# GrumpyZhou/patch2pix

Hardware: AMD Instinct MI355X
Metric: image-pairs/sec (480x640, ptmax=400), matching hot path, feature pyramids resident in HBM (higher is better)
Workload: dtype f32-equivalent: fp16x2 (every f32 operand, scaled by an exact power of two, = sum of 2 fp16 planes to within 2^-24 of its magnitude; 3 fp16 MFMA products per f32 product, f32 accumulate); second convolution as Winograd F(2x2,3x3) (transforms in f32, filters transformed in f64)

## Files before the change

include/p2p_hip.h:

```cpp
#ifndef P2P_HIP_H
#define P2P_HIP_H

#include <stddef.h>
#include <stdint.h>

#ifdef __cplusplus
extern "C" {
#endif

#define P2P_OK            0
#define P2P_EINVAL       -1
#define P2P_EHIP         -2
#define P2P_EUNSUPPORTED -3
#define P2P_ENOMEM       -4

typedef void *p2p_stream_t;
typedef struct p2p_ncn p2p_ncn;
typedef struct p2p_regressor p2p_regressor;

int p2p_version(void);
const char *p2p_last_error(void);


int p2p_ncn_create(const float *w1, const float *b1, const float *w2, const float *b2, p2p_ncn **out);
void p2p_ncn_destroy(p2p_ncn *ncn);
int p2p_ncn_set_tile(p2p_ncn *ncn, int ta, int tb, int tc);

typedef struct p2p_ncn_config { int n_layers, kernel_size[4], channels[4], symmetric; } p2p_ncn_config;
typedef struct p2p_ncn_tensors { const float *w[4], *b[4]; } p2p_ncn_tensors;
int p2p_ncn_create_config(const p2p_ncn_config *config, const p2p_ncn_tensors *tensors, p2p_ncn **out);
int p2p_ncn_is_generic(const p2p_ncn *ncn);

typedef struct p2p_bn_params {
    const float *weight, *bias, *running_mean, *running_var;
} p2p_bn_params;

typedef struct p2p_regressor_params {
    const float *conv1_w;
    p2p_bn_params bn1;
    const float *conv2_w;
    p2p_bn_params bn2;
    const float *fc1_w, *fc1_b;
    p2p_bn_params bnf1;
    const float *fc2_w, *fc2_b;
    p2p_bn_params bnf2;
    const float *fc3_w, *fc3_b;
} p2p_regressor_params;

int p2p_regressor_create(const p2p_regressor_params *params, p2p_regressor **out);
void p2p_regressor_destroy(p2p_regressor *reg);

#define P2P_REGRESS_F32     0
#define P2P_REGRESS_FP16X2  3
#define P2P_REGRESS_FP16X2W 4
#define P2P_REGRESS_DEFAULT P2P_REGRESS_FP16X2W
int p2p_regressor_set_mode(p2p_regressor *reg, int mode);
int p2p_regressor_get_mode(const p2p_regressor *reg);

#define P2P_FEAT_COMB_PRE  0
#define P2P_FEAT_COMB_POST 1
typedef struct p2p_regressor_config {
    int n_feat, feat_idx[4];
    int feat_comb;
    int n_conv, conv_dim[4], conv_ker[4], conv_str[4];
    int n_fc, fc_dim[4];
    int psize;
} p2p_regressor_config;
typedef struct p2p_regressor_tensors {
    const float *conv_w[4];
    p2p_bn_params conv_bn[4];
    const float *fc_w[4], *fc_b[4];
    p2p_bn_params fc_bn[4];
    const float *out_w, *out_b;
} p2p_regressor_tensors;
int p2p_regressor_create_config(const p2p_regressor_config *config, const p2p_regressor_tensors *tensors, p2p_regressor **out);
#define P2P_REGRESS_GENERIC 16


size_t p2p_coarse_workspace_bytes(int channels, int hA, int wA, int hB, int wB, int ksize);
size_t p2p_coarse_workspace_bytes_for(const p2p_ncn *ncn, int channels, int hA, int wA, int hB, int wB, int ksize);
size_t p2p_neigh_consensus_workspace_bytes(const p2p_ncn *ncn, int hA, int wA, int hB, int wB);

int p2p_coarse_forward(const float *featA, const float *featB, int channels, int hA, int wA, int hB, int wB,
                       int ksize, const p2p_ncn *ncn, float *corr4d_out, uint8_t *delta_out,
                       void *workspace, size_t workspace_bytes, p2p_stream_t stream);

int p2p_coarse_forward_batch(const float *featA, const float *featB, int batch, int channels, int hA, int wA, int hB,
                             int wB, int ksize, const p2p_ncn *ncn, float *corr4d_out, uint8_t *delta_out,
                             void *workspace, size_t workspace_bytes, p2p_stream_t stream);

int p2p_neigh_consensus_batch(const float *x, int batch, int hA, int wA, int hB, int wB, const p2p_ncn *ncn, float *y_out,
                              void *workspace, size_t workspace_bytes, p2p_stream_t stream);

int p2p_delta_unpack(const uint8_t *delta, size_t n, int ksize, int64_t *out, p2p_stream_t stream);

int p2p_coarse_matches(const float *corr4d, const uint8_t *delta, int hA, int wA, int hB, int wB, int ksize,
                       int upsample, int center, int64_t *matches_out, float *scores_out, p2p_stream_t stream);

int p2p_coarse_matches_batch(const float *corr4d, const uint8_t *delta, int batch, int hA, int wA, int hB, int wB,
                             int ksize, int upsample, int center, int64_t *matches_out, float *scores_out,
                             p2p_stream_t stream);

int p2p_coarse_matches_topk_batch(const float *corr4d, const uint8_t *delta, int batch, int hA, int wA, int hB, int wB,
                                  int ksize, int upsample, int center, int topk, int do_softmax,
                                  int64_t *matches_out, float *scores_out, p2p_stream_t stream);

#define P2P_SCORE_NONE    0
#define P2P_SCORE_SOFTMAX 1
#define P2P_SCORE_L1      2
size_t p2p_coarse_score_workspace_bytes(int batch, int hA, int wA, int hB, int wB);
int p2p_coarse_score_batch(const float *corr4d, int batch, int hA, int wA, int hB, int wB, int normalize,
                           float *cell_scores, float *pair_scores, void *workspace, size_t workspace_bytes,
                           p2p_stream_t stream);

size_t p2p_filter_coarse_workspace_bytes(int batch, int n);
int p2p_filter_coarse_batch(const int64_t *matches, const float *scores, int batch, int n, float ncn_thres, int mutual,
                            int64_t *out_matches, float *out_scores, int *out_counts, void *workspace,
                            size_t workspace_bytes, p2p_stream_t stream);

int p2p_match_tail_batch(const float *fine, const float *scores, const int64_t *coarse, const int *counts,
                         const double *scale, int batch, int stride, float io_thres, double *out_matches,
                         float *out_scores, double *out_coarse, int *out_counts, p2p_stream_t stream);

#define P2P_F32 0
#define P2P_F64 1
#define P2P_I64 2
#define P2P_EPI_SAMPSON  0
#define P2P_EPI_SYM      1
#define P2P_EPI_SYM_SQRT 2
#define P2P_EPI_VALUE    3
int p2p_epipolar_batch(const void *matches, int matches_dtype, const int *counts, const double *F, int batch, int stride,
                       int kind, double eps, const double *edges, int nbins, void *dist, int dist_dtype, int *hist,
                       p2p_stream_t stream);



int p2p_correlation_batch(const float *featA, const float *featB, int batch, int channels, int hA, int wA, int hB, int wB,
                          float *out, p2p_stream_t stream);

int p2p_maxpool4d_batch(const float *x, int batch, int h1, int w1, int h2, int w2, int k, float *pooled_out, uint8_t *delta_out,
                        p2p_stream_t stream);

size_t p2p_mutual_matching_workspace_bytes(int batch, int hA, int wA, int hB, int wB);
int p2p_mutual_matching_batch(const float *x, int batch, int hA, int wA, int hB, int wB, float *y_out, void *workspace,
                              size_t workspace_bytes, p2p_stream_t stream);

typedef struct p2p_conv4d p2p_conv4d;
int p2p_conv4d_create(const float *weight, const float *bias, int c_in, int c_out, int kernel_size, p2p_conv4d **out);
void p2p_conv4d_destroy(p2p_conv4d *conv);
int p2p_conv4d_forward_batch(const p2p_conv4d *conv, const float *x, int batch, int h1, int w1, int h2, int w2, float *y_out,
                             p2p_stream_t stream);

int p2p_l2_normalize(const float *x, size_t outer, int channels, size_t inner, float *y, p2p_stream_t stream);


typedef struct p2p_pyramid {
    const float *level[4];
    int height, width;
} p2p_pyramid;

size_t p2p_regress_workspace_bytes(int n);
size_t p2p_regress_workspace_bytes_mode(int n, int mode);
size_t p2p_regress_workspace_bytes_for(const p2p_regressor *reg, int n);
int p2p_regress(const p2p_regressor *reg1, const p2p_regressor *reg2,
                const p2p_pyramid *im1, const p2p_pyramid *im2,
                const void *proposals, int is_float, int n,
                float *matches1, float *probs1, float *raw1,
                float *matches2, float *probs2, float *raw2,
                void *workspace, size_t workspace_bytes, p2p_stream_t stream);

int p2p_regress_batch(const p2p_regressor *reg1, const p2p_regressor *reg2, int nitems,
                      const p2p_pyramid *im1, const p2p_pyramid *im2, const int *counts,
                      const void *proposals, int is_float,
                      float *matches1, float *probs1, float *raw1,
                      float *matches2, float *probs2, float *raw2,
                      void *workspace, size_t workspace_bytes, p2p_stream_t stream);

int p2p_regress_batch_dev(const p2p_regressor *reg1, const p2p_regressor *reg2, int nitems,
                          const p2p_pyramid *im1, const p2p_pyramid *im2, const int *dev_counts, int stride,
                          const void *proposals, int is_float,
                          float *matches1, float *probs1, float *raw1,
                          float *matches2, float *probs2, float *raw2,
                          void *workspace, size_t workspace_bytes, p2p_stream_t stream);


typedef struct p2p_conv p2p_conv;
int p2p_conv_create(const float *weight, const p2p_bn_params *bn, int ci, int co, int ks, int stride, p2p_conv **out);
void p2p_conv_destroy(p2p_conv *conv);
int p2p_conv_set_tile(p2p_conv *conv, int mt, int nt, int wn);

int p2p_conv_forward(const p2p_conv *conv, const float *x, const int *xmax, int n, int h, int w, const float *residual,
                     int relu, float *y, int *ymax, p2p_stream_t stream);

typedef struct p2p_stem p2p_stem;
int p2p_stem_create(const float *weight, const p2p_bn_params *bn, p2p_stem **out);
void p2p_stem_destroy(p2p_stem *stem);
int p2p_stem_forward(const p2p_stem *stem, const float *image, const int *imax, int n, int h, int w, float *y, p2p_stream_t stream);

int p2p_maxpool_nhwc(const float *x, int n, int c, int h, int w, float *y, int *ymax, p2p_stream_t stream);

int p2p_nhwc_to_nchw(const float *x, int n, int h, int w, int c, float *y, p2p_stream_t stream);

int p2p_absmax_batch(const float *x, size_t count, int items, int *out, p2p_stream_t stream);


typedef struct p2p_resize_item {
    const uint8_t *pixels;
    int in_h, in_w;
    const int32_t *table_x, *table_y;
    int ksize_x, ksize_y;
} p2p_resize_item;
size_t p2p_resize_workspace_bytes(int batch, int max_in_h, int max_in_w, int out_h, int out_w);
int p2p_resize_bicubic_batch(const p2p_resize_item *items, int batch, int out_h, int out_w, uint8_t *out_u8, float *out_f32,
                             size_t out_f32_stride, const float *lut, void *workspace, size_t workspace_bytes,
                             p2p_stream_t stream);

#ifdef __cplusplus
}
#endif
#endif
```

patch2pix_amd/_lib.py:

```python
import ctypes
import os

import torch

_HERE = os.path.dirname(os.path.abspath(__file__))
LIB_PATH = os.path.join(_HERE, "csrc", "libp2p_hip.so")
_ALLOW_EXPERIMENT = os.environ.get("P2P_ALLOW_EXPERIMENT") == "1"
if os.environ.get("P2P_LIB_PATH"):
    if not _ALLOW_EXPERIMENT:
        raise ImportError("P2P_LIB_PATH is set but P2P_ALLOW_EXPERIMENT=1 is not: refusing to load a library other than "
                          f"{LIB_PATH}")
    LIB_PATH = os.environ["P2P_LIB_PATH"]

if not os.path.exists(LIB_PATH):
    raise ImportError(
        f"{LIB_PATH} not found: build the HIP extension first (python -m patch2pix_amd.build, "
        "or __graft_entry__.build()). There is no CPU fallback for the matching path.")

lib = ctypes.CDLL(LIB_PATH)

c_float_p = ctypes.c_void_p
c_stream = ctypes.c_void_p


class BnParams(ctypes.Structure):
    _fields_ = [("weight", ctypes.c_void_p), ("bias", ctypes.c_void_p),
                ("running_mean", ctypes.c_void_p), ("running_var", ctypes.c_void_p)]


class RegressorParams(ctypes.Structure):
    _fields_ = [("conv1_w", ctypes.c_void_p), ("bn1", BnParams),
                ("conv2_w", ctypes.c_void_p), ("bn2", BnParams),
                ("fc1_w", ctypes.c_void_p), ("fc1_b", ctypes.c_void_p), ("bnf1", BnParams),
                ("fc2_w", ctypes.c_void_p), ("fc2_b", ctypes.c_void_p), ("bnf2", BnParams),
                ("fc3_w", ctypes.c_void_p), ("fc3_b", ctypes.c_void_p)]


class RegressorConfig(ctypes.Structure):
    _fields_ = [("n_feat", ctypes.c_int), ("feat_idx", ctypes.c_int * 4), ("feat_comb", ctypes.c_int),
                ("n_conv", ctypes.c_int), ("conv_dim", ctypes.c_int * 4), ("conv_ker", ctypes.c_int * 4),
                ("conv_str", ctypes.c_int * 4), ("n_fc", ctypes.c_int), ("fc_dim", ctypes.c_int * 4), ("psize", ctypes.c_int)]


class RegressorTensors(ctypes.Structure):
    _fields_ = [("conv_w", ctypes.c_void_p * 4), ("conv_bn", BnParams * 4),
                ("fc_w", ctypes.c_void_p * 4), ("fc_b", ctypes.c_void_p * 4), ("fc_bn", BnParams * 4),
                ("out_w", ctypes.c_void_p), ("out_b", ctypes.c_void_p)]


class NcnConfig(ctypes.Structure):
    _fields_ = [("n_layers", ctypes.c_int), ("kernel_size", ctypes.c_int * 4), ("channels", ctypes.c_int * 4),
                ("symmetric", ctypes.c_int)]


class NcnTensors(ctypes.Structure):
    _fields_ = [("w", ctypes.c_void_p * 4), ("b", ctypes.c_void_p * 4)]


class ResizeItem(ctypes.Structure):
    _fields_ = [("pixels", ctypes.c_void_p), ("in_h", ctypes.c_int), ("in_w", ctypes.c_int),
                ("table_x", ctypes.c_void_p), ("table_y", ctypes.c_void_p), ("ksize_x", ctypes.c_int), ("ksize_y", ctypes.c_int)]


class Pyramid(ctypes.Structure):
    _fields_ = [("level", ctypes.c_void_p * 4), ("height", ctypes.c_int), ("width", ctypes.c_int)]


def _sig(name, restype, argtypes):
    fn = getattr(lib, name)
    fn.restype = restype
    fn.argtypes = argtypes
    return fn


p2p_version = _sig("p2p_version", ctypes.c_int, [])
VERSION_EXPERIMENT = 0x40000000
if p2p_version() & VERSION_EXPERIMENT and not _ALLOW_EXPERIMENT:
    raise ImportError(f"{LIB_PATH} is an experiment build (-DP2P_EXPERIMENT); set P2P_ALLOW_EXPERIMENT=1 to load it")
p2p_last_error = _sig("p2p_last_error", ctypes.c_char_p, [])
p2p_ncn_create = _sig("p2p_ncn_create", ctypes.c_int,
                      [ctypes.c_void_p] * 4 + [ctypes.POINTER(ctypes.c_void_p)])
p2p_ncn_destroy = _sig("p2p_ncn_destroy", None, [ctypes.c_void_p])
p2p_ncn_set_tile = _sig("p2p_ncn_set_tile", ctypes.c_int, [ctypes.c_void_p] + [ctypes.c_int] * 3)
p2p_ncn_create_config = _sig("p2p_ncn_create_config", ctypes.c_int,
                             [ctypes.POINTER(NcnConfig), ctypes.POINTER(NcnTensors), ctypes.POINTER(ctypes.c_void_p)])
p2p_ncn_is_generic = _sig("p2p_ncn_is_generic", ctypes.c_int, [ctypes.c_void_p])
p2p_regressor_create = _sig("p2p_regressor_create", ctypes.c_int,
                            [ctypes.POINTER(RegressorParams), ctypes.POINTER(ctypes.c_void_p)])
p2p_regressor_create_config = _sig("p2p_regressor_create_config", ctypes.c_int,
                                   [ctypes.POINTER(RegressorConfig), ctypes.POINTER(RegressorTensors),
                                    ctypes.POINTER(ctypes.c_void_p)])
p2p_regressor_destroy = _sig("p2p_regressor_destroy", None, [ctypes.c_void_p])
p2p_coarse_workspace_bytes = _sig("p2p_coarse_workspace_bytes", ctypes.c_size_t, [ctypes.c_int] * 6)
p2p_coarse_workspace_bytes_for = _sig("p2p_coarse_workspace_bytes_for", ctypes.c_size_t, [ctypes.c_void_p] + [ctypes.c_int] * 6)
p2p_neigh_consensus_workspace_bytes = _sig("p2p_neigh_consensus_workspace_bytes", ctypes.c_size_t,
                                           [ctypes.c_void_p] + [ctypes.c_int] * 4)
p2p_coarse_forward = _sig("p2p_coarse_forward", ctypes.c_int,
                          [ctypes.c_void_p, ctypes.c_void_p] + [ctypes.c_int] * 6 +
                          [ctypes.c_void_p, ctypes.c_void_p, ctypes.c_void_p, ctypes.c_void_p, ctypes.c_size_t, c_stream])
p2p_coarse_forward_batch = _sig("p2p_coarse_forward_batch", ctypes.c_int,
                                [ctypes.c_void_p, ctypes.c_void_p] + [ctypes.c_int] * 7 +
                                [ctypes.c_void_p, ctypes.c_void_p, ctypes.c_void_p, ctypes.c_void_p, ctypes.c_size_t, c_stream])
p2p_neigh_consensus_batch = _sig("p2p_neigh_consensus_batch", ctypes.c_int,
                                 [ctypes.c_void_p] + [ctypes.c_int] * 5 + [ctypes.c_void_p, ctypes.c_void_p, ctypes.c_void_p,
                                                                           ctypes.c_size_t, c_stream])
p2p_delta_unpack = _sig("p2p_delta_unpack", ctypes.c_int,
                        [ctypes.c_void_p, ctypes.c_size_t, ctypes.c_int, ctypes.c_void_p, c_stream])
p2p_coarse_matches = _sig("p2p_coarse_matches", ctypes.c_int,
                          [ctypes.c_void_p, ctypes.c_void_p] + [ctypes.c_int] * 7 +
                          [ctypes.c_void_p, ctypes.c_void_p, c_stream])
p2p_coarse_matches_batch = _sig("p2p_coarse_matches_batch", ctypes.c_int,
                                [ctypes.c_void_p, ctypes.c_void_p] + [ctypes.c_int] * 8 +
                                [ctypes.c_void_p, ctypes.c_void_p, c_stream])
p2p_coarse_matches_topk_batch = _sig("p2p_coarse_matches_topk_batch", ctypes.c_int,
                                     [ctypes.c_void_p, ctypes.c_void_p] + [ctypes.c_int] * 10 +
                                     [ctypes.c_void_p, ctypes.c_void_p, c_stream])
p2p_coarse_score_workspace_bytes = _sig("p2p_coarse_score_workspace_bytes", ctypes.c_size_t, [ctypes.c_int] * 5)
p2p_coarse_score_batch = _sig("p2p_coarse_score_batch", ctypes.c_int,
                              [ctypes.c_void_p] + [ctypes.c_int] * 6 +
                              [ctypes.c_void_p, ctypes.c_void_p, ctypes.c_void_p, ctypes.c_size_t, c_stream])
SCORE_NORMS = {None: 0, "softmax": 1, "l1": 2}
p2p_filter_coarse_workspace_bytes = _sig("p2p_filter_coarse_workspace_bytes", ctypes.c_size_t, [ctypes.c_int, ctypes.c_int])
p2p_filter_coarse_batch = _sig("p2p_filter_coarse_batch", ctypes.c_int,
                               [ctypes.c_void_p, ctypes.c_void_p, ctypes.c_int, ctypes.c_int, ctypes.c_float, ctypes.c_int,
                                ctypes.c_void_p, ctypes.c_void_p, ctypes.c_void_p, ctypes.c_void_p, ctypes.c_size_t, c_stream])
p2p_match_tail_batch = _sig("p2p_match_tail_batch", ctypes.c_int,
                            [ctypes.c_void_p] * 5 + [ctypes.c_int, ctypes.c_int, ctypes.c_float] + [ctypes.c_void_p] * 4 + [c_stream])
p2p_epipolar_batch = _sig("p2p_epipolar_batch", ctypes.c_int,
                          [ctypes.c_void_p, ctypes.c_int, ctypes.c_void_p, ctypes.c_void_p, ctypes.c_int, ctypes.c_int, ctypes.c_int,
                           ctypes.c_double, ctypes.c_void_p, ctypes.c_int, ctypes.c_void_p, ctypes.c_int, ctypes.c_void_p, c_stream])
DTYPES = {"float32": 0, "float64": 1, "int64": 2}
EPI_KINDS = {"sampson": 0, "sym": 1, "sym_sqrt": 2, "value": 3}
EPI_MAX_BINS = 16
p2p_regress = _sig("p2p_regress", ctypes.c_int,
                   [ctypes.c_void_p, ctypes.c_void_p, ctypes.POINTER(Pyramid), ctypes.POINTER(Pyramid),
                    ctypes.c_void_p, ctypes.c_int, ctypes.c_int] + [ctypes.c_void_p] * 6 + [ctypes.c_void_p, ctypes.c_size_t, c_stream])
p2p_regress_workspace_bytes = _sig("p2p_regress_workspace_bytes", ctypes.c_size_t, [ctypes.c_int])
p2p_regress_workspace_bytes_mode = _sig("p2p_regress_workspace_bytes_mode", ctypes.c_size_t, [ctypes.c_int, ctypes.c_int])
p2p_regress_workspace_bytes_for = _sig("p2p_regress_workspace_bytes_for", ctypes.c_size_t, [ctypes.c_void_p, ctypes.c_int])

p2p_regress_batch = _sig("p2p_regress_batch", ctypes.c_int,
                         [ctypes.c_void_p, ctypes.c_void_p, ctypes.c_int, ctypes.POINTER(Pyramid), ctypes.POINTER(Pyramid),
                          ctypes.POINTER(ctypes.c_int), ctypes.c_void_p, ctypes.c_int] + [ctypes.c_void_p] * 6 +
                         [ctypes.c_void_p, ctypes.c_size_t, c_stream])

p2p_regress_batch_dev = _sig("p2p_regress_batch_dev", ctypes.c_int,
                             [ctypes.c_void_p, ctypes.c_void_p, ctypes.c_int, ctypes.POINTER(Pyramid), ctypes.POINTER(Pyramid),
                              ctypes.c_void_p, ctypes.c_int, ctypes.c_void_p, ctypes.c_int] + [ctypes.c_void_p] * 6 +
                             [ctypes.c_void_p, ctypes.c_size_t, c_stream])

p2p_conv_create = _sig("p2p_conv_create", ctypes.c_int,
                       [ctypes.c_void_p, ctypes.POINTER(BnParams)] + [ctypes.c_int] * 4 + [ctypes.POINTER(ctypes.c_void_p)])
p2p_conv_destroy = _sig("p2p_conv_destroy", None, [ctypes.c_void_p])
p2p_conv_set_tile = _sig("p2p_conv_set_tile", ctypes.c_int, [ctypes.c_void_p, ctypes.c_int, ctypes.c_int, ctypes.c_int])
p2p_conv_forward = _sig("p2p_conv_forward", ctypes.c_int,
                        [ctypes.c_void_p, ctypes.c_void_p, ctypes.c_void_p] + [ctypes.c_int] * 3 +
                        [ctypes.c_void_p, ctypes.c_int, ctypes.c_void_p, ctypes.c_void_p, c_stream])
p2p_stem_create = _sig("p2p_stem_create", ctypes.c_int, [ctypes.c_void_p, ctypes.POINTER(BnParams), ctypes.POINTER(ctypes.c_void_p)])
p2p_stem_destroy = _sig("p2p_stem_destroy", None, [ctypes.c_void_p])
p2p_stem_forward = _sig("p2p_stem_forward", ctypes.c_int, [ctypes.c_void_p] * 3 + [ctypes.c_int] * 3 + [ctypes.c_void_p, c_stream])
p2p_maxpool_nhwc = _sig("p2p_maxpool_nhwc", ctypes.c_int, [ctypes.c_void_p] + [ctypes.c_int] * 4 + [ctypes.c_void_p, ctypes.c_void_p, c_stream])
p2p_nhwc_to_nchw = _sig("p2p_nhwc_to_nchw", ctypes.c_int, [ctypes.c_void_p] + [ctypes.c_int] * 4 + [ctypes.c_void_p, c_stream])
p2p_absmax_batch = _sig("p2p_absmax_batch", ctypes.c_int, [ctypes.c_void_p, ctypes.c_size_t, ctypes.c_int, ctypes.c_void_p, c_stream])

p2p_resize_workspace_bytes = _sig("p2p_resize_workspace_bytes", ctypes.c_size_t, [ctypes.c_int] * 5)
p2p_resize_bicubic_batch = _sig("p2p_resize_bicubic_batch", ctypes.c_int,
                                [ctypes.POINTER(ResizeItem)] + [ctypes.c_int] * 3 +
                                [ctypes.c_void_p, ctypes.c_void_p, ctypes.c_size_t, ctypes.c_void_p, ctypes.c_void_p, ctypes.c_size_t,
                                 c_stream])

p2p_correlation_batch = _sig("p2p_correlation_batch", ctypes.c_int, [ctypes.c_void_p, ctypes.c_void_p] + [ctypes.c_int] * 6 + [ctypes.c_void_p, c_stream])
p2p_maxpool4d_batch = _sig("p2p_maxpool4d_batch", ctypes.c_int, [ctypes.c_void_p] + [ctypes.c_int] * 6 + [ctypes.c_void_p, ctypes.c_void_p, c_stream])
p2p_mutual_matching_workspace_bytes = _sig("p2p_mutual_matching_workspace_bytes", ctypes.c_size_t, [ctypes.c_int] * 5)
p2p_mutual_matching_batch = _sig("p2p_mutual_matching_batch", ctypes.c_int,
                                 [ctypes.c_void_p] + [ctypes.c_int] * 5 + [ctypes.c_void_p, ctypes.c_void_p, ctypes.c_size_t, c_stream])
p2p_conv4d_create = _sig("p2p_conv4d_create", ctypes.c_int, [ctypes.c_void_p, ctypes.c_void_p] + [ctypes.c_int] * 3 + [ctypes.POINTER(ctypes.c_void_p)])
p2p_conv4d_destroy = _sig("p2p_conv4d_destroy", None, [ctypes.c_void_p])
p2p_conv4d_forward_batch = _sig("p2p_conv4d_forward_batch", ctypes.c_int,
                                [ctypes.c_void_p, ctypes.c_void_p] + [ctypes.c_int] * 5 + [ctypes.c_void_p, c_stream])
p2p_l2_normalize = _sig("p2p_l2_normalize", ctypes.c_int, [ctypes.c_void_p, ctypes.c_size_t, ctypes.c_int, ctypes.c_size_t, ctypes.c_void_p, c_stream])

p2p_regressor_set_mode = _sig("p2p_regressor_set_mode", ctypes.c_int, [ctypes.c_void_p, ctypes.c_int])
p2p_regressor_get_mode = _sig("p2p_regressor_get_mode", ctypes.c_int, [ctypes.c_void_p])
REGRESS_MODES = {"f32": 0, "fp16x2": 3, "fp16x2w": 4}
REGRESS_GENERIC = 16
FEAT_COMB = {"pre": 0, "post": 1}

EXPORTS = ["p2p_version", "p2p_last_error", "p2p_ncn_create", "p2p_ncn_destroy", "p2p_ncn_set_tile", "p2p_regressor_create",
           "p2p_regressor_destroy", "p2p_coarse_workspace_bytes", "p2p_coarse_forward", "p2p_coarse_forward_batch",
           "p2p_neigh_consensus_batch", "p2p_delta_unpack", "p2p_coarse_matches", "p2p_coarse_matches_batch", "p2p_filter_coarse_workspace_bytes", "p2p_filter_coarse_batch", "p2p_match_tail_batch", "p2p_regress", "p2p_regress_workspace_bytes", "p2p_regress_workspace_bytes_mode", "p2p_regress_batch", "p2p_regress_batch_dev", "p2p_regressor_set_mode",
           "p2p_regressor_get_mode", "p2p_conv_create", "p2p_conv_destroy", "p2p_conv_set_tile", "p2p_conv_forward", "p2p_absmax_batch", "p2p_stem_create", "p2p_stem_destroy", "p2p_stem_forward",
           "p2p_maxpool_nhwc", "p2p_nhwc_to_nchw", "p2p_regressor_create_config", "p2p_regress_workspace_bytes_for",
           "p2p_coarse_matches_topk_batch", "p2p_ncn_create_config", "p2p_ncn_is_generic", "p2p_coarse_workspace_bytes_for",
           "p2p_neigh_consensus_workspace_bytes", "p2p_resize_workspace_bytes", "p2p_resize_bicubic_batch",
           "p2p_coarse_score_workspace_bytes", "p2p_coarse_score_batch", "p2p_epipolar_batch",
           "p2p_correlation_batch", "p2p_maxpool4d_batch", "p2p_mutual_matching_workspace_bytes", "p2p_mutual_matching_batch",
           "p2p_conv4d_create", "p2p_conv4d_destroy", "p2p_conv4d_forward_batch", "p2p_l2_normalize"]


def check(status, what):
    if status != 0:
        msg = p2p_last_error().decode("utf-8", "replace")
        if status == -3:
            raise NotImplementedError(f"{what}: {msg}")
        raise RuntimeError(f"{what} failed with status {status}: {msg}")
```

patch2pix_amd/csrc/api.hip:

```cpp
#include "p2p_common.h"

namespace p2p {
static thread_local char g_err[512] = "";
void set_error(const char *fmt, ...) {
    va_list ap;
    va_start(ap, fmt);
    vsnprintf(g_err, sizeof(g_err), fmt, ap);
    va_end(ap);
}
}

#ifdef P2P_EXPERIMENT
extern "C" int p2p_version(void) { return 110 | P2P_VERSION_EXPERIMENT; }
#else
extern "C" int p2p_version(void) { return 110; }
#endif
extern "C" const char *p2p_last_error(void) { return p2p::g_err; }

#include "coarse_api.hip"
#include "operators_api.hip"
#include "regress_api.hip"
#include "preprocess.hip"
```

patch2pix_amd/csrc/coarse.hip:

```cpp
#include "coarse_common.h"

namespace p2p {

constexpr float MM_EPS = 1e-5f;

__device__ __forceinline__ int f2key(float f) {
    int b = __float_as_int(f);
    return b >= 0 ? b : b ^ 0x7fffffff;
}
__device__ __forceinline__ float key2f(int k) { return __int_as_float(k >= 0 ? k : k ^ 0x7fffffff); }
constexpr int KEY_NEG_INF = (int)0xff800000 ^ 0x7fffffff;

constexpr int PREP_P = 16;
constexpr float CORR_FP16_SCALE = 4096.0f;
__device__ __forceinline__ int prep_row_k4(int pp) { return (pp & ~31) + (pp & 3) + 2 * (pp & 12) + ((pp >> 2) & 4); }
template <bool PERM_A>
__global__ __launch_bounds__(256) void prep_kernel(PrepArgs a) {
    const int img = blockIdx.y;
    if (img == 0) {
        const int i = blockIdx.x * 256 + threadIdx.x;
        if (i <= a.nkeys) a.keys[blockIdx.z * a.sKeys + i] = (i < a.nkeys) ? KEY_NEG_INF : 0;
    }
    const int h = a.h[img], w = a.w[img], C = a.C, k = a.k;
    const bool perm = PERM_A && img == 0;
    if ((int)blockIdx.x * PREP_P >= h * w) return;
    const float *__restrict__ F = a.F[img] + blockIdx.z * a.sF[img];
    unsigned short *__restrict__ Fn = a.Fn[img] + blockIdx.z * a.sFn;
    if (((int)blockIdx.x + 1) * PREP_P >= h * w) {
        const int pad0 = h * w, pad1 = (pad0 + 127) & ~127, pieces = (C >> 5) * 2 * 4;
        for (int e = threadIdx.x; e < (pad1 - pad0) * pieces; e += 256) {
            const int pr = pad0 + e / pieces;
            const int r = (perm ? prep_row_k4(pr) : pr) & 127, q = e % pieces, kc = q >> 3, pl = (q >> 2) & 1, piece = q & 3;
            unsigned short *d = Fn + ((size_t)(pad0 >> 7) * (C >> 5) + kc) * (2 * 128 * 32) + pl * (128 * 32) + (r * 4 + piece) * 8;
            *(f32x4 *)d = (f32x4){0.f, 0.f, 0.f, 0.f};
        }
    }
    __shared__ float tile[256 * (PREP_P + 1)];
    __shared__ float part[16][PREP_P];
    __shared__ float inv[PREP_P];
    const int hw = h * w;
    const int p0 = blockIdx.x * PREP_P;
    const int tid = threadIdx.x;
    for (int e = tid; e < C * 4; e += 256) {
        const int c = e >> 2, q = e & 3;
        const int pos = p0 + 4 * q;
        f32x4 v = {0.f, 0.f, 0.f, 0.f};
        if (pos + 3 < hw && (hw & 3) == 0) v = *(const f32x4 *)(F + (size_t)c * hw + pos);
        else
            for (int i = 0; i < 4; ++i) if (pos + i < hw) v[i] = F[(size_t)c * hw + pos + i];
        float *t = tile + c * (PREP_P + 1) + 4 * q;
        t[0] = v[0]; t[1] = v[1]; t[2] = v[2]; t[3] = v[3];
    }
    __syncthreads();
    {
        const int p = tid & 15, g = tid >> 4;
        float ss = 0.f;
        for (int c = g; c < C; c += 16) { const float v = tile[c * (PREP_P + 1) + p]; ss = fmaf(v, v, ss); }
        part[g][p] = ss;
    }
    __syncthreads();
    if (tid < PREP_P) {
        float ss = 0.f;
#pragma unroll
        for (int g = 0; g < 16; ++g) ss += part[g][tid];
        inv[tid] = 1.0f / sqrtf(ss + 1e-6f);
    }
    __syncthreads();
    const int wc = w / k;
    for (int p = 0; p < PREP_P; ++p) {
        const int pos = p0 + p;
        if (pos >= hw) break;
        const int i = pos / w, j = pos - i * w;
        int pp = ((i / k) * wc + (j / k)) * (k * k) + (i % k) * k + (j % k);
        if (perm) pp = prep_row_k4(pp);
        for (int c = tid; c < C; c += 256) {
            const float x = tile[c * (PREP_P + 1) + p] * inv[p] * CORR_FP16_SCALE;
            const int r = pp & 127;
            unsigned short *d = Fn + ((size_t)(pp >> 7) * (C >> 5) + (c >> 5)) * (2 * 128 * 32) +
                                (r * 4 + (((c >> 3) & 3) ^ ((r >> 2) & 3))) * 8 + (c & 7);
            const _Float16 h0 = (_Float16)x;
            d[0] = __builtin_bit_cast(unsigned short, h0);
            d[128 * 32] = __builtin_bit_cast(unsigned short, (_Float16)(x - (float)h0));
        }
    }
}

void launch_prep(const PrepArgs &a, unsigned nz, hipStream_t stream) {
    const int gp = std::max(ceil_div(std::max(a.h[0] * a.w[0], a.h[1] * a.w[1]), PREP_P), ceil_div(a.nkeys + 1, 256));
    if (a.k == 4) hipLaunchKernelGGL(prep_kernel<true>, dim3(gp, 2, nz), dim3(256), 0, stream, a);
    else hipLaunchKernelGGL(prep_kernel<false>, dim3(gp, 2, nz), dim3(256), 0, stream, a);
}

constexpr int CT = 128;
constexpr int CX_AB = 16;
typedef _Float16 cf16x8 __attribute__((ext_vector_type(8)));
constexpr int CX_BLK = 2 * CT * 64;
constexpr int CX_STAGE = 2 * CX_BLK, CX_LDS = 2 * CX_STAGE;
__device__ __forceinline__ f32x16 cx_mfma(const f32x4 &a, const f32x4 &b, const f32x16 &c) {
    return __builtin_amdgcn_mfma_f32_32x32x16_f16(__builtin_bit_cast(cf16x8, a), __builtin_bit_cast(cf16x8, b), c, 0, 0, 0);
}
#define CX_ISSUE(IT, SLOT)                                                                                             \
    {                                                                                                                  \
        const unsigned char *ga_ = Ab + (size_t)(IT) * CX_BLK + lane16;                                                \
        const unsigned char *gb_ = Bb + (size_t)(IT) * CX_BLK + lane16;                                                \
        unsigned char *la_ = cx + (SLOT) * CX_STAGE + wave * 4096;                                                     \
        P2P_GLOBAL_LOAD_LDS16(ga_, la_, 0); P2P_GLOBAL_LOAD_LDS16(ga_, la_, 1024);                                     \
        P2P_GLOBAL_LOAD_LDS16(ga_, la_, 2048); P2P_GLOBAL_LOAD_LDS16(ga_, la_, 3072);                                  \
        P2P_GLOBAL_LOAD_LDS16(gb_, la_ + CX_BLK, 0); P2P_GLOBAL_LOAD_LDS16(gb_, la_ + CX_BLK, 1024);                   \
        P2P_GLOBAL_LOAD_LDS16(gb_, la_ + CX_BLK, 2048); P2P_GLOBAL_LOAD_LDS16(gb_, la_ + CX_BLK, 3072);                \
    }
#define CX_READ(FA, FB, SLOT, S)                                                                                       \
    {                                                                                                                  \
        const unsigned char *pa_ = cx + (SLOT) * CX_STAGE + ((S) ? aoff1 : aoff0);                                     \
        const unsigned char *pb_ = cx + (SLOT) * CX_STAGE + CX_BLK + ((S) ? boff1 : boff0);                            \
        _Pragma("unroll") for (int t_ = 0; t_ < 2; ++t_)                                                               \
            _Pragma("unroll") for (int q_ = 0; q_ < 2; ++q_) {                                                         \
                FA[t_][q_] = *(const f32x4 *)(pa_ + t_ * 2048 + q_ * 8192);                                            \
                FB[t_][q_] = *(const f32x4 *)(pb_ + t_ * 2048 + q_ * 8192);                                            \
            }                                                                                                          \
    }
#define CX_SLAB(FA, FB)                                                                                                \
    _Pragma("unroll") for (int t_ = 0; t_ < 3; ++t_) {                                                                 \
        const int pa_ = (t_ == 0) ? 1 : 0, pb_ = (t_ == 1) ? 1 : 0;                                                    \
        _Pragma("unroll") for (int i_ = 0; i_ < 2; ++i_)                                                               \
            _Pragma("unroll") for (int j_ = 0; j_ < 2; ++j_) acc[i_][j_] = cx_mfma(FA[i_][pa_], FB[j_][pb_], acc[i_][j_]); \
    }
#define CX_PIPE()                                                                                                      \
    _Pragma("unroll") for (int g_ = 0; g_ < 8; ++g_) {                                                                 \
        __builtin_amdgcn_sched_group_barrier(0x008, 1, 0); __builtin_amdgcn_sched_group_barrier(0x100, 1, 0); }        \
    __builtin_amdgcn_sched_group_barrier(0x008, 4, 0); __builtin_amdgcn_sched_barrier(0);

template <int KS>
__global__ __launch_bounds__(256, 2) void corr_pool_kernel(const unsigned short *__restrict__ A, const unsigned short *__restrict__ B,
                                                           int nA, int nB, int C, float *__restrict__ P,
                                                           uint8_t *__restrict__ delta, size_t sAB, size_t sP, size_t sDelta,
                                                           int gx, int gy, int ntiles, int per_xcd) {
    const int Gx = gridDim.x >> 3, xcd = blockIdx.x & 7;
    int tj = blockIdx.x >> 3;
    int rowA0 = 0, rowB0 = 0, zp = 0;
    const unsigned char *Ab = nullptr, *Bb = nullptr;
    auto locate = [&](int j, int &ra, int &rb, int &z, const unsigned char *&pa, const unsigned char *&pb) -> bool {
        const int L = xcd * per_xcd + j;
        if (j >= per_xcd || L >= ntiles) return false;
        const int tp = gx * gy;
        z = L / tp;
        const int r = L - z * tp;
        const int blk = r / (CX_AB * gx), rr = r - blk * (CX_AB * gx);
        const int hb = min(CX_AB, gy - blk * CX_AB);
        const int bcol = rr / hb, arow = blk * CX_AB + rr - bcol * hb;
        ra = arow * CT; rb = bcol * CT;
        pa = (const unsigned char *)(A + (size_t)z * sAB) + (size_t)arow * (C >> 5) * CX_BLK;
        pb = (const unsigned char *)(B + (size_t)z * sAB) + (size_t)bcol * (C >> 5) * CX_BLK;
        return true;
    };
    if (!locate(tj, rowA0, rowB0, zp, Ab, Bb)) return;
    P2P_DYN_SHARED(unsigned char, cx);
    const int tid = threadIdx.x, lane = tid & 63;
    const int wave = __builtin_amdgcn_readfirstlane(tid >> 6);
    const int wr = wave >> 1, wc = wave & 1;
    const int half = lane >> 5, l31 = lane & 31;
    const unsigned lane16 = wave * 4096 + lane * 16;
    const int sw = (l31 >> 2) & 3;
    const unsigned aoff0 = ((wr * 64 + l31) * 4 + ((0 + half) ^ sw)) * 16, aoff1 = ((wr * 64 + l31) * 4 + ((2 + half) ^ sw)) * 16;
    const unsigned boff0 = ((wc * 64 + l31) * 4 + ((0 + half) ^ sw)) * 16, boff1 = ((wc * 64 + l31) * 4 + ((2 + half) ^ sw)) * 16;

    const int nk = C / 32;
    CX_ISSUE(0, 0)
#pragma unroll 1
  for (;;) {
    f32x16 acc[2][2];
#pragma unroll
    for (int i = 0; i < 2; ++i)
#pragma unroll
        for (int j = 0; j < 2; ++j) acc[i][j] = (f32x16){0};

    f32x4 xa[2][2], xb[2][2], ya[2][2], yb[2][2];
#pragma unroll 1
    for (int it = 0; it < nk; it += 2) {
        P2P_WAIT_VMCNT(0);
        __builtin_amdgcn_s_barrier();
        __builtin_amdgcn_sched_barrier(0);
        if (it + 1 < nk) CX_ISSUE(it + 1, 1)
        CX_READ(xa, xb, 0, 0)
        __builtin_amdgcn_sched_barrier(0);
        CX_READ(ya, yb, 0, 1)
        CX_SLAB(xa, xb)
        CX_PIPE()
        CX_SLAB(ya, yb)
        __builtin_amdgcn_sched_barrier(0);
        if (it + 1 >= nk) break;
        P2P_WAIT_VMCNT(0);
        __builtin_amdgcn_s_barrier();
        __builtin_amdgcn_sched_barrier(0);
        if (it + 2 < nk) CX_ISSUE(it + 2, 0)
        CX_READ(xa, xb, 1, 0)
        __builtin_amdgcn_sched_barrier(0);
        CX_READ(ya, yb, 1, 1)
        CX_SLAB(xa, xb)
        CX_PIPE()
        CX_SLAB(ya, yb)
        __builtin_amdgcn_sched_barrier(0);
    }
    const int rowA0c = rowA0, rowB0c = rowB0;
    float *Pz = P + (size_t)zp * sP;
    uint8_t *dz = delta ? delta + (size_t)zp * sDelta : nullptr;
    tj += Gx;
    const bool more = locate(tj, rowA0, rowB0, zp, Ab, Bb);
    __builtin_amdgcn_s_barrier();
    if (more) CX_ISSUE(0, 0)
    __builtin_amdgcn_sched_barrier(0);
    constexpr float inv = 1.0f / (CORR_FP16_SCALE * CORR_FP16_SCALE);

    if (KS == 1) {
#pragma unroll
        for (int i = 0; i < 2; ++i)
#pragma unroll
            for (int j = 0; j < 2; ++j) {
                const int tr = rowA0c + wr * 64 + i * 32, tc = rowB0c + wc * 64 + j * 32;
#pragma unroll
                for (int r = 0; r < 16; ++r) {
                    const int row = tr + (r & 3) + 8 * (r >> 2) + 4 * half, col = tc + l31;
                    if (row < nA && col < nB) Pz[(size_t)row * nB + col] = acc[i][j][r] * inv;
                }
            }
    } else if (KS == 2)
    {
        const int nAc = nA >> 2, nBc = nB >> 2;
        const int crow0 = ((rowA0c + wr * 64) >> 2) + half, ccol0 = (rowB0c + wc * 64 + l31) >> 2;
        const bool writer = (lane & 3) == 0;
        const bool full = ((rowA0c + CT) >> 2) <= nAc && ((rowB0c + CT) >> 2) <= nBc;
        float pbest[2][2][4];
        int ps[2][2][4];
#pragma unroll
        for (int i = 0; i < 2; ++i)
#pragma unroll
            for (int j = 0; j < 2; ++j)
#pragma unroll
                for (int g = 0; g < 4; ++g) {
                    float best = acc[i][j][4 * g];
                    int s = 0;
#pragma unroll
                    for (int r = 1; r < 4; ++r) {
                        const float v = acc[i][j][4 * g + r];
                        if (v > best) { best = v; s = r; }
                    }
                    s = s * 4 + (lane & 3);
                    {
                        const float ov = __uint_as_float(P2P_SWAP_ADJACENT(__float_as_uint(best)));
                        const int os = (int)P2P_SWAP_ADJACENT((unsigned)s);
                        if (ov > best || (ov == best && os < s)) { best = ov; s = os; }
                    }
                    {
                        const float ov = __uint_as_float(P2P_SWAP_PAIRS(__float_as_uint(best)));
                        const int os = (int)P2P_SWAP_PAIRS((unsigned)s);
                        if (ov > best || (ov == best && os < s)) { best = ov; s = os; }
                    }
                    pbest[i][j][g] = best * inv;
                    ps[i][j][g] = s;
                }
        if (writer) {
            float *Pl = Pz + (unsigned)(crow0 * nBc + ccol0);
            uint8_t *Dl = dz ? dz + (unsigned)(crow0 * nBc + ccol0) : nullptr;
#pragma unroll
            for (int i = 0; i < 2; ++i)
#pragma unroll
                for (int j = 0; j < 2; ++j)
#pragma unroll
                    for (int g = 0; g < 4; ++g) {
                        const int dr = 8 * i + 2 * g, dc = 8 * j;
                        if (full || (crow0 + dr < nAc && ccol0 + dc < nBc)) {
                            const unsigned at = (unsigned)(dr * nBc + dc);
                            Pl[at] = pbest[i][j][g];
                            if (Dl) Dl[at] = (uint8_t)ps[i][j][g];
                        }
                    }
        }
    }
    if (KS == 4) {
        const int nAc = nA >> 4, nBc = nB >> 4;
        const int crow0 = ((rowA0c + wr * 64) >> 4) + half, ccol0 = (rowB0c + wc * 64 + l31) >> 4;
        float pbest[2][2];
        int ps[2][2];
#pragma unroll
        for (int i = 0; i < 2; ++i)
#pragma unroll
            for (int j = 0; j < 2; ++j) {
                float best = acc[i][j][0];
                int s = 0;
#pragma unroll
                for (int r = 1; r < 16; ++r) {
                    const float v = acc[i][j][r];
                    if (v > best) { best = v; s = r; }
                }
                s = s * 16 + (lane & 15);
#define CX_K4_STEP(XCHG)                                                                                               \
                {                                                                                                      \
                    const float ov = __uint_as_float(XCHG(__float_as_uint(best)));                                     \
                    const int os = (int)XCHG((unsigned)s);                                                             \
                    if (ov > best || (ov == best && os < s)) { best = ov; s = os; }                                    \
                }
                CX_K4_STEP(P2P_SWAP_ADJACENT)
                CX_K4_STEP(P2P_SWAP_PAIRS)
                CX_K4_STEP(P2P_MIRROR_HALF_ROW)
                CX_K4_STEP(P2P_SWAP_HALF_ROWS)
#undef CX_K4_STEP
                pbest[i][j] = best * inv;
                ps[i][j] = s;
            }
        if ((lane & 15) == 0) {
#pragma unroll
            for (int i = 0; i < 2; ++i)
#pragma unroll
                for (int j = 0; j < 2; ++j) {
                    const int cr = crow0 + 2 * i, cc = ccol0 + 2 * j;
                    if (cr < nAc && cc < nBc) {
                        const unsigned at = (unsigned)(cr * nBc + cc);
                        Pz[at] = pbest[i][j];
                        if (dz) dz[at] = (uint8_t)ps[i][j];
                    }
                }
        }
    }
    if (!more) break;
  }
}

int launch_corr_pool(const unsigned short *fnA, const unsigned short *fnB, int nA, int nB, int C, int ksize, float *P, uint8_t *delta,
                     size_t sAB, size_t sP, size_t sDelta, unsigned nz, hipStream_t stream) {
    static DeviceOnce attr_set_dev;
    const int dev = raise_lds_limit(attr_set_dev, {{(const void *)corr_pool_kernel<1>, CX_LDS}, {(const void *)corr_pool_kernel<2>, CX_LDS},
                                                   {(const void *)corr_pool_kernel<4>, CX_LDS}});
    if (dev < 0) return dev;
    const int gx = ceil_div(nB, CT), gy = ceil_div(nA, CT);
    const long long ntiles = (long long)gx * gy * nz;
    P2P_REQUIRE(ntiles < (1ll << 30), P2P_EUNSUPPORTED, "p2p_coarse_forward: %lld correlation tiles in one launch", ntiles);
    const int per_xcd = (int)((ntiles + 7) / 8);
    const dim3 cgrid((unsigned)(8 * std::min(per_xcd, 64)));
    if (ksize == 1) delta = nullptr, sDelta = 0;
    const auto kernel = ksize == 1 ? corr_pool_kernel<1> : (ksize == 4 ? corr_pool_kernel<4> : corr_pool_kernel<2>);
    hipLaunchKernelGGL(kernel, cgrid, dim3(256), CX_LDS, stream, fnA, fnB, nA, nB, C, P, delta, sAB, sP, sDelta, gx, gy, (int)ntiles, per_xcd);
    return P2P_OK;
}

__global__ __launch_bounds__(256) void maxima_kernel(const float *__restrict__ X, int nA, int nB, int *rkey, int *ckey, size_t sX,
                                                     size_t sKeys, const float *__restrict__ X2, int col_groups) {
    X += blockIdx.z * sX;
    if (X2) X2 += blockIdx.z * sX;
    rkey += blockIdx.z * sKeys;
    ckey += blockIdx.z * sKeys;
    const int gcol = (nB + 255) / 256;
    if ((int)blockIdx.x < col_groups) {
        const int col = ((int)blockIdx.x % gcol) * 256 + threadIdx.x;
        if (col >= nB) return;
        const int r0 = ((int)blockIdx.x / gcol) * 64, r1 = min(r0 + 64, nA);
        float cm = -INFINITY;
        if (X2) {
#pragma unroll 8
            for (int r = r0; r < r1; ++r) cm = fmaxf(cm, X[(size_t)r * nB + col] + X2[(size_t)r * nB + col]);
        } else {
#pragma unroll 8
            for (int r = r0; r < r1; ++r) cm = fmaxf(cm, X[(size_t)r * nB + col]);
        }
        atomicMax(&ckey[col], f2key(cm));
        return;
    }
    const int row = ((int)blockIdx.x - col_groups) * 4 + (threadIdx.x >> 6), lane = threadIdx.x & 63;
    if (row >= nA) return;
    const float *x = X + (size_t)row * nB;
    float rm = -INFINITY;
    if (X2) {
        const float *x2 = X2 + (size_t)row * nB;
        for (int c = lane; c < nB; c += 64) rm = fmaxf(rm, x[c] + x2[c]);
    } else {
        for (int c = lane; c < nB; c += 64) rm = fmaxf(rm, x[c]);
    }
#pragma unroll
    for (int m = 32; m >= 1; m >>= 1) rm = fmaxf(rm, __shfl_xor(rm, m));
    if (lane == 0) rkey[row] = f2key(rm);
}

void launch_maxima(const float *X, int nA, int nB, int *rkey, int *ckey, size_t sX, size_t sKeys, const float *X2, unsigned nz,
                   hipStream_t stream) {
    const int col_groups = ceil_div(nB, 256) * ceil_div(nA, 64);
    const dim3 grid(col_groups + ceil_div(nA, 4), 1, nz);
    hipLaunchKernelGGL(maxima_kernel, grid, dim3(256), 0, stream, X, nA, nB, rkey, ckey, sX, sKeys, X2, col_groups);
}

__device__ __forceinline__ float mm_value(float x, float max_over_b, float max_over_a) {
    const float xa = x / (max_over_b + MM_EPS);
    const float xb = x / (max_over_a + MM_EPS);
    return x * (xa * xb);
}

typedef int mm_i32x4 __attribute__((ext_vector_type(4)));
template <bool VEC>
__global__ __launch_bounds__(256) void mm_apply_kernel(const float *X, int nA, int nB, const int *__restrict__ rkey,
                                                       const int *__restrict__ ckey, float *out, size_t sX, size_t sKeys,
                                                       size_t sOut, int *amax, const float *X2) {
    X += blockIdx.z * sX;
    if (X2) X2 += blockIdx.z * sX;
    rkey += blockIdx.z * sKeys;
    ckey += blockIdx.z * sKeys;
    out += blockIdx.z * sOut;
    constexpr int V = VEC ? 4 : 1;
    const unsigned per_row = (unsigned)nB / V;
    const unsigned i = blockIdx.x * 256u + threadIdx.x;
    float m = 0.f;
    if (i < (unsigned)nA * per_row) {
        const unsigned r = i / per_row, c = (i - r * per_row) * V;
        const size_t at = (size_t)r * nB + c;
        const float mb = key2f(rkey[r]);
        if constexpr (VEC) {
            f32x4 x = *(const f32x4 *)(X + at);
            if (X2) {
                const f32x4 y = *(const f32x4 *)(X2 + at);
#pragma unroll
                for (int j = 0; j < 4; ++j) x[j] += y[j];
            }
            const mm_i32x4 ck = *(const mm_i32x4 *)(ckey + c);
            f32x4 v;
#pragma unroll
            for (int j = 0; j < 4; ++j) {
                v[j] = mm_value(x[j], mb, key2f(ck[j]));
                m = fmaxf(m, fabsf(v[j]));
            }
            *(f32x4 *)(out + at) = v;
        } else {
            const float v = mm_value(X2 ? X[at] + X2[at] : X[at], mb, key2f(ckey[c]));
            out[at] = v;
            m = fabsf(v);
        }
    }
    if (amax) {
#pragma unroll
        for (int d = 32; d >= 1; d >>= 1) m = fmaxf(m, __shfl_xor(m, d));
        int *dst = amax + blockIdx.z * sKeys;
        if ((threadIdx.x & 63) == 0 && __float_as_int(m) > *(volatile int *)dst) atomicMax(dst, __float_as_int(m));
    }
}

void launch_mm_apply(const float *X, int nA, int nB, const int *rkey, const int *ckey, float *out, size_t sX, size_t sKeys,
                     size_t sOut, int *amax, const float *X2, size_t nz, hipStream_t stream) {
    const bool vec = nB % 4 == 0 && sX % 4 == 0 && sOut % 4 == 0 && sKeys % 4 == 0 && ((uintptr_t)X & 15) == 0 &&
                     ((uintptr_t)out & 15) == 0 && ((uintptr_t)X2 & 15) == 0 && ((uintptr_t)ckey & 15) == 0;
    const size_t items = (size_t)nA * (nB / (vec ? 4 : 1));
    const dim3 grid((unsigned)((items + 255) / 256), 1, (unsigned)nz);
    if (vec) hipLaunchKernelGGL(mm_apply_kernel<true>, grid, dim3(256), 0, stream, X, nA, nB, rkey, ckey, out, sX, sKeys, sOut, amax, X2);
    else hipLaunchKernelGGL(mm_apply_kernel<false>, grid, dim3(256), 0, stream, X, nA, nB, rkey, ckey, out, sX, sKeys, sOut, amax, X2);
}

}

#include "consensus_generic.hip"
#include "matches.hip"
#include "score.hip"
#include "operators.hip"
```

patch2pix_amd/csrc/coarse_api.hip:

```cpp
#include "coarse_common.h"

using namespace p2p;

struct CoarseWs {
    size_t fnA, fnB, P, Y, Y2, keys, act, total;
};
static CoarseWs coarse_ws(int C, int hA, int wA, int hB, int wB, int k, const NcGen *gen = nullptr) {
    auto al = [](size_t b) { return (b + 255) & ~size_t(255); };
    const size_t nA = (size_t)hA * wA, nB = (size_t)hB * wB;
    const size_t nAc = nA / (k * k), nBc = nB / (k * k);
    CoarseWs w;
    size_t off = 0;
    w.fnA = off; off += al(((nA + 127) / 128) * 128 * C * 4);
    w.fnB = off; off += al(((nB + 127) / 128) * 128 * C * 4);
    w.P = off; off += al(nAc * nBc * 4);
    w.Y = off; off += al(nAc * nBc * 4);
    w.Y2 = off; off += al(nAc * nBc * 4);
    w.keys = off; off += al((2 * (nAc + nBc) + 1) * 4);
    w.act = off;
    if (gen) off += nc_generic_ws_bytes(*gen, nAc * nBc);
    w.total = off;
    return w;
}

extern "C" int p2p_ncn_create(const float *w1, const float *b1, const float *w2, const float *b2, p2p_ncn **out) {
    P2P_REQUIRE(w1 && b1 && w2 && b2 && out, P2P_EINVAL, "p2p_ncn_create: null argument");
    DeviceBlob wf;
    pack_nc_fused(w1, b1, w2, wf);
    const int st = wf.upload("p2p_ncn_create: the consensus weights");
    if (st != P2P_OK) return st;
    *out = new p2p_ncn{b2[0], std::move(wf), {0, 0, 0}, nullptr};
    return P2P_OK;
}

extern "C" int p2p_ncn_create_config(const p2p_ncn_config *config, const p2p_ncn_tensors *tensors, p2p_ncn **out) {
    P2P_REQUIRE(out, P2P_EINVAL, "p2p_ncn_create_config: null argument");
    NcGen *g = nullptr;
    const int st = nc_generic_create(config, tensors, &g);
    if (st != P2P_OK) return st;
    *out = new p2p_ncn{0.f, DeviceBlob(), {0, 0, 0}, g};
    return P2P_OK;
}

extern "C" int p2p_ncn_is_generic(const p2p_ncn *ncn) { return ncn ? (ncn->gen ? 1 : 0) : -1; }

extern "C" int p2p_ncn_set_tile(p2p_ncn *ncn, int ta, int tb, int tc) {
    P2P_REQUIRE(ncn && ta >= 0 && tb >= 0 && tc >= 0, P2P_EINVAL, "p2p_ncn_set_tile: bad argument");
    P2P_REQUIRE(!ncn->gen, P2P_EUNSUPPORTED, "p2p_ncn_set_tile: a generic consensus handle has no work-group tile to force");
    P2P_REQUIRE((tb > 0 && tc > 0) || (ta == 0 && tb == 0 && tc == 0), P2P_EINVAL,
                "p2p_ncn_set_tile: (%d, %d, %d) is neither (0, 0, 0) nor a tile with tb, tc > 0", ta, tb, tc);
    ncn->tile[0] = ta; ncn->tile[1] = tb; ncn->tile[2] = tc;
    return P2P_OK;
}

extern "C" void p2p_ncn_destroy(p2p_ncn *ncn) { delete ncn; }

extern "C" size_t p2p_coarse_workspace_bytes(int channels, int hA, int wA, int hB, int wB, int ksize) {
    if (channels <= 0 || hA <= 0 || wA <= 0 || hB <= 0 || wB <= 0 || ksize < 1) return 0;
    return coarse_ws(channels, hA, wA, hB, wB, ksize).total;
}

extern "C" size_t p2p_coarse_workspace_bytes_for(const p2p_ncn *ncn, int channels, int hA, int wA, int hB, int wB, int ksize) {
    if (!ncn || channels <= 0 || hA <= 0 || wA <= 0 || hB <= 0 || wB <= 0 || ksize < 1) return 0;
    return coarse_ws(channels, hA, wA, hB, wB, ksize, ncn->gen).total;
}

extern "C" size_t p2p_neigh_consensus_workspace_bytes(const p2p_ncn *ncn, int hA, int wA, int hB, int wB) {
    if (!ncn || hA <= 0 || wA <= 0 || hB <= 0 || wB <= 0) return 0;
    return ncn->gen ? nc_generic_ws_bytes(*ncn->gen, (size_t)hA * wA * hB * wB) : sizeof(int);
}

extern "C" int p2p_coarse_forward_batch(const float *featA, const float *featB, int batch, int C, int hA, int wA, int hB,
                                        int wB, int ksize, const p2p_ncn *ncn, float *corr4d_out, uint8_t *delta_out,
                                        void *workspace, size_t workspace_bytes, p2p_stream_t stream_) {
    hipStream_t stream = (hipStream_t)stream_;
    P2P_REQUIRE(featA && featB && ncn && corr4d_out && workspace, P2P_EINVAL, "p2p_coarse_forward: null argument");
    P2P_REQUIRE(batch >= 1 && batch <= 65535, P2P_EINVAL, "p2p_coarse_forward: batch %d out of range", batch);
    P2P_REQUIRE(ksize == 1 || ksize == 2 || ksize == 4, P2P_EUNSUPPORTED, "p2p_coarse_forward: ksize %d not supported (1, 2 or 4)", ksize);
    P2P_REQUIRE(C > 0 && C % 32 == 0 && C <= 256, P2P_EUNSUPPORTED, "p2p_coarse_forward: channels %d (multiple of 32, <= 256)", C);
    P2P_REQUIRE(hA > 0 && wA > 0 && hB > 0 && wB > 0 && hA % ksize == 0 && wA % ksize == 0 && hB % ksize == 0 &&
                    wB % ksize == 0, P2P_EINVAL, "p2p_coarse_forward: feature map sizes must be positive multiples of ksize");
    const size_t ws_any = coarse_ws(C, hA, wA, hB, wB, ksize).total;
    P2P_REQUIRE(workspace_bytes >= ws_any, P2P_ENOMEM, "p2p_coarse_forward: workspace %zu < %zu bytes (one pair)", workspace_bytes, ws_any);
    const CoarseWs ws = coarse_ws(C, hA, wA, hB, wB, ksize, ncn->gen);
    P2P_REQUIRE(workspace_bytes >= ws.total, P2P_ENOMEM, "p2p_coarse_forward: workspace %zu < %zu bytes (one pair)", workspace_bytes,
                ws.total);
    P2P_REQUIRE(!ncn->gen || ((uintptr_t)workspace & 15) == 0, P2P_EINVAL,
                "p2p_coarse_forward: the workspace of a generic handle must be 16-byte aligned");
    const int nA = hA * wA, nB = hB * wB, kk = ksize * ksize;
    const int nAc = nA / kk, nBc = nB / kk;
    const size_t nel = (size_t)nAc * nBc;
    const size_t sWs = ws.total / 4;
    const int per_launch = (int)std::min<size_t>(batch, workspace_bytes / ws.total);
    const int d0 = hA / ksize, d1 = wA / ksize, d2 = hB / ksize, d3 = wB / ksize;
    for (int z0 = 0; z0 < batch; z0 += per_launch) {
        const unsigned nz = (unsigned)std::min(per_launch, batch - z0);
        const float *fA = featA + (size_t)z0 * C * nA, *fB = featB + (size_t)z0 * C * nB;
        float *out = corr4d_out + (size_t)z0 * nel;
        uint8_t *dout = delta_out ? delta_out + (size_t)z0 * nel : nullptr;
        char *base = (char *)workspace;
        unsigned short *fnA = (unsigned short *)(base + ws.fnA), *fnB = (unsigned short *)(base + ws.fnB);
        float *P = (float *)(base + ws.P), *Y = (float *)(base + ws.Y), *Y2 = (float *)(base + ws.Y2);
        int *rkey1 = (int *)(base + ws.keys), *ckey1 = rkey1 + nAc, *rkey2 = ckey1 + nBc, *ckey2 = rkey2 + nAc;
        const int nkeys = 2 * (nAc + nBc);
        int *xmax = rkey1 + nkeys;
        launch_prep(PrepArgs{{fA, fB}, {fnA, fnB}, {hA, hB}, {wA, wB}, {(size_t)C * nA, (size_t)C * nB}, C, ksize, 2 * sWs, rkey1, nkeys, sWs},
                    nz, stream);
        int st = launch_corr_pool(fnA, fnB, nA, nB, C, ksize, P, dout, 2 * sWs, sWs, nel, nz, stream);
        if (st != P2P_OK) return st;
        launch_maxima(P, nAc, nBc, rkey1, ckey1, sWs, sWs, nullptr, nz, stream);
        launch_mm_apply(P, nAc, nBc, rkey1, ckey1, P, sWs, sWs, sWs, xmax, nullptr, nz, stream);
        if (ncn->gen) {
            st = launch_nc_generic(*ncn->gen, P, sWs, Y, sWs, (float *)(base + ws.act), sWs, (int)nz, d0, d1, d2, d3, stream);
            Y2 = nullptr;
        } else {
            st = launch_nc_fused(P, Y, Y2, sWs, (int)nz, d0, d1, d2, d3, ncn->wfused.dev<unsigned char>(), ncn->b2, xmax, sWs, ncn->tile, stream);
        }
        if (st != P2P_OK) return st;
        launch_maxima(Y, nAc, nBc, rkey2, ckey2, sWs, sWs, Y2, nz, stream);
        launch_mm_apply(Y, nAc, nBc, rkey2, ckey2, out, sWs, sWs, nel, nullptr, Y2, nz, stream);
    }
    return check_launch("coarse_forward kernels");
}

extern "C" int p2p_coarse_forward(const float *featA, const float *featB, int C, int hA, int wA, int hB, int wB,
                                  int ksize, const p2p_ncn *ncn, float *corr4d_out, uint8_t *delta_out,
                                  void *workspace, size_t workspace_bytes, p2p_stream_t stream) {
    return p2p_coarse_forward_batch(featA, featB, 1, C, hA, wA, hB, wB, ksize, ncn, corr4d_out, delta_out, workspace,
                                    workspace_bytes, stream);
}

extern "C" int p2p_neigh_consensus_batch(const float *x, int batch, int hA, int wA, int hB, int wB, const p2p_ncn *ncn, float *y_out,
                                         void *workspace, size_t workspace_bytes, p2p_stream_t stream_) {
    hipStream_t stream = (hipStream_t)stream_;
    P2P_REQUIRE(x && ncn && y_out && workspace, P2P_EINVAL, "p2p_neigh_consensus: null argument");
    P2P_REQUIRE(batch >= 1 && batch <= 65535 && hA > 0 && wA > 0 && hB > 0 && wB > 0, P2P_EINVAL, "p2p_neigh_consensus: bad sizes");
    if (ncn->gen) {
        const size_t cells = (size_t)hA * wA * hB * wB, per = nc_generic_ws_bytes(*ncn->gen, cells);
        P2P_REQUIRE(workspace_bytes >= per, P2P_ENOMEM, "p2p_neigh_consensus: workspace %zu < %zu bytes (one volume)", workspace_bytes, per);
        P2P_REQUIRE(((uintptr_t)workspace & 15) == 0, P2P_EINVAL, "p2p_neigh_consensus: the workspace of a generic handle must be 16-byte aligned");
        const int per_launch = (int)std::min<size_t>(batch, workspace_bytes / per);
        for (int z0 = 0; z0 < batch; z0 += per_launch) {
            const int st = launch_nc_generic(*ncn->gen, x + (size_t)z0 * cells, cells, y_out + (size_t)z0 * cells, cells, (float *)workspace,
                                             per / sizeof(float), std::min(per_launch, batch - z0), hA, wA, hB, wB, stream);
            if (st != P2P_OK) return st;
        }
        return P2P_OK;
    }
    P2P_REQUIRE(workspace_bytes >= (size_t)batch * sizeof(int), P2P_ENOMEM, "p2p_neigh_consensus: workspace of %zu bytes needed (4 per volume)",
                (size_t)batch * sizeof(int));
    const size_t nel = (size_t)hA * wA * hB * wB;
    int *xmax = (int *)workspace;
    P2P_HIP_CHECK(hipMemsetAsync(y_out, 0, (size_t)batch * nel * sizeof(float), stream));
    P2P_HIP_CHECK(hipMemsetAsync(xmax, 0, (size_t)batch * sizeof(int), stream));
    const int st = launch_absmax(x, nel, nel, batch, xmax, 1, stream);
    if (st != P2P_OK) return st;
    return launch_nc_fused(x, y_out, nullptr, nel, batch, hA, wA, hB, wB, ncn->wfused.dev<unsigned char>(), ncn->b2, xmax, 1, ncn->tile, stream);
}

extern "C" int p2p_delta_unpack(const uint8_t *delta, size_t n, int ksize, int64_t *out, p2p_stream_t stream) {
    P2P_REQUIRE(delta && out && ksize >= 1, P2P_EINVAL, "p2p_delta_unpack: bad argument");
    if (n == 0) return P2P_OK;
    launch_delta_unpack(delta, n, ksize, (long long *)out, (hipStream_t)stream);
    return check_launch("delta_unpack_kernel");
}

static int check_match_args(const char *fn, const float *corr4d, const uint8_t *delta, int batch, int hA, int wA, int hB, int wB,
                            int ksize, const int64_t *matches_out, const float *scores_out) {
    P2P_REQUIRE(corr4d && matches_out && scores_out, P2P_EINVAL, "%s: null argument", fn);
    P2P_REQUIRE(batch >= 1 && batch <= 65535, P2P_EINVAL, "%s: batch %d out of range", fn, batch);
    P2P_REQUIRE(hA > 0 && wA > 0 && hB > 0 && wB > 0 && ksize >= 1, P2P_EINVAL, "%s: bad sizes", fn);
    P2P_REQUIRE(ksize == 1 || delta, P2P_EINVAL, "%s: delta required when ksize > 1", fn);
    return P2P_OK;
}

extern "C" int p2p_coarse_matches_batch(const float *corr4d, const uint8_t *delta, int batch, int hA, int wA, int hB, int wB,
                                        int ksize, int upsample, int center, int64_t *matches_out, float *scores_out,
                                        p2p_stream_t stream) {
    const int st = check_match_args("p2p_coarse_matches", corr4d, delta, batch, hA, wA, hB, wB, ksize, matches_out, scores_out);
    if (st != P2P_OK) return st;
    const int nA = hA * wA, nB = hB * wB;
    MatchArgs m{corr4d, delta, hA, wA, hB, wB, ksize, upsample, center, (long long *)matches_out, scores_out,
                (size_t)nA * nB, (size_t)nA + nB};
    launch_matches(m, batch, (hipStream_t)stream);
    return check_launch("match kernels");
}

extern "C" int p2p_coarse_matches_topk_batch(const float *corr4d, const uint8_t *delta, int batch, int hA, int wA, int hB, int wB,
                                             int ksize, int upsample, int center, int topk, int do_softmax,
                                             int64_t *matches_out, float *scores_out, p2p_stream_t stream) {
    const int st = check_match_args("p2p_coarse_matches_topk", corr4d, delta, batch, hA, wA, hB, wB, ksize, matches_out, scores_out);
    if (st != P2P_OK) return st;
    const int nA = hA * wA, nB = hB * wB;
    P2P_REQUIRE(topk >= 1 && topk <= 8, P2P_EINVAL, "p2p_coarse_matches_topk: topk %d out of range (1 to 8)", topk);
    P2P_REQUIRE(topk <= std::min(nA, nB), P2P_EINVAL, "p2p_coarse_matches_topk: topk %d exceeds the %d cells of an image", topk,
                std::min(nA, nB));
    MatchArgs m{corr4d, delta, hA, wA, hB, wB, ksize, upsample, center, (long long *)matches_out, scores_out,
                (size_t)nA * nB, (size_t)topk * ((size_t)nA + nB)};
    launch_matches_topk(m, batch, topk, do_softmax ? 1 : 0, (hipStream_t)stream);
    return check_launch("top-k match kernels");
}

extern "C" size_t p2p_coarse_score_workspace_bytes(int batch, int hA, int wA, int hB, int wB) {
    if (batch < 1 || batch > 65535 || hA <= 0 || wA <= 0 || hB <= 0 || wB <= 0) return 0;
    return (size_t)batch * ((size_t)hA * wA + (size_t)hB * wB) * sizeof(float);
}

extern "C" int p2p_coarse_score_batch(const float *corr4d, int batch, int hA, int wA, int hB, int wB, int normalize,
                                      float *cell_scores, float *pair_scores, void *workspace, size_t workspace_bytes,
                                      p2p_stream_t stream) {
    P2P_REQUIRE(corr4d && pair_scores, P2P_EINVAL, "p2p_coarse_score: null argument");
    P2P_REQUIRE(batch >= 1 && batch <= 65535, P2P_EINVAL, "p2p_coarse_score: batch %d out of range", batch);
    P2P_REQUIRE(hA > 0 && wA > 0 && hB > 0 && wB > 0, P2P_EINVAL, "p2p_coarse_score: bad sizes");
    const long long nA = (long long)hA * wA, nB = (long long)hB * wB;
    P2P_REQUIRE(nA + nB < (1ll << 30), P2P_EINVAL, "p2p_coarse_score: bad sizes (%lld + %lld cells)", nA, nB);
    P2P_REQUIRE(normalize == P2P_SCORE_NONE || normalize == P2P_SCORE_SOFTMAX || normalize == P2P_SCORE_L1, P2P_EINVAL,
                "p2p_coarse_score: unknown normalisation %d", normalize);
    if (!cell_scores) {
        const size_t need = p2p_coarse_score_workspace_bytes(batch, hA, wA, hB, wB);
        P2P_REQUIRE(workspace && workspace_bytes >= need, P2P_ENOMEM, "p2p_coarse_score: workspace of %zu bytes needed without cell_scores",
                    need);
        P2P_REQUIRE(((uintptr_t)workspace & 3) == 0, P2P_EINVAL, "p2p_coarse_score: the workspace must be 4-byte aligned");
        cell_scores = (float *)workspace;
    }
    launch_score(ScoreArgs{corr4d, cell_scores, pair_scores, (int)nA, (int)nB, (size_t)(nA * nB)}, batch, normalize, (hipStream_t)stream);
    return check_launch("score kernels");
}

extern "C" int p2p_coarse_matches(const float *corr4d, const uint8_t *delta, int hA, int wA, int hB, int wB, int ksize,
                                  int upsample, int center, int64_t *matches_out, float *scores_out, p2p_stream_t stream) {
    return p2p_coarse_matches_batch(corr4d, delta, 1, hA, wA, hB, wB, ksize, upsample, center, matches_out, scores_out, stream);
}
```

patch2pix_amd/csrc/coarse_common.h:

```cpp
#pragma once
#include "host_pack.h"
#include <algorithm>

namespace p2p {

struct NcGen;

struct PrepArgs {
    const float *F[2];
    unsigned short *Fn[2];
    int h[2], w[2];
    size_t sF[2];
    int C, k;
    size_t sFn;
    int *keys;
    int nkeys;
    size_t sKeys;
};
void launch_prep(const PrepArgs &a, unsigned nz, hipStream_t stream);
int launch_corr_pool(const unsigned short *fnA, const unsigned short *fnB, int nA, int nB, int C, int ksize, float *P, uint8_t *delta,
                     size_t sAB, size_t sP, size_t sDelta, unsigned nz, hipStream_t stream);
void launch_maxima(const float *X, int nA, int nB, int *rkey, int *ckey, size_t sX, size_t sKeys, const float *X2, unsigned nz, hipStream_t stream);
void launch_mm_apply(const float *X, int nA, int nB, const int *rkey, const int *ckey, float *out, size_t sX, size_t sKeys,
                     size_t sOut, int *amax, const float *X2, size_t nz, hipStream_t stream);

struct MatchArgs {
    const float *X;
    const uint8_t *delta;
    int hA, wA, hB, wB, ksize, upsample, center;
    long long *matches;
    float *scores;
    size_t sX, sM;
};
void launch_matches(const MatchArgs &m, int batch, hipStream_t stream);
void launch_matches_topk(const MatchArgs &m, int batch, int topk, int do_softmax, hipStream_t stream);
void launch_delta_unpack(const uint8_t *delta, size_t n, int k, long long *out, hipStream_t stream);

struct ScoreArgs {
    const float *X;
    float *cells;
    float *pair;
    int nA, nB;
    size_t sX;
};
void launch_score(const ScoreArgs &a, int batch, int normalize, hipStream_t stream);

void pack_nc_fused(const float *w1, const float *b1, const float *w2, DeviceBlob &out);
int launch_nc_fused(const float *X, float *Y, float *Y2, size_t stride, int pairs, int d0, int d1, int d2, int d3,
                    const unsigned char *w_dev, float b2, const int *xmax, size_t xmax_stride, const int *forced_tile,
                    hipStream_t stream);
int launch_absmax(const float *x, size_t n, size_t stride, int pairs, int *out, size_t out_stride, hipStream_t stream);

int nc_generic_create(const p2p_ncn_config *cfg, const p2p_ncn_tensors *t, NcGen **out);
void nc_generic_destroy(NcGen *g);
size_t nc_generic_ws_bytes(const NcGen &g, size_t cells);
int launch_nc_generic(const NcGen &g, const float *X, size_t s_x, float *Y, size_t s_y, float *act, size_t s_act, int pairs,
                      int d0, int d1, int d2, int d3, hipStream_t stream);

struct Conv4dLayer;
int conv4d_create(const float *weight, const float *bias, int c_in, int c_out, int k, Conv4dLayer **out);
void conv4d_destroy(Conv4dLayer *h);
void conv4d_dims(const Conv4dLayer &h, int *c_in, int *c_out);
int launch_conv4d(const Conv4dLayer &h, const float *x, float *y, int pairs, int d0, int d1, int d2, int d3, hipStream_t stream);

struct CorrelationArgs {
    const float *A, *B;
    float *out;
    int C, nA, nB;
    size_t sA, sB, sOut;
};
void launch_correlation(const CorrelationArgs &a, int batch, hipStream_t stream);
struct MaxPool4dArgs {
    const float *x;
    float *pooled;
    uint8_t *code;
    int k, p1, p2, p3;
    size_t cells;
};
void launch_maxpool4d(const MaxPool4dArgs &a, int batch, hipStream_t stream);
void launch_l2_normalize(const float *x, size_t outer, int C, size_t inner, float *y, hipStream_t stream);
void launch_mutual_matching(const float *x, int nA, int nB, float *y, int *keys, size_t sKeys, int batch, hipStream_t stream);

}

struct p2p_ncn {
    float b2;
    p2p::DeviceBlob wfused;
    int tile[3];
    p2p::NcGen *gen;
    ~p2p_ncn() { p2p::nc_generic_destroy(gen); }
};

struct p2p_conv4d {
    p2p::Conv4dLayer *layer;
    ~p2p_conv4d() { p2p::conv4d_destroy(layer); }
};
```

patch2pix_amd/csrc/consensus.hip:

```cpp
#include "coarse_common.h"

#include <algorithm>
#include <cmath>
#include <cstdlib>
#include <cstring>
#include <vector>

namespace p2p {

typedef _Float16 nh8 __attribute__((ext_vector_type(8)));
typedef float nf4 __attribute__((ext_vector_type(4)));

constexpr int NCF_THREADS = 512, NCF_WAVES = 8, NCF_HWAVES = 4;
constexpr int NCF_W1_BYTES = 7 * 2 * 64 * 16;
constexpr int NCF_W2_BYTES = 5 * 2 * 64 * 16;
constexpr int NCF_C_FLOATS = 64;
constexpr int NCF_BRANCH_BYTES = NCF_W1_BYTES + NCF_W2_BYTES + NCF_C_FLOATS * 4;

struct NcFusedArgs {
    const float *X;
    float *Y;
    float *Y2;
    size_t stride;
    int d0, d1, d2, d3;
    int ta, tb, tc, td, P;
    int na, nb, nc, nd;
    const unsigned char *w;
    float b2;
    const int *xmax;
    size_t xmax_stride;
};

__host__ __device__ __forceinline__ int nc_hidden_used(int tc, int P) {
    const int n = (tc + 2) * P, r = ((n + 63) >> 6) * 64;
    return (n > r ? n : r) + 2;
}
__host__ __device__ __forceinline__ int nc_hidden_slots(int tc, int P) { return (nc_hidden_used(tc, P) + 15) & ~15; }
__host__ __device__ __forceinline__ int nc_yrow(int tc, int P) {
    int r = (tc * P + 3) & ~3;
    while ((r & 63) != 4 && (r & 63) != 12 && (r & 63) != 20 && (r & 63) != 28 && (r & 63) != 36 && (r & 63) != 44 && (r & 63) != 52 && (r & 63) != 60) r += 4;
    return r;
}
__device__ __forceinline__ int clampi(int v, int lo, int hi) { return v < lo ? lo : (v > hi ? hi : v); }
__device__ __forceinline__ unsigned short nf2h(float f) { return __builtin_bit_cast(unsigned short, (_Float16)f); }
__device__ __forceinline__ float nh2f(unsigned short b) { return (float)__builtin_bit_cast(_Float16, b); }
#define NCF_MFMA32(a, b, c) __builtin_amdgcn_mfma_f32_32x32x16_f16(__builtin_bit_cast(nh8, (a)), __builtin_bit_cast(nh8, (b)), (c), 0, 0, 0)
#define NCF_MFMA16(a, b, c) __builtin_amdgcn_mfma_f32_16x16x32_f16(__builtin_bit_cast(nh8, (a)), __builtin_bit_cast(nh8, (b)), (c), 0, 0, 0)

typedef _Float16 nh2 __attribute__((ext_vector_type(2)));
typedef float nf2 __attribute__((ext_vector_type(2)));
__device__ __forceinline__ unsigned npk(float x, float y) {
    const nf2 v = {x, y};
    return __builtin_bit_cast(unsigned, __builtin_convertvector(v, nh2));
}
__device__ __forceinline__ float npk_lo(unsigned h) { return (float)__builtin_bit_cast(nh2, h)[0]; }
__device__ __forceinline__ float npk_hi(unsigned h) { return (float)__builtin_bit_cast(nh2, h)[1]; }

#ifdef NCF_TIMING
#define NT_DECL unsigned nt_[8] = {0, 0, 0, 0, 0, 0, 0, 0}; unsigned nt_last_ = (unsigned)__builtin_amdgcn_s_memtime();
#define NT(i) { const unsigned n_ = (unsigned)__builtin_amdgcn_s_memtime(); nt_[i] += n_ - nt_last_; nt_last_ = n_; }
#else
#define NT_DECL
#define NT(i)
#endif
constexpr int NCF_KRING = 3;

__host__ __device__ __forceinline__ int nc_xplane(int tc, int P) { return (9 * (tc + 4) * P * 2 + 15) & ~15; }

template <int FTB>
__global__ __launch_bounds__(NCF_THREADS, 1) void nc_fused_kernel(NcFusedArgs a) {
    P2P_DYN_SHARED(unsigned char, sm);
    constexpr bool FIXED = FTB > 0;
    const int tid = threadIdx.x, lane = tid & 63, wave = __builtin_amdgcn_readfirstlane(tid >> 6);
    const int br = wave >> 2, hw = wave & 3;
    const float *X = a.X + (size_t)blockIdx.z * a.stride;
    float *Y = ((br && a.Y2) ? a.Y2 : a.Y) + (size_t)blockIdx.z * a.stride;
    const bool plain = a.Y2 != nullptr;
    int g = blockIdx.x;
    const int dt0 = (g % a.nd) * a.td; g /= a.nd;
    const int c0 = (g % a.nc) * a.tc; g /= a.nc;
    const int b0 = (g % a.nb) * a.tb; g /= a.nb;
    const int a0 = g * a.ta;
    const int TA = a.ta, TB = FIXED ? FTB : a.tb, TC = FIXED ? 8 : a.tc, TD = FIXED ? 40 : a.td, P = FIXED ? 44 : a.P;
    const int XROWS = TC + 4, HROWS = TC + 2;
    const int HNU = FIXED ? nc_hidden_used(8, 44) : nc_hidden_used(TC, P), HN = FIXED ? nc_hidden_slots(8, 44) : nc_hidden_slots(TC, P);
    const int XPLANE = FIXED ? nc_xplane(8, 44) : nc_xplane(TC, P);
    const int HKH = HN * 16, HPLANE = 2 * HKH;
    const int YROW = nc_yrow(TC, P), YSLOT = TB * YROW;
    unsigned char *Xs = sm;
    unsigned char *Hs = sm + 2 * XPLANE + br * 2 * HPLANE;
    float *Ya = (float *)(sm + 2 * XPLANE + 4 * HPLANE) + br * 3 * YSLOT;
    const size_t nB = (size_t)a.d2 * a.d3;

    const unsigned char *wb = a.w + (size_t)br * NCF_BRANCH_BYTES;
    nf4 w1[7][2];
#pragma unroll
    for (int s = 0; s < 7; ++s)
#pragma unroll
        for (int p = 0; p < 2; ++p) w1[s][p] = *(const nf4 *)(wb + ((s * 2 + p) * 64 + lane) * 16);
    nf4 w2[5][2];
#pragma unroll
    for (int s = 0; s < 5; ++s)
#pragma unroll
        for (int p = 0; p < 2; ++p) w2[s][p] = *(const nf4 *)(wb + NCF_W1_BYTES + ((s * 2 + p) * 64 + lane) * 16);
#pragma unroll
    for (int s = 0; s < 7; ++s)
#pragma unroll
        for (int p = 0; p < 2; ++p) P2P_OPAQUE_V4(w1[s][p]);
#pragma unroll
    for (int s = 0; s < 5; ++s)
#pragma unroll
        for (int p = 0; p < 2; ++p) P2P_OPAQUE_V4(w2[s][p]);
    const float *cf = (const float *)(wb + NCF_W1_BYTES + NCF_W2_BYTES);
    const int xeb = (a.xmax[(size_t)blockIdx.z * a.xmax_stride] >> 23) & 0xff;
    const int E = min(max(xeb - 126, 0), 100);
    const float up = __int_as_float((127 + E) << 23), down = __int_as_float((127 - E) << 23);
    const float xscale = 4096.0f * down;
    const float yun = cf[33] * up;
    float e1s[16], e1b[16];
    {
        const float hscale = cf[32] * down;
#pragma unroll
        for (int c = 0; c < 16; ++c) { e1s[c] = cf[c] * up * hscale; e1b[c] = cf[16 + c] * hscale; }
    }

    for (int i = tid; i < 2 * 3 * YSLOT; i += NCF_THREADS) ((float *)(sm + 2 * XPLANE + 4 * HPLANE))[i] = 0.f;
    for (int i = tid; i < 4 * HPLANE / 16; i += NCF_THREADS) *(nf4 *)(sm + 2 * XPLANE + i * 16) = (nf4){0.f, 0.f, 0.f, 0.f};

    const int a_hi = min(a0 + TA, a.d0);
    const int ap_first = max(a0 - 1, 0), ap_last = min(a0 + TA, a.d0 - 1);
    const int bp_first = max(b0 - 1, 0), bp_last = min(b0 + TB, a.d1 - 1);

    auto flush = [&](int aout) {
        float *slot = Ya + (aout % 3) * YSLOT;
        const int ybase = (aout * a.d1 + b0) * (int)nB + c0 * a.d3 + dt0 + lane;
        const bool lane_in = lane < TD && dt0 + lane < a.d3;
        auto row = [&](int r) {
            const int bb = r / TC, ro = r - bb * TC;
            if (lane < TD) {
                float *cell = slot + bb * YROW + ro * P + lane + 1;
                const float v = fmaxf(*cell + a.b2, 0.f);
                *cell = 0.f;
                if (lane_in && b0 + bb < a.d1 && c0 + ro < a.d2) {
                    float *dst = Y + (unsigned)(ybase + bb * (int)nB + ro * a.d3);
                    if (plain) *dst = v; else unsafeAtomicAdd(dst, v);
                }
            }
        };
        if (FIXED) {
#pragma unroll 2
            for (int i = 0; i < 2 * FTB; ++i) row(hw + NCF_HWAVES * i);
        } else {
            for (int r = hw; r < TB * TC; r += NCF_HWAVES) row(r);
        }
    };

    const int nbp = bp_last - bp_first + 1, nstrips = (ap_last - ap_first + 1) * nbp;
    const int sB = (int)nB, sA = a.d1 * sB;
    const int cp = min(lane & 31, P / 2 - 1), rh = lane >> 5;
    const int dcol = dt0 - 2 + 2 * cp;
    const int coff0 = clampi(dcol, 0, a.d3 - 1), coff1 = clampi(dcol + 1, 0, a.d3 - 1);
    const bool okd0 = dcol >= 0 && dcol < a.d3, okd1 = dcol + 1 >= 0 && dcol + 1 < a.d3;
    float q0v[NCF_KRING], q1v[NCF_KRING];
    int crow[NCF_KRING], lrow[NCF_KRING];
    float m0v[NCF_KRING], m1v[NCF_KRING];
#pragma unroll
    for (int k = 0; k < NCF_KRING; ++k) {
        const int it = wave + NCF_WAVES * k, i3 = min(it / 6, 2), rp = it - 6 * i3;
        const int xr = min(2 * rp + rh, XROWS - 1), ic = c0 - 2 + xr;
        crow[k] = clampi(ic, 0, a.d2 - 1) * a.d3;
        lrow[k] = (xr * P + 2 * cp) * 2;
        const bool rowok = ic >= 0 && ic < a.d2;
        m0v[k] = (rowok && okd0) ? xscale : 0.f;
        m1v[k] = (rowok && okd1) ? xscale : 0.f;
    }
    int isrc[NCF_KRING], idst[NCF_KRING];
    bool iin[NCF_KRING];
    const bool k0_second = wave >= 6, k1_third = wave >= 4;
    auto rot3 = [](int m, int i) { return m + i >= 3 ? m + i - 3 : m + i; };
    auto triple = [&](int pa, int pb, bool along_a, int ma, int mb) {
        int src3[3], dst3[3];
        bool in3[3];
#pragma unroll
        for (int i = 0; i < 3; ++i) {
            const int ia = along_a ? pa + i : pa, ib = along_a ? pb : pb + i;
            const int sa = along_a ? rot3(ma, i) : ma, sb = along_a ? mb : rot3(mb, i);
            src3[i] = clampi(ia, 0, a.d0 - 1) * sA + clampi(ib, 0, a.d1 - 1) * sB;
            in3[i] = ia >= 0 && ia < a.d0 && ib >= 0 && ib < a.d1;
            dst3[i] = (sa * 3 + sb) * XROWS * P * 2;
        }
        isrc[0] = k0_second ? src3[1] : src3[0]; iin[0] = k0_second ? in3[1] : in3[0]; idst[0] = k0_second ? dst3[1] : dst3[0];
        isrc[1] = k1_third ? src3[2] : src3[1]; iin[1] = k1_third ? in3[2] : in3[1]; idst[1] = k1_third ? dst3[2] : dst3[1];
        isrc[2] = src3[2]; iin[2] = in3[2]; idst[2] = dst3[2];
    };
    static_assert(NCF_KRING == 3 && NCF_WAVES == 8, "the item -> plane table above");
    auto ring_load = [&]() {
#pragma unroll
        for (int k = 0; k < NCF_KRING; ++k) {
            const int src = isrc[k] + crow[k];
            q0v[k] = X[(unsigned)(src + coff0)]; q1v[k] = X[(unsigned)(src + coff1)];
        }
    };
    auto ring_store = [&]() {
#pragma unroll
        for (int k = 0; k < NCF_KRING; ++k) {
            const float f = iin[k] ? 1.f : 0.f;
            const int dst = idst[k] + lrow[k];
            const float x0 = q0v[k] * m0v[k] * f, x1 = q1v[k] * m1v[k] * f;
            const unsigned h = npk(x0, x1);
            *(unsigned *)(Xs + dst) = h;
            *(unsigned *)(Xs + XPLANE + dst) = npk(x0 - npk_lo(h), x1 - npk_hi(h));
        }
    };

    const int l31 = lane & 31, kb5 = lane >> 5;
    const int nt1 = (HROWS * P + 63) >> 6;
    int s2qh[2] = {0, 0};
    int s2dst[2] = {0, 0};
    unsigned s2ok = 0;
#pragma unroll
    for (int u = 0; u < 2; ++u) {
        const int t = hw + NCF_HWAVES * u, q0 = t * 64;
        s2qh[u] = min(q0 + 2 * l31, HROWS * P - 2);
#pragma unroll
        for (int sp = 0; sp < 2; ++sp) {
            const int fl = q0 + 2 * l31 + sp, rowh = fl / P, col = fl - rowh * P;
            const int ic = c0 - 1 + rowh, id = dt0 + col - 1;
            const bool ok = t < nt1 && rowh < HROWS && col <= TD + 1 && ic >= 0 && ic < a.d2 && id >= 0 && id < a.d3;
            s2ok |= (unsigned)ok << (2 * u + sp);
        }
        s2dst[u] = (((s2ok >> (2 * u + kb5)) & 1u) ? q0 + 2 * l31 + kb5 + 1 : HNU) * 16;
    }
    const unsigned char *s2x[2] = {Xs + s2qh[0] * 2, Xs + s2qh[1] * 2};
    const int row16 = lane & 15, kb4 = lane >> 4;
    const int l2da3 = (lane & 15) / 3 % 3, l2da = (lane & 15) < 9 ? (lane & 15) / 3 : 64, l2db = (lane & 15) < 9 ? (lane & 15) % 3 : 64;
    int s3off[5];
#pragma unroll
    for (int st = 0; st < 5; ++st) {
        const int tap = min(2 * st + (kb4 >> 1), 8);
        s3off[st] = (kb4 & 1) * HKH + ((tap / 3) * P + tap % 3) * 16;
    }
    const int nt2 = (TC * P + 15) >> 4;

    auto strip_bp = [&](int ap, int j) { return (ap & 1) ? bp_last - j : bp_first + j; };
    __syncthreads();
    NT_DECL
    {
        const int bq = strip_bp(ap_first, 0);
        for (int i = 0; i < 3; ++i) {
            triple(ap_first - 1, bq - 1 + i, true, (ap_first + 2) % 3, (bq + 2 + i) % 3);
            ring_load();
            ring_store();
        }
    }
    __syncthreads();
    NT(0)
    int pending = -1;
    for (int strip = 0, row = 0, j = 0; strip < nstrips; ++strip, (j + 1 < nbp ? ++j : (j = 0, ++row))) {
        const int ap = ap_first + row, bp = strip_bp(ap, j);
        const bool more = strip + 1 < nstrips, same_row = j + 1 < nbp;
        const int dir = (ap & 1) ? -1 : 1;
        const int npa = same_row ? ap - 1 : ap + 2, npb = same_row ? bp + 2 * dir : bp - 1;
        if (pending >= 0) flush(pending);
        pending = -1;
        NT(5)
        const int am = (ap + 2) % 3, bm = (bp + 2) % 3;
        triple(npa, npb, same_row, am, same_row ? rot3(bm, dir > 0 ? 0 : 2) : bm);
        if (more) ring_load();
        {
            const int sa0 = am * 3 * XROWS * P, sa1 = rot3(am, 1) * 3 * XROWS * P, sa2 = rot3(am, 2) * 3 * XROWS * P;
            const int sl0 = bm * XROWS * P, sl1 = rot3(bm, 1) * XROWS * P, sl2 = rot3(bm, 2) * XROWS * P;
            auto xoff = [&](int gq) {
                const int da = gq / 9, db = (gq / 3) % 3, dc = gq % 3;
                return (da == 0 ? sa0 : da == 1 ? sa1 : sa2) + (db == 0 ? sl0 : db == 1 ? sl1 : sl2) + dc * P;
            };
            f32x16 acc[2] = {{0}, {0}};
            nf4 xv[2][2][2];
            auto frags = [&](int sl, nf4 (&d)[2][2]) {
                int oa0 = xoff(4 * sl), oa1 = xoff(4 * sl + 1), ob0 = xoff(4 * sl + 2), ob1 = xoff(min(4 * sl + 3, 26));
                P2P_OPAQUE_S(oa0); P2P_OPAQUE_S(oa1); P2P_OPAQUE_S(ob0); P2P_OPAQUE_S(ob1);
                const int o0 = kb5 ? ob0 : oa0, o1 = kb5 ? ob1 : oa1;
#pragma unroll
                for (int u = 0; u < 2; ++u)
#pragma unroll
                    for (int p = 0; p < 2; ++p) {
                        const unsigned *x0 = (const unsigned *)(s2x[u] + p * XPLANE + o0 * 2);
                        const unsigned *x1 = (const unsigned *)(s2x[u] + p * XPLANE + o1 * 2);
                        d[u][p] = (nf4){__uint_as_float(x0[0]), __uint_as_float(x0[1]), __uint_as_float(x1[0]), __uint_as_float(x1[1])};
                    }
            };
            frags(0, xv[0]);
#ifndef NCF_NOPRIO
            __builtin_amdgcn_s_setprio(1);
#endif
#pragma unroll
            for (int sl = 0; sl < 7; ++sl) {
                nf4 (&c)[2][2] = xv[sl & 1];
                if (sl < 6) frags(sl + 1, xv[(sl + 1) & 1]);
                acc[0] = NCF_MFMA32(w1[sl][0], c[0][1], acc[0]); acc[1] = NCF_MFMA32(w1[sl][0], c[1][1], acc[1]);
                acc[0] = NCF_MFMA32(w1[sl][1], c[0][0], acc[0]); acc[1] = NCF_MFMA32(w1[sl][1], c[1][0], acc[1]);
                acc[0] = NCF_MFMA32(w1[sl][0], c[0][0], acc[0]); acc[1] = NCF_MFMA32(w1[sl][0], c[1][0], acc[1]);
#pragma unroll
                for (int q = 0; q < 6; ++q) {
                    __builtin_amdgcn_sched_group_barrier(0x008, 1, 0);
                    __builtin_amdgcn_sched_group_barrier(0x002, 6, 0);
                    __builtin_amdgcn_sched_group_barrier(0x100, 2, 0);
                }
                __builtin_amdgcn_sched_barrier(0);
            }
            __builtin_amdgcn_s_setprio(0);
#pragma unroll
            for (int u = 0; u < 2; ++u) {
                if (hw + NCF_HWAVES * u >= nt1) break;
                unsigned char *dst = Hs + s2dst[u];
#pragma unroll
                for (int kh = 0; kh < 2; ++kh) {
                    float h[8];
#pragma unroll
                    for (int j = 0; j < 4; ++j) {
                        const nf2 av = {acc[u][8 * kh + 2 * j], acc[u][8 * kh + 2 * j + 1]};
                        const nf2 sv = {e1s[8 * kh + 2 * j], e1s[8 * kh + 2 * j + 1]}, bv = {e1b[8 * kh + 2 * j], e1b[8 * kh + 2 * j + 1]};
                        const nf2 hv = __builtin_elementwise_fma(av, sv, bv);
                        h[2 * j] = fmaxf(hv[0], 0.f); h[2 * j + 1] = fmaxf(hv[1], 0.f);
                    }
                    unsigned p0[4], p1[4];
#pragma unroll
                    for (int j = 0; j < 4; ++j) {
                        p0[j] = npk(h[2 * j], h[2 * j + 1]);
                        p1[j] = npk(h[2 * j] - npk_lo(p0[j]), h[2 * j + 1] - npk_hi(p0[j]));
                    }
                    *(nf4 *)(dst + kh * HKH) = (nf4){__uint_as_float(p0[0]), __uint_as_float(p0[1]), __uint_as_float(p0[2]), __uint_as_float(p0[3])};
                    *(nf4 *)(dst + kh * HKH + HPLANE) = (nf4){__uint_as_float(p1[0]), __uint_as_float(p1[1]), __uint_as_float(p1[2]), __uint_as_float(p1[3])};
                }
            }
        }
        NT(1)
        __syncthreads();
        NT(2)
        {
            const int aout = ap + 1 - l2da, bout = bp + 1 - l2db;
            const bool lane_ok = aout >= a0 && aout < a_hi && bout >= b0 && bout < min(b0 + TB, a.d1);
            const int apm = rot3(am, 2), sl3 = apm - l2da3;
            float *ydst = Ya + (sl3 < 0 ? sl3 + 3 : sl3) * YSLOT + (bout - b0) * YROW;
            const bool yalign = (YROW & 3) == 0;
            if (FIXED) {
                const unsigned char *hl = Hs + row16 * 16;
                float *yl = ydst + 4 * kb4;
#pragma unroll
                for (int i = 0; i < 3; ++i) {
                    const int qa = (hw + 8 * i) * 16;
                    const bool has_b = i < 2 || hw < 2;
                    const int qb = has_b ? qa + 64 : qa;
                    const unsigned char *ha = hl + qa * 16, *hb = hl + qb * 16;
                    nf4 accA = {0.f, 0.f, 0.f, 0.f}, accB = {0.f, 0.f, 0.f, 0.f};
                    nf4 fr[2][4];
                    auto frags3 = [&](int st, nf4 (&d)[4]) {
                        d[0] = *(const nf4 *)(ha + s3off[st]); d[1] = *(const nf4 *)(ha + s3off[st] + HPLANE);
                        d[2] = *(const nf4 *)(hb + s3off[st]); d[3] = *(const nf4 *)(hb + s3off[st] + HPLANE);
                    };
                    frags3(0, fr[0]);
#pragma unroll
                    for (int st = 0; st < 5; ++st) {
                        nf4 (&c)[4] = fr[st & 1];
                        if (st < 4) frags3(st + 1, fr[(st + 1) & 1]);
                        __builtin_amdgcn_sched_barrier(0);
                        accA = NCF_MFMA16(c[1], w2[st][0], accA); accB = NCF_MFMA16(c[3], w2[st][0], accB);
                        accA = NCF_MFMA16(c[0], w2[st][1], accA); accB = NCF_MFMA16(c[2], w2[st][1], accB);
                        accA = NCF_MFMA16(c[0], w2[st][0], accA); accB = NCF_MFMA16(c[2], w2[st][0], accB);
                        __builtin_amdgcn_sched_barrier(0);
                    }
                    if (lane_ok) {
                        nf4 va = *(nf4 *)(yl + qa);
                        va += accA * yun;
                        *(nf4 *)(yl + qa) = va;
                        if (has_b) {
                            nf4 vb = *(nf4 *)(yl + qb);
                            vb += accB * yun;
                            *(nf4 *)(yl + qb) = vb;
                        }
                    }
                }
            } else
            for (int t = hw; t < nt2; t += 2 * NCF_HWAVES) {
                const int qa = t * 16, qb = qa + NCF_HWAVES * 16;
                const unsigned char *ha = Hs + min(qa + row16, TC * P - 1) * 16, *hb = Hs + min(qb + row16, TC * P - 1) * 16;
                nf4 accA = {0.f, 0.f, 0.f, 0.f}, accB = {0.f, 0.f, 0.f, 0.f};
                nf4 fr[2][4];
                auto frags3 = [&](int st, nf4 (&d)[4]) {
                    d[0] = *(const nf4 *)(ha + s3off[st]); d[1] = *(const nf4 *)(ha + s3off[st] + HPLANE);
                    d[2] = *(const nf4 *)(hb + s3off[st]); d[3] = *(const nf4 *)(hb + s3off[st] + HPLANE);
                };
                frags3(0, fr[0]);
#pragma unroll
                for (int st = 0; st < 5; ++st) {
                    nf4 (&c)[4] = fr[st & 1];
                    if (st < 4) frags3(st + 1, fr[(st + 1) & 1]);
                    __builtin_amdgcn_sched_barrier(0);
                    accA = NCF_MFMA16(c[1], w2[st][0], accA); accB = NCF_MFMA16(c[3], w2[st][0], accB);
                    accA = NCF_MFMA16(c[0], w2[st][1], accA); accB = NCF_MFMA16(c[2], w2[st][1], accB);
                    accA = NCF_MFMA16(c[0], w2[st][0], accA); accB = NCF_MFMA16(c[2], w2[st][0], accB);
                    __builtin_amdgcn_sched_barrier(0);
                }
                if (lane_ok) {
                    float *ya = ydst + qa + 4 * kb4, *yb = ydst + qb + 4 * kb4;
                    if (yalign) {
                        if (qa + 4 * kb4 + 3 < TC * P) {
                            nf4 v = *(nf4 *)ya;
                            v += accA * yun;
                            *(nf4 *)ya = v;
                        } else {
#pragma unroll
                            for (int r = 0; r < 4; ++r) if (qa + 4 * kb4 + r < TC * P) ya[r] += accA[r] * yun;
                        }
                        if (qb + 4 * kb4 + 3 < TC * P) {
                            nf4 v = *(nf4 *)yb;
                            v += accB * yun;
                            *(nf4 *)yb = v;
                        } else {
#pragma unroll
                            for (int r = 0; r < 4; ++r) if (qb + 4 * kb4 + r < TC * P) yb[r] += accB[r] * yun;
                        }
                    } else {
#pragma unroll
                        for (int r = 0; r < 4; ++r) {
                            if (qa + 4 * kb4 + r < TC * P) ya[r] += accA[r] * yun;
                            if (qb + 4 * kb4 + r < TC * P) yb[r] += accB[r] * yun;
                        }
                    }
                }
            }
        }
        NT(3)
        if (more) ring_store();
        NT(4)
        if (!same_row && ap - 1 >= a0) pending = ap - 1;
        __syncthreads();
        NT(6)
    }
    if (pending >= 0) flush(pending);
    if (nstrips > 0 && ap_last < a_hi && ap_last >= a0) flush(ap_last);
#ifdef NCF_TIMING
    __syncthreads();
    if (blockIdx.x == 5 && br == 0 && lane == 0) {
        for (int i = 0; i < 8; ++i) Y[hw * 8 + i] = (float)nt_[i];
        Y[32] = (float)nstrips;
    }
#endif
}

static void put2(unsigned char *frag, int lane, int j, float v) {
    uint16_t *d = (uint16_t *)frag;
    split_fp16_planes(v, &d[lane * 8 + j], &d[(64 + lane) * 8 + j]);
}

void pack_nc_fused(const float *w1, const float *b1, const float *w2, DeviceBlob &out) {
    unsigned char *const bytes = out.at<unsigned char>(out.take<unsigned char>(2 * NCF_BRANCH_BYTES));
    auto W1 = [&](int o, int da, int db, int dc, int dd) { return w1[(((da * 16 + o) * 3 + db) * 3 + dc) * 3 + dd]; };
    auto W2 = [&](int c, int da, int db, int dc, int dd) { return w2[(((da * 16 + c) * 3 + db) * 3 + dc) * 3 + dd]; };
    for (int br = 0; br < 2; ++br) {
        auto W1b = [&](int o, int da, int db, int dc, int dd) { return br ? W1(o, dc, dd, da, db) : W1(o, da, db, dc, dd); };
        auto W2b = [&](int c, int da, int db, int dc, int dd) { return br ? W2(c, dc, dd, da, db) : W2(c, da, db, dc, dd); };
        unsigned char *base = bytes + (size_t)br * NCF_BRANCH_BYTES;
        int t1[16];
        float hmax = 0.f, w2max = 0.f;
        for (int o = 0; o < 16; ++o) {
            float mx = 0.f, sum = std::fabs(b1[o]);
            for (int t = 0; t < 81; ++t) {
                const float v = W1b(o, t / 27, (t / 9) % 3, (t / 3) % 3, t % 3);
                mx = std::max(mx, std::fabs(v));
                sum += std::fabs(v);
            }
            t1[o] = pow2_exponent_to(mx, 12);
            hmax = std::max(hmax, sum);
            for (int t = 0; t < 81; ++t) w2max = std::max(w2max, std::fabs(W2b(o, t / 27, (t / 9) % 3, (t / 3) % 3, t % 3)));
        }
        const int sh = pow2_exponent_to(2.f * hmax, 13), t2 = pow2_exponent_to(w2max, 12);
        for (int sl = 0; sl < 7; ++sl)
            for (int lane = 0; lane < 64; ++lane)
                for (int j = 0; j < 8; ++j) {
                    const int k = sl * 16 + 8 * (lane >> 5) + j, gq = k >> 2, e = k & 3;
                    const int n = lane & 31, s = (n >> 2) & 1, o = (n & 3) + 4 * (n >> 3), dd = e - s;
                    float v = 0.f;
                    if (gq < 27 && dd >= 0 && dd <= 2) v = std::ldexp(W1b(o, gq / 9, (gq / 3) % 3, gq % 3, dd), t1[o]);
                    put2(base + sl * 2 * 64 * 16, lane, j, v);
                }
        for (int st = 0; st < 5; ++st)
            for (int lane = 0; lane < 64; ++lane)
                for (int j = 0; j < 8; ++j) {
                    const int kb = lane >> 4, tap = 2 * st + (kb >> 1), ch = 8 * (kb & 1) + j, n = lane & 15;
                    float v = 0.f;
                    if (tap < 9 && n < 9) v = std::ldexp(W2b(ch, n / 3, n % 3, tap / 3, tap % 3), t2);
                    put2(base + NCF_W1_BYTES + st * 2 * 64 * 16, lane, j, v);
                }
        float *cf = (float *)(base + NCF_W1_BYTES + NCF_W2_BYTES);
        for (int o = 0; o < 16; ++o) {
            cf[o] = std::ldexp(1.f, -12 - t1[o]);
            cf[16 + o] = b1[o];
        }
        cf[32] = std::ldexp(1.f, sh);
        cf[33] = std::ldexp(1.f, -sh - t2);
    }
}

size_t nc_fused_lds_bytes(int tb, int tc, int P) {
    return (size_t)2 * nc_xplane(tc, P) + 2 * ((size_t)2 * 2 * nc_hidden_slots(tc, P) * 16 + (size_t)3 * tb * nc_yrow(tc, P) * 4);
}

__global__ __launch_bounds__(256) void absmax_kernel(const float *__restrict__ x, size_t n, size_t stride, int *out, size_t out_stride) {
    __shared__ float part[4];
    x += (size_t)blockIdx.z * stride;
    float m = 0.f;
    const size_t n4 = (((size_t)x & 15) == 0) ? n >> 2 : 0;
    const size_t step = (size_t)gridDim.x * 256;
    size_t i = (size_t)blockIdx.x * 256 + threadIdx.x;
    for (; i + 3 * step < n4; i += 4 * step) {
        const nf4 v0 = ((const nf4 *)x)[i], v1 = ((const nf4 *)x)[i + step], v2 = ((const nf4 *)x)[i + 2 * step], v3 = ((const nf4 *)x)[i + 3 * step];
        m = fmaxf(fmaxf(m, fmaxf(fabsf(v0[0]), fabsf(v0[1]))), fmaxf(fabsf(v0[2]), fabsf(v0[3])));
        m = fmaxf(fmaxf(m, fmaxf(fabsf(v1[0]), fabsf(v1[1]))), fmaxf(fabsf(v1[2]), fabsf(v1[3])));
        m = fmaxf(fmaxf(m, fmaxf(fabsf(v2[0]), fabsf(v2[1]))), fmaxf(fabsf(v2[2]), fabsf(v2[3])));
        m = fmaxf(fmaxf(m, fmaxf(fabsf(v3[0]), fabsf(v3[1]))), fmaxf(fabsf(v3[2]), fabsf(v3[3])));
    }
    for (; i < n4; i += step) {
        const nf4 v = ((const nf4 *)x)[i];
        m = fmaxf(fmaxf(m, fmaxf(fabsf(v[0]), fabsf(v[1]))), fmaxf(fabsf(v[2]), fabsf(v[3])));
    }
    for (size_t j = 4 * n4 + (size_t)blockIdx.x * 256 + threadIdx.x; j < n; j += step) m = fmaxf(m, fabsf(x[j]));
#pragma unroll
    for (int d = 32; d >= 1; d >>= 1) m = fmaxf(m, __shfl_xor(m, d));
    if ((threadIdx.x & 63) == 0) part[threadIdx.x >> 6] = m;
    __syncthreads();
    if (threadIdx.x == 0) {
        const float mm = fmaxf(fmaxf(part[0], part[1]), fmaxf(part[2], part[3]));
        int *dst = out + (size_t)blockIdx.z * out_stride;
        if (__float_as_int(mm) > *(volatile int *)dst) atomicMax(dst, __float_as_int(mm));
    }
}

int launch_absmax(const float *x, size_t n, size_t stride, int pairs, int *out, size_t out_stride, hipStream_t stream) {
    const unsigned blocks = (unsigned)std::min<size_t>((n + 16383) / 16384, 256);
    hipLaunchKernelGGL(absmax_kernel, dim3(blocks, 1, pairs), dim3(256), 0, stream, x, n, stride, out, out_stride);
    return check_launch("absmax_kernel");
}

constexpr size_t NCF_LDS_MAX = 160 * 1024;
constexpr int NCF_SLOTS = 256;

static long nc_fused_tile(NcFusedArgs &a, int pairs, const int *forced) {
    const int d0 = a.d0, d1 = a.d1, d2 = a.d2, d3 = a.d3;
    a.nd = ceil_div(d3, 60);
    a.td = ceil_div(d3, a.nd);
    a.P = (a.td + 4 + 1) & ~1;
    a.tc = 8;
    const bool forced_bc = forced && forced[1] > 0 && forced[2] > 0;
    if (forced_bc) a.tc = forced[2];
    a.tc = std::min(a.tc, d2);
    while (a.tc > 1 && (a.tc + 4 > 12 || (a.tc + 2) * a.P > 512)) --a.tc;
    a.nc = ceil_div(d2, a.tc);
    const int forced_ta = forced_bc ? forced[0] : 0;
    long best = -1;
    int best_ta = 0, best_tb = 0;
    for (int cand : {10, 5}) {
        int tb = std::min(forced_bc ? forced[1] : cand, d1);
        while (tb > 1 && nc_fused_lds_bytes(tb, a.tc, a.P) > NCF_LDS_MAX) --tb;
        const long per_a = (long)ceil_div(d1, tb) * a.nc * a.nd * pairs;
        int ta = forced_ta > 0 ? forced_ta : d0;
        if (forced_ta <= 0)
            while (ta > 4 && ceil_div(d0, ta) * per_a < NCF_SLOTS) ta = (ta + 1) / 2;
        ta = std::min(ta, d0);
        const long groups = ceil_div(d0, ta) * per_a;
        const long cost = (groups + NCF_SLOTS - 1) / NCF_SLOTS * (ta + 2) * (tb + 2);
        if (best < 0 || cost < best) { best = cost; best_ta = ta; best_tb = tb; }
        if (forced_bc) break;
    }
    a.ta = best_ta; a.tb = best_tb;
    a.na = ceil_div(d0, a.ta); a.nb = ceil_div(d1, a.tb);
    return (long)a.na * a.nb * a.nc * a.nd * pairs;
}

int launch_nc_fused(const float *X, float *Y, float *Y2, size_t stride, int pairs, int d0, int d1, int d2, int d3,
                    const unsigned char *w_dev, float b2, const int *xmax, size_t xmax_stride, const int *forced_tile,
                    hipStream_t stream) {
    P2P_REQUIRE((unsigned long long)d0 * d1 * d2 * d3 < (1ull << 31), P2P_EUNSUPPORTED,
                "consensus volume %d x %d x %d x %d has 2^31 cells or more", d0, d1, d2, d3);
    NcFusedArgs a{};
    a.X = X; a.Y = Y; a.Y2 = Y2; a.stride = stride; a.d0 = d0; a.d1 = d1; a.d2 = d2; a.d3 = d3; a.w = w_dev; a.b2 = b2;
    a.xmax = xmax; a.xmax_stride = xmax_stride;
    nc_fused_tile(a, pairs, forced_tile);
    const size_t lds = nc_fused_lds_bytes(a.tb, a.tc, a.P);
    P2P_REQUIRE(a.P <= 64 && lds <= NCF_LDS_MAX && a.tc + 4 <= 12 && (a.tc + 2) * a.P <= 512, P2P_EUNSUPPORTED,
                "consensus tile does not fit (P %d, tc %d, LDS %zu)", a.P, a.tc, lds);
    static DeviceOnce attr_set;
    const int dev = raise_lds_limit(attr_set, {{(const void *)nc_fused_kernel<0>, (int)NCF_LDS_MAX}, {(const void *)nc_fused_kernel<5>, (int)NCF_LDS_MAX},
                                               {(const void *)nc_fused_kernel<10>, (int)NCF_LDS_MAX}});
    if (dev < 0) return dev;
    const dim3 grid(a.na * a.nb * a.nc * a.nd, 1, pairs);
    const bool fixed = a.tc == 8 && a.td == 40 && a.P == 44;
    if (fixed && a.tb == 10)
        hipLaunchKernelGGL(nc_fused_kernel<10>, grid, dim3(NCF_THREADS), lds, stream, a);
    else if (fixed && a.tb == 5)
        hipLaunchKernelGGL(nc_fused_kernel<5>, grid, dim3(NCF_THREADS), lds, stream, a);
    else
        hipLaunchKernelGGL(nc_fused_kernel<0>, grid, dim3(NCF_THREADS), lds, stream, a);
    return check_launch("nc_fused_kernel");
}

}
```

patch2pix_amd/csrc/matches.hip:

```cpp
#pragma once
#include "coarse_common.h"

namespace p2p {

__device__ __forceinline__ MatchArgs match_args_of_pair(MatchArgs m, size_t z) {
    m.X += z * m.sX;
    if (m.delta) m.delta += z * m.sX;
    m.matches += z * m.sM * 4;
    m.scores += z * m.sM;
    return m;
}

template <bool RECIP>
__device__ __forceinline__ void emit_match_as(const MatchArgs &m, int out_row, int ra, int cb, float s) {
    int ia = ra / m.wA, ja = ra - ia * m.wA, ib = cb / m.wB, jb = cb - ib * m.wB;
    if (m.ksize > 1 && m.delta) {
        const int k = m.ksize;
        int code = m.delta[(size_t)ra * (m.hB * m.wB) + cb];
        const int dl = code % k; code /= k;
        const int dk = code % k; code /= k;
        const int dj = code % k; code /= k;
        ia = ia * k + code; ja = ja * k + dj; ib = ib * k + dk; jb = jb * k + dl;
    } else if (m.ksize > 1) {
        ia *= m.ksize; ja *= m.ksize; ib *= m.ksize; jb *= m.ksize;
    }
    const long long up = m.upsample, off = m.center ? m.upsample / 2 : 0;
    long long *o = m.matches + (size_t)out_row * 4;
    o[0] = up * ja + off; o[1] = up * ia + off; o[2] = up * jb + off; o[3] = up * ib + off;
    m.scores[out_row] = RECIP ? 1.0f / s : s;
}
__device__ __forceinline__ void emit_match(const MatchArgs &m, int out_row, int ra, int cb, float sum_exp) { emit_match_as<true>(m, out_row, ra, cb, sum_exp); }

template <bool ONE>
__device__ __forceinline__ bool match_candidate(float v, int i, float pv, int pi) {
    if constexpr (ONE) return true;
    else return v < pv || (v == pv && i > pi);
}

constexpr int MC_COLS = 16, MC_SLICES = 16;
template <bool ONE>
__device__ __forceinline__ void match_cols_scan(const MatchArgs &m_, int topk, int do_softmax) {
    const MatchArgs m = match_args_of_pair(m_, blockIdx.z);
    __shared__ float smax[MC_SLICES][MC_COLS];
    __shared__ int sarg[MC_SLICES][MC_COLS];
    __shared__ float ssum[MC_SLICES][MC_COLS];
    const int nA = m.hA * m.wA, nB = m.hB * m.wB;
    const int cs = threadIdx.x & (MC_COLS - 1), rs = threadIdx.x / MC_COLS;
    const int col = blockIdx.x * MC_COLS + cs;
    const bool ok = col < nB;
    float pv = INFINITY, top = 0.f, total = 1.f;
    int pi = -1;
    for (int t = 0; ONE || t < topk; ++t) {
        float best = -INFINITY;
        int arg = 0x7fffffff;
        if (ok)
            for (int r = rs; r < nA; r += MC_SLICES) {
                const float v = m.X[(size_t)r * nB + col];
                if (match_candidate<ONE>(v, r, pv, pi) && v > best) { best = v; arg = r; }
            }
        smax[rs][cs] = best; sarg[rs][cs] = arg;
        __syncthreads();
        float gb = smax[0][cs];
        int ga = sarg[0][cs];
#pragma unroll
        for (int s = 1; s < MC_SLICES; ++s) {
            const float v = smax[s][cs];
            const int a = sarg[s][cs];
            if (v > gb || (v == gb && a < ga)) { gb = v; ga = a; }
        }
        bool softmax = true;
        if constexpr (!ONE) softmax = do_softmax;
        if (t == 0) {
            top = gb;
            if (softmax) {
                float sum = 0.f;
                if (ok)
                    for (int r = rs; r < nA; r += MC_SLICES) sum += expf(m.X[(size_t)r * nB + col] - gb);
                ssum[rs][cs] = sum;
                __syncthreads();
                if (rs == 0 && ok) {
                    total = 0.f;
#pragma unroll
                    for (int s = 0; s < MC_SLICES; ++s) total += ssum[s][cs];
                }
            }
        }
        if constexpr (ONE) {
            if (rs == 0 && ok) emit_match(m, col, ga, col, total);
            return;
        } else {
            ga = min(ga, nA - 1);
            if (rs == 0 && ok)
                emit_match_as<false>(m, t * nB + col, ga, col, softmax ? (t == 0 ? 1.0f : expf(gb - top)) / total : gb);
            pv = gb; pi = ga;
            __syncthreads();
        }
    }
}
__global__ __launch_bounds__(256) void match_cols_kernel(MatchArgs m) { match_cols_scan<true>(m, 1, 1); }
__global__ __launch_bounds__(256) void match_cols_topk_kernel(MatchArgs m, int topk, int do_softmax) { match_cols_scan<false>(m, topk, do_softmax); }

template <bool ONE>
__device__ __forceinline__ void match_rows_scan(const MatchArgs &m_, int topk, int do_softmax) {
    const MatchArgs m = match_args_of_pair(m_, blockIdx.z);
    const int nA = m.hA * m.wA, nB = m.hB * m.wB;
    const int row = blockIdx.x * 4 + (threadIdx.x >> 6);
    const int lane = threadIdx.x & 63;
    if (row >= nA) return;
    const float *x = m.X + (size_t)row * nB;
    float pv = INFINITY, top = 0.f, total = 1.f;
    int pi = -1;
    for (int t = 0; ONE || t < topk; ++t) {
        float best = -INFINITY;
        int arg = 0x7fffffff;
        for (int c = lane; c < nB; c += 64) {
            const float v = x[c];
            if (match_candidate<ONE>(v, c, pv, pi) && v > best) { best = v; arg = c; }
        }
#pragma unroll
        for (int s = 32; s >= 1; s >>= 1) {
            const float ov = __shfl_xor(best, s);
            const int oa = __shfl_xor(arg, s);
            if (ov > best || (ov == best && oa < arg)) { best = ov; arg = oa; }
        }
        bool softmax = true;
        if constexpr (!ONE) softmax = do_softmax;
        if (t == 0) {
            top = best;
            if (softmax) {
                float sum = 0.f;
                for (int c = lane; c < nB; c += 64) sum += expf(x[c] - best);
#pragma unroll
                for (int s = 32; s >= 1; s >>= 1) sum += __shfl_xor(sum, s);
                total = sum;
            }
        }
        if constexpr (ONE) {
            if (lane == 0) emit_match(m, nB + row, row, arg, total);
            return;
        } else {
            arg = min(arg, nB - 1);
            if (lane == 0)
                emit_match_as<false>(m, topk * nB + row * topk + t, row, arg, softmax ? (t == 0 ? 1.0f : expf(best - top)) / total : best);
            pv = best; pi = arg;
        }
    }
}
__global__ __launch_bounds__(256) void match_rows_kernel(MatchArgs m) { match_rows_scan<true>(m, 1, 1); }
__global__ __launch_bounds__(256) void match_rows_topk_kernel(MatchArgs m, int topk, int do_softmax) { match_rows_scan<false>(m, topk, do_softmax); }

void launch_matches(const MatchArgs &m, int batch, hipStream_t stream) {
    hipLaunchKernelGGL(match_cols_kernel, dim3(ceil_div(m.hB * m.wB, MC_COLS), 1, batch), dim3(256), 0, stream, m);
    hipLaunchKernelGGL(match_rows_kernel, dim3(ceil_div(m.hA * m.wA, 4), 1, batch), dim3(256), 0, stream, m);
}

void launch_matches_topk(const MatchArgs &m, int batch, int topk, int do_softmax, hipStream_t stream) {
    hipLaunchKernelGGL(match_cols_topk_kernel, dim3(ceil_div(m.hB * m.wB, MC_COLS), 1, batch), dim3(256), 0, stream, m, topk, do_softmax);
    hipLaunchKernelGGL(match_rows_topk_kernel, dim3(ceil_div(m.hA * m.wA, 4), 1, batch), dim3(256), 0, stream, m, topk, do_softmax);
}

__global__ void delta_unpack_kernel(const uint8_t *__restrict__ delta, size_t n, int k, long long *__restrict__ out) {
    const size_t i = (size_t)blockIdx.x * blockDim.x + threadIdx.x;
    if (i >= n) return;
    int s = delta[i];
    out[3 * n + i] = s % k; s /= k;
    out[2 * n + i] = s % k; s /= k;
    out[1 * n + i] = s % k; s /= k;
    out[i] = s;
}

void launch_delta_unpack(const uint8_t *delta, size_t n, int k, long long *out, hipStream_t stream) {
    hipLaunchKernelGGL(delta_unpack_kernel, dim3((unsigned)((n + 255) / 256)), dim3(256), 0, stream, delta, n, k, out);
}

}
```

patch2pix_amd/networks/patch2pix.py:

```python
import numpy as np
import torch
import torch.nn as nn

from . import resnet
from .utils import filter_coarse
from .. import ops, staging


class _Holder(nn.Module):

    def __init__(self, spec):
        super().__init__()
        children = {}
        for name, (shape, kind) in spec.items():
            head, _, rest = name.partition(".")
            if rest:
                children.setdefault(head, {})[rest] = (shape, kind)
            elif kind == "param":
                self.register_parameter(head, nn.Parameter(torch.zeros(shape), requires_grad=False))
            else:
                dtype = torch.int64 if kind == "long" else torch.float32
                self.register_buffer(head, torch.zeros(shape, dtype=dtype))
        for head, sub in children.items():
            self.add_module(head, _Holder(sub))


def _bn_spec(prefix, n):
    return {f"{prefix}.weight": ((n,), "param"), f"{prefix}.bias": ((n,), "param"),
            f"{prefix}.running_mean": ((n,), "buffer"), f"{prefix}.running_var": ((n,), "buffer"),
            f"{prefix}.num_batches_tracked": ((), "long")}


def _regressor_spec(layout):
    shapes, bns = ops.regressor_shapes(layout)
    spec = {k: (shp, "param") for k, shp in shapes.items()}
    for prefix, n in bns.items():
        spec.update(_bn_spec(prefix, n))
    return spec


def _ncn_spec(layout):
    return {k: (shp, "param") for k, shp in ops.ncn_shapes(layout).items()}


def _ncn_layout_of(config):
    nc = getattr(config, "ncn_config", None)
    if nc is not None:
        return ops.ncn_layout(nc)
    wd = getattr(config, "weights_dict", None) or {}
    sub = {k[len("ncn."):]: v for k, v in wd.items() if k.startswith("ncn.conv.")}
    return ops.ncn_layout(sub if sub else None)


_NCN_SPEC = _ncn_spec(ops.RELEASED_NCN_LAYOUT)


class Delta4d:

    def __init__(self, packed, ksize):
        self.packed = packed
        self.ksize = ksize
        self._planes = None

    def _materialise(self):
        if self._planes is None:
            planes = ops.delta_unpack(self.packed, self.ksize)
            self._planes = tuple(p.unsqueeze(1) for p in planes)
        return self._planes

    def __iter__(self):
        return iter(self._materialise())

    def __len__(self):
        return 4

    def __getitem__(self, i):
        return self._materialise()[i]


class Patch2Pix(nn.Module):
    def __init__(self, config):
        super().__init__()
        self.device = torch.device(config.device)
        if self.device.type != "cuda":
            raise RuntimeError("patch2pix_amd runs the matching path on an MI355X; no CPU fallback exists "
                               f"(config.device={config.device})")
        if getattr(config, "training", False):
            raise NotImplementedError("training is out of scope of the MI355X matching path")
        self.backbone = config.backbone
        if self.backbone != "ResNet34":
            raise NotImplementedError(f"backbone {self.backbone}: only ResNet34 (the released model) is provided")
        self.change_stride = config.change_stride
        self.upsample = 16
        self.feats_downsample = [1, 2, 2, 2, 2]
        feat_dims = [3, 64, 64, 128, 256]
        self.extract = resnet.ResNet34()
        if self.change_stride:
            self.extract.change_stride(target="layer3")
            self.upsample //= 2
            self.feats_downsample[-1] = 1
        else:
            raise NotImplementedError("change_stride=False (upsample 16) is not implemented by the HIP fine stage")
        self._ncn_layout = _ncn_layout_of(config)
        self.ncn = _Holder(_ncn_spec(self._ncn_layout))

        self.regressor_config = config.regressor_config
        self.regress_mid = None
        self.regress_fine = None
        if self.regressor_config:
            rc = self.regressor_config
            self.regr_batch = config.regr_batch
            self.feat_idx = list(config.feat_idx)
            self._layout = ops.regressor_layout(rc, self.feat_idx)
            rc.feat_dim = sum(feat_dims[i] for i in self.feat_idx)
            self.ptype = ["center", "center"]
            self.psize = rc.psize
            self.pshift = rc.pshift
            self.panc = rc.panc
            self.shared = rc.shared
            self.regress_mid = _Holder(_regressor_spec(self._layout))
            self.regress_fine = self.regress_mid if self.shared else _Holder(_regressor_spec(self._layout))
        self.to(self.device)
        self._packed = None
        self._ticket_ring = staging.PinnedRing(4)
        self.init_weights_(weights_dict=config.weights_dict)
        self.eval()

    def init_weights_(self, weights_dict=None, pretrained=True):
        if weights_dict:
            own = self.state_dict()
            picked = {k: v for k, v in weights_dict.items() if k in own}
            missing = [k for k in own if k not in picked and not k.endswith("num_batches_tracked")]
            if missing and any(not k.startswith("extract.") for k in missing) and any(
                    k.startswith(("ncn.", "regress_")) for k in weights_dict):
                raise KeyError(f"checkpoint lacks hot-path weights: {missing[:5]} ...")
            self.load_state_dict(picked, strict=False)
            if not any(k.startswith(("ncn.", "regress_")) for k in picked):
                import warnings
                warnings.warn("Patch2Pix: the checkpoint holds none of the ncn.* / regress_* weights; the matching path keeps "
                              "its initial (zero) parameters and its matches are meaningless", RuntimeWarning)
        self._packed = None

    def load_state_dict(self, *args, **kwargs):
        self._packed = None
        return super().load_state_dict(*args, **kwargs)

    def _weights(self):
        if self._packed is None:
            sd = self.state_dict()
            ncn = ops.NcnWeights.from_state_dict({k[len("ncn."):]: v for k, v in sd.items() if k.startswith("ncn.")}, self.device,
                                                 symmetric_mode=self._ncn_layout["symmetric_mode"])
            mid = fine = None
            if self.regress_mid is not None:
                sub = lambda p: {k[len(p):]: v for k, v in sd.items() if k.startswith(p)}
                mid = ops.RegressorWeights(sub("regress_mid."), self.device, self.regressor_config, self.feat_idx)
                fine = mid if self.shared else ops.RegressorWeights(sub("regress_fine."), self.device,
                                                                    self.regressor_config, self.feat_idx)
            self._packed = (ncn, mid, fine)
        return self._packed

    def forward_coarse_match(self, feat1, feat2, ksize=1):
        ncn = self._weights()[0]
        b, _, h1, w1 = feat1.shape
        _, _, h2, w2 = feat2.shape
        k = max(ksize, 1)
        shape = (b, 1, h1 // k, w1 // k, h2 // k, w2 // k)
        corr4d = torch.empty(shape, dtype=torch.float32, device=feat1.device)
        packed = torch.empty(shape, dtype=torch.uint8, device=feat1.device) if ksize > 1 else None
        ops.coarse_forward_batch(feat1, feat2, ksize, ncn, out_corr=corr4d[:, 0],
                                 out_delta=packed[:, 0] if packed is not None else None)
        delta4d = Delta4d(packed[:, 0], ksize) if ksize > 1 else None
        return corr4d, delta4d

    def forward(self, im1, im2, ksize=1, return_feats=False):
        feat1s, feat2s = self._pyramids(im1, im2)
        feat1, feat2 = feat1s[-1], feat2s[-1]
        corr4d, delta4d = self.forward_coarse_match(feat1, feat2, ksize=ksize)
        if return_feats:
            return corr4d, delta4d, feat1s, feat2s
        return corr4d, delta4d

    def _packed_delta(self, delta4d, ksize):
        if delta4d is not None and not isinstance(delta4d, Delta4d):
            di, dj, dk, dl = delta4d
            s = ((di * ksize + dj) * ksize + dk) * ksize + dl
            delta4d = Delta4d(s[:, 0].to(torch.uint8).contiguous(), ksize)
        return delta4d.packed if delta4d is not None else None

    def cal_coarse_matches(self, corr4d, delta4d, ksize=1, do_softmax=True, upsample=16, sort=False,
                           center=True, pshift=0):
        packed = self._packed_delta(delta4d, ksize)
        if do_softmax:
            matches_, score_ = ops.coarse_matches_batch(corr4d[:, 0], packed, ksize, upsample, center)
        else:
            matches_, score_ = ops.coarse_matches_topk_batch(corr4d[:, 0], packed, ksize, upsample, center, 1, False)
        if sort:
            order = torch.sort(-score_)[1]
            score_ = torch.gather(score_, 1, order)
            matches_ = torch.gather(matches_, 1, order.unsqueeze(-1).expand(-1, -1, 4))
        return matches_, score_

    def cal_coarse_matches_topk(self, corr4d, delta4d, topk, ksize=1, do_softmax=True, upsample=16, center=True):
        return ops.coarse_matches_topk_batch(corr4d[:, 0], self._packed_delta(delta4d, ksize), ksize, upsample, center,
                                             topk, do_softmax)

    def cal_coarse_score(self, corr4d, normalize='softmax'):
        return ops.coarse_score_batch(corr4d[:, 0], normalize).mean()

    def score_from_feats(self, feats1, feats2, ksize=2, normalize='softmax'):
        ops.score_norm(normalize)
        corr4d, _ = self.forward_coarse_match(feats1[-1], feats2[-1], ksize=ksize)
        return ops.coarse_score_batch(corr4d[:, 0], normalize)

    def predict_score(self, im1, im2, ksize=2, normalize='softmax'):
        ops.score_norm(normalize)
        feats1, feats2 = self._pyramids(im1, im2)
        return self.score_from_feats(feats1, feats2, ksize, normalize)

    def shift_to_anchors(self, matches):
        if self.panc == 1:
            return matches
        s = self.pshift
        tmpl = torch.tensor([[-s, -s, 0, 0], [s, -s, 0, 0], [-s, s, 0, 0], [s, s, 0, 0],
                             [0, 0, -s, -s], [0, 0, s, -s], [0, 0, -s, s], [0, 0, s, s]], device=self.device)
        return [(m.unsqueeze(1) + tmpl).reshape(-1, 4) for m in matches]

    def forward_fine_match(self, feats1, feats2, coarse_matches, psize=16, ptype="center", regressor=None):
        _, mid_w, fine_w = self._weights()
        w = fine_w if (regressor is self.regress_fine and regressor is not self.regress_mid) else mid_w
        nb = len(coarse_matches)
        outs = ops.regress_batch(w, None, [[f[b] for f in feats1[:4]] for b in range(nb)],
                                 [[f[b] for f in feats2[:4]] for b in range(nb)],
                                 [self._as_proposals(p) for p in coarse_matches])
        return [o["matches1"] for o in outs], [o["probs1"] for o in outs]

    def _as_proposals(self, props):
        props = props.to(self.device)
        if props.dtype not in (torch.int64, torch.float32):
            props = props.float() if props.is_floating_point() else props.long()
        return props

    def _fine_chain(self, feats1, feats2, coarse_matches):
        _, mid_w, fine_w = self._weights()
        nb = len(coarse_matches)
        outs = ops.regress_batch(mid_w, fine_w, [[f[b] for f in feats1[:4]] for b in range(nb)],
                                 [[f[b] for f in feats2[:4]] for b in range(nb)],
                                 [self._as_proposals(p) for p in coarse_matches])
        return ([o["matches2"] for o in outs], [o["probs2"] for o in outs],
                [o["matches1"] for o in outs], [o["probs1"] for o in outs])

    def predict_coarse(self, im1, im2, ksize=2, ncn_thres=0.0, mutual=False, center=True):
        corr4d, delta4d = self.forward(im1, im2, ksize)
        coarse_matches, match_scores = self.cal_coarse_matches(corr4d, delta4d, ksize=ksize,
                                                               upsample=self.upsample, center=center)
        return filter_coarse(coarse_matches, match_scores, ncn_thres, mutual)

    def predict_coarse_topk(self, im1, im2, topk, ksize=2, ncn_thres=0.0, mutual=False, center=True):
        corr4d, delta4d = self.forward(im1, im2, ksize)
        coarse_matches, match_scores = self.cal_coarse_matches_topk(corr4d, delta4d, topk, ksize=ksize,
                                                                    upsample=self.upsample, center=center)
        return filter_coarse(coarse_matches, match_scores, ncn_thres, mutual)

    def predict_fine_topk(self, im1, im2, topk, ksize=2, ncn_thres=0.0, mutual=True, return_all=False):
        feats1, feats2 = self._pyramids(im1, im2)
        corr4d, delta4d = self.forward_coarse_match(feats1[-1], feats2[-1], ksize=ksize)
        matches_, score_ = self.cal_coarse_matches_topk(corr4d, delta4d, topk, ksize=ksize, upsample=self.upsample,
                                                        center=True)
        coarse_matches, _ = filter_coarse(matches_, score_, ncn_thres, mutual)
        coarse_matches = self.shift_to_anchors(coarse_matches)
        fine, fine_scores, mid, mid_scores = self._fine_chain(feats1, feats2, coarse_matches)
        if return_all:
            return fine, fine_scores, mid, mid_scores, coarse_matches
        return fine, fine_scores, coarse_matches

    def coarse_async(self, feats1, feats2, ksize=2):
        corr4d, delta4d = self.forward_coarse_match(feats1[-1], feats2[-1], ksize=ksize)
        matches_, score_ = self.cal_coarse_matches(corr4d, delta4d, ksize=ksize, upsample=self.upsample, center=True)
        return dict(feats1=feats1, feats2=feats2, matches=matches_, scores=score_,
                    staged=staging.readback([matches_, score_], self._ticket_ring))

    def fine_from_ticket(self, ticket, ncn_thres=0.0, mutual=True, return_all=False, ptmax=None):
        host = ticket["staged"].wait()
        coarse_matches, match_scores = filter_coarse(ticket["matches"], ticket["scores"], ncn_thres, mutual, ptmax=ptmax,
                                                     host_copy=None if host is None else (host[0].numpy(), host[1].numpy()))
        coarse_matches = self.shift_to_anchors(coarse_matches)
        fine, fine_scores, mid, mid_scores = self._fine_chain(ticket["feats1"], ticket["feats2"], coarse_matches)
        if return_all:
            return fine, fine_scores, mid, mid_scores, coarse_matches
        return fine, fine_scores, coarse_matches

    def predict_fine_device(self, feats1, feats2, ksize=2, ncn_thres=0.0, mutual=True):
        if self.panc != 1:
            raise NotImplementedError("predict_fine_device: panc > 1 goes through predict_fine_from_feats")
        if max(feats1[0].shape[-2:] + feats2[0].shape[-2:]) >= (1 << 15):
            raise NotImplementedError("predict_fine_device: image sides must be below 32768 pixels")
        _, mid_w, fine_w = self._weights()
        corr4d, delta4d = self.forward_coarse_match(feats1[4], feats2[4], ksize=ksize)
        matches_, score_ = self.cal_coarse_matches(corr4d, delta4d, ksize=ksize, upsample=self.upsample, center=True)
        coarse, _, counts = ops.filter_coarse_batch(matches_, score_, ncn_thres, mutual)
        nb = coarse.shape[0]
        out = ops.regress_batch_dev(mid_w, fine_w, [[f[b] for f in feats1[:4]] for b in range(nb)],
                                    [[f[b] for f in feats2[:4]] for b in range(nb)], coarse, counts)
        return out["matches2"], out["probs2"], coarse, counts

    @staticmethod
    def unpad(fine, fine_scores, coarse, counts):
        n = counts.cpu().tolist()
        if any(c < 0 for c in n):
            raise RuntimeError("Patch2Pix.unpad: the device-side filter_coarse asked for the host path (count -1: a "
                               "coordinate outside [0, 2^15)); call predict_fine_from_feats / estimate_matches instead")
        return ([fine[b, :c] for b, c in enumerate(n)], [fine_scores[b, :c] for b, c in enumerate(n)],
                [coarse[b, :c] for b, c in enumerate(n)])

    def predict_fine_from_feats(self, feats1, feats2, ksize=2, ncn_thres=0.0, mutual=True, return_all=False,
                                ptmax=None):
        ticket = self.coarse_async(feats1, feats2, ksize)
        return self.fine_from_ticket(ticket, ncn_thres, mutual, return_all, ptmax)

    def _pyramids(self, im1, im2):
        return resnet.pair_pyramids(self.extract, im1, im2)

    def predict_fine(self, im1, im2, ksize=2, ncn_thres=0.0, mutual=True, return_all=False):
        feats1, feats2 = self._pyramids(im1, im2)
        return self.predict_fine_from_feats(feats1, feats2, ksize, ncn_thres, mutual, return_all)

    def refine_matches(self, im1, im2, coarse_matches, io_thres):
        if len(coarse_matches) == 0:
            return np.empty((0, 4)), np.empty((0,)), np.empty((0, 4))
        if isinstance(coarse_matches, np.ndarray):
            coarse_t = torch.from_numpy(coarse_matches).to(self.device)
        else:
            coarse_t = coarse_matches.to(self.device)
            coarse_matches = coarse_matches.cpu().data.numpy()
        feats1, feats2 = self._pyramids(im1, im2)
        fine, fine_scores, _, _ = self._fine_chain(feats1, feats2, [coarse_t])
        refined = fine[0].cpu().data.numpy()
        scores = fine_scores[0].cpu().data.numpy()
        if io_thres > 0:
            pos = np.where(scores > io_thres)[0]
            if len(pos) > 0:
                coarse_matches, refined, scores = coarse_matches[pos], refined[pos], scores[pos]
        return refined, scores, coarse_matches
```

patch2pix_amd/ops.py:

```python
import ctypes
import math
import os

import numpy as np
import torch

from . import _lib, staging


def _stream():
    return ctypes.c_void_p(torch.cuda.current_stream().cuda_stream)


def _f32c(t, name):
    if t.dtype != torch.float32 or not t.is_cuda:
        raise TypeError(f"{name} must be a float32 tensor on the GPU (got {t.dtype}, {t.device})")
    return t.contiguous()


def _host(t):
    return t.detach().to("cpu", torch.float32).contiguous()


RELEASED_NCN_LAYOUT = dict(kernel_sizes=[3, 3], channels=[16, 1], symmetric_mode=True)
NCN_MAX_LAYERS, NCN_KERNEL_SIZES, NCN_MAX_CHANNELS = 4, (3, 5), 16


def ncn_layout(source=None, symmetric_mode=None):
    if source is None:
        lay = {k: (list(v) if isinstance(v, list) else v) for k, v in RELEASED_NCN_LAYOUT.items()}
    elif isinstance(source, dict) and any(str(k).startswith("conv.") for k in source):
        ks, ch, cin, i = [], [], 1, 0
        while f"conv.{2 * i}.weight" in source:
            shp = tuple(source[f"conv.{2 * i}.weight"].shape)
            if len(shp) != 6 or len({shp[0], shp[3], shp[4], shp[5]}) != 1:
                raise ValueError(f"conv.{2 * i}.weight has shape {shp}: expected the stored layout [k, c_out, c_in, k, k, k]")
            if shp[2] != cin:
                raise ValueError(f"conv.{2 * i}.weight has {shp[2]} input channels where the layer below it gives {cin}")
            bias = source.get(f"conv.{2 * i}.bias")
            if bias is None or tuple(bias.shape) != (shp[1],):
                raise ValueError(f"conv.{2 * i}.bias is missing or is not of shape ({shp[1]},)")
            ks.append(int(shp[0])); ch.append(int(shp[1])); cin = shp[1]; i += 1
        if not ks:
            raise ValueError("no conv.0.weight among the consensus tensors")
        lay = dict(kernel_sizes=ks, channels=ch, symmetric_mode=True)
    else:
        get = (lambda k, d=None: source.get(k, d)) if isinstance(source, dict) else (lambda k, d=None: getattr(source, k, d))
        ks, ch = get("kernel_sizes"), get("channels")
        if ks is None or ch is None:
            raise ValueError("a consensus configuration needs kernel_sizes and channels")
        lay = dict(kernel_sizes=[int(k) for k in ks], channels=[int(c) for c in ch], symmetric_mode=bool(get("symmetric_mode", True)))
    if symmetric_mode is not None:
        lay["symmetric_mode"] = bool(symmetric_mode)
    ks, ch = lay["kernel_sizes"], lay["channels"]
    if not ks or len(ks) != len(ch):
        raise ValueError(f"kernel_sizes {ks} and channels {ch} must be non-empty lists of one length")
    if any(k <= 0 for k in ks) or any(c <= 0 for c in ch):
        raise ValueError(f"kernel_sizes {ks} / channels {ch}: sizes must be positive")
    if len(ks) > NCN_MAX_LAYERS:
        raise NotImplementedError(f"kernel_sizes {ks}: at most {NCN_MAX_LAYERS} consensus layers are implemented")
    if any(k not in NCN_KERNEL_SIZES for k in ks):
        raise NotImplementedError(f"kernel_sizes {ks}: kernel sizes 3 and 5 are implemented")
    if any(c > NCN_MAX_CHANNELS for c in ch):
        raise NotImplementedError(f"channels {ch}: at most {NCN_MAX_CHANNELS} channels per layer are implemented")
    if ch[-1] != 1:
        raise NotImplementedError(f"channels {ch}: the last layer must have one channel (the volume is [B,1,...] downstream)")
    return lay


def ncn_shapes(lay):
    shapes, cin = {}, 1
    for i, (k, c) in enumerate(zip(lay["kernel_sizes"], lay["channels"])):
        shapes[f"conv.{2 * i}.weight"], shapes[f"conv.{2 * i}.bias"] = (k, c, cin, k, k, k), (c,)
        cin = c
    return shapes


class NcnWeights:

    layout, generic = RELEASED_NCN_LAYOUT, False

    def __init__(self, w1, b1, w2, b2, device):
        keep = [_host(w1), _host(b1), _host(w2), _host(b2)]
        if tuple(keep[0].shape) != (3, 16, 1, 3, 3, 3) or tuple(keep[2].shape) != (3, 1, 16, 3, 3, 3):
            raise NotImplementedError("only NeighConsensus(kernel_sizes=[3,3], channels=[16,1]) is implemented")
        self.handle = ctypes.c_void_p()
        with torch.cuda.device(device):
            _lib.check(_lib.p2p_ncn_create(*[t.data_ptr() for t in keep], ctypes.byref(self.handle)), "p2p_ncn_create")
        self.device = torch.device(device)

    @classmethod
    def from_state_dict(cls, sd, device, symmetric_mode=True, generic=False):
        lay = ncn_layout({k: v for k, v in sd.items() if k.startswith("conv.")}, symmetric_mode)
        if not generic and lay == RELEASED_NCN_LAYOUT:
            return cls(sd["conv.0.weight"], sd["conv.0.bias"], sd["conv.2.weight"], sd["conv.2.bias"], device)
        n = len(lay["kernel_sizes"])
        keep = [(_host(sd[f"conv.{2 * i}.weight"]), _host(sd[f"conv.{2 * i}.bias"])) for i in range(n)]
        c, t = _lib.NcnConfig(), _lib.NcnTensors()
        c.n_layers, c.symmetric = n, int(lay["symmetric_mode"])
        for i in range(n):
            c.kernel_size[i], c.channels[i] = lay["kernel_sizes"][i], lay["channels"][i]
            t.w[i], t.b[i] = keep[i][0].data_ptr(), keep[i][1].data_ptr()
        self = cls.__new__(cls)
        self.handle = ctypes.c_void_p()
        with torch.cuda.device(device):
            _lib.check(_lib.p2p_ncn_create_config(ctypes.byref(c), ctypes.byref(t), ctypes.byref(self.handle)), "p2p_ncn_create_config")
        self.device, self.layout, self.generic = torch.device(device), lay, True
        return self

    def set_tile(self, ta=0, tb=0, tc=0):
        if self.generic:
            raise NotImplementedError("set_tile: a generic consensus handle has no work-group tile to force")
        _lib.check(_lib.p2p_ncn_set_tile(self.handle, int(ta), int(tb), int(tc)), "p2p_ncn_set_tile")

    def __del__(self):
        if getattr(self, "handle", None) and _lib is not None:
            _lib.p2p_ncn_destroy(self.handle)
            self.handle = None


def _parse_conv_tile(text):
    try:
        t = tuple(int(v) for v in text.split(","))
    except ValueError:
        t = ()
    if len(t) != 3 or min(t) < 0:
        raise ValueError(f"P2P_CONV_TILE={text!r}: expected three non-negative integers 'mt,nt,wn'")
    return t


FORCED_CONV_TILE = _parse_conv_tile(os.environ["P2P_CONV_TILE"]) if os.environ.get("P2P_CONV_TILE") else None


class ConvBN:

    def __init__(self, conv_weight, bn_weight, bn_bias, bn_mean, bn_var, stride, device):
        keep = [_host(t) for t in (conv_weight, bn_weight, bn_bias, bn_mean, bn_var)]
        co, ci, ks, ks2 = keep[0].shape
        if ks != ks2:
            raise NotImplementedError("square kernels only")
        bn = _lib.BnParams(*[t.data_ptr() for t in keep[1:]])
        self.handle = ctypes.c_void_p()
        with torch.cuda.device(device):
            _lib.check(_lib.p2p_conv_create(keep[0].data_ptr(), ctypes.byref(bn), ci, co, ks, int(stride), ctypes.byref(self.handle)),
                       "p2p_conv_create")
        self.ci, self.co, self.ks, self.stride = ci, co, ks, int(stride)
        self.device = torch.device(device)
        self._tile = None

    def __del__(self):
        if getattr(self, "handle", None) and _lib is not None:
            _lib.p2p_conv_destroy(self.handle)
            self.handle = None

    def forward(self, x, xmax, residual=None, relu=True, ymax=None):
        n, h, w, ci = x.shape
        if ci != self.ci or x.dtype != torch.float32 or not x.is_cuda or not x.is_contiguous():
            raise TypeError(f"ConvBN.forward: expected a contiguous float32 NHWC tensor with {self.ci} channels on the GPU")
        if FORCED_CONV_TILE != self._tile:
            _lib.check(_lib.p2p_conv_set_tile(self.handle, *(FORCED_CONV_TILE or (0, 0, 0))), "p2p_conv_set_tile")
            self._tile = FORCED_CONV_TILE
        pad = self.ks // 2
        ho, wo = (h + 2 * pad - self.ks) // self.stride + 1, (w + 2 * pad - self.ks) // self.stride + 1
        y = torch.empty((n, ho, wo, self.co), device=x.device, dtype=torch.float32)
        if residual is not None and (residual.shape != y.shape or not residual.is_contiguous()):
            raise TypeError("ConvBN.forward: residual must be a contiguous NHWC tensor of the output's shape")
        _lib.check(_lib.p2p_conv_forward(self.handle, x.data_ptr(), xmax.data_ptr(), n, h, w,
                                         residual.data_ptr() if residual is not None else None, int(relu), y.data_ptr(),
                                         ymax.data_ptr() if ymax is not None else None, _stream()), "p2p_conv_forward")
        return y


class Stem:

    def __init__(self, conv_weight, bn_weight, bn_bias, bn_mean, bn_var, device):
        keep = [_host(t) for t in (conv_weight, bn_weight, bn_bias, bn_mean, bn_var)]
        if tuple(keep[0].shape) != (64, 3, 7, 7):
            raise NotImplementedError("only the ResNet stem Conv2d(3, 64, 7, 2, 3) is implemented")
        bn = _lib.BnParams(*[t.data_ptr() for t in keep[1:]])
        self.handle = ctypes.c_void_p()
        with torch.cuda.device(device):
            _lib.check(_lib.p2p_stem_create(keep[0].data_ptr(), ctypes.byref(bn), ctypes.byref(self.handle)), "p2p_stem_create")
        self.device = torch.device(device)

    def __del__(self):
        if getattr(self, "handle", None) and _lib is not None:
            _lib.p2p_stem_destroy(self.handle)
            self.handle = None

    def forward(self, image):
        image = _f32c(image, "image")
        n, c, h, w = image.shape
        if c != 3:
            raise TypeError("Stem.forward: three-channel images only")
        imax = absmax_batch(image)
        y = torch.empty((n, 64, (h - 1) // 2 + 1, (w - 1) // 2 + 1), device=image.device, dtype=torch.float32)
        _lib.check(_lib.p2p_stem_forward(self.handle, image.data_ptr(), imax.data_ptr(), n, h, w, y.data_ptr(), _stream()), "p2p_stem_forward")
        return y


def maxpool_nhwc(x, ymax=None):
    x = _f32c(x, "x")
    n, c, h, w = x.shape
    y = torch.empty((n, (h - 1) // 2 + 1, (w - 1) // 2 + 1, c), device=x.device, dtype=torch.float32)
    _lib.check(_lib.p2p_maxpool_nhwc(x.data_ptr(), n, c, h, w, y.data_ptr(), ymax.data_ptr() if ymax is not None else None, _stream()),
               "p2p_maxpool_nhwc")
    return y


def nhwc_to_nchw(x):
    x = _f32c(x, "x")
    n, h, w, c = x.shape
    y = torch.empty((n, c, h, w), device=x.device, dtype=torch.float32)
    _lib.check(_lib.p2p_nhwc_to_nchw(x.data_ptr(), n, h, w, c, y.data_ptr(), _stream()), "p2p_nhwc_to_nchw")
    return y


def absmax_batch(x):
    x = _f32c(x, "x")
    out = torch.empty((x.shape[0],), device=x.device, dtype=torch.int32)
    _lib.check(_lib.p2p_absmax_batch(x.data_ptr(), x[0].numel(), x.shape[0], out.data_ptr(), _stream()), "p2p_absmax_batch")
    return out


FEAT_DIMS = (3, 64, 64, 128, 256)
RELEASED_LAYOUT = dict(feat_idx=[0, 1, 2, 3], feat_comb="pre", conv_dims=[512, 512], conv_kers=[3, 3], conv_strs=[2, 1],
                       fc_dims=[512, 256], psize=[16, 16])


def regressor_layout(config=None, feat_idx=None):
    get = (lambda k, d=None: config.get(k, d)) if isinstance(config, dict) else (lambda k, d=None: getattr(config, k, d))
    lay = {k: (list(v) if isinstance(v, list) else v) for k, v in RELEASED_LAYOUT.items()}
    if feat_idx is not None:
        lay["feat_idx"] = [int(i) for i in feat_idx]
    if config is not None:
        lay["feat_comb"] = get("feat_comb", "pre")
        lay["conv_dims"] = [int(d) for d in get("conv_dims")]
        lay["conv_kers"] = [int(k) for k in get("conv_kers")]
        strs = get("conv_strs")
        lay["conv_strs"] = [int(v) for v in strs] if strs is not None else [2] * len(lay["conv_kers"])
        lay["fc_dims"] = [int(d) for d in get("fc_dims")]
        ps = get("psize", [16, 16])
        lay["psize"] = [int(v) for v in ps] if isinstance(ps, (list, tuple)) else [int(ps), int(ps)]
    fi = lay["feat_idx"]
    if not fi or any(b <= a for a, b in zip(fi, fi[1:])) or any(i < 0 or i > 4 for i in fi):
        raise ValueError(f"feat_idx {fi}: a non-empty, strictly ascending list of pyramid levels")
    if 4 in fi:
        raise NotImplementedError(f"feat_idx {fi}: level 4 is not implemented by the fine stage (the pyramid handed to the "
                                  "library carries levels 0..3)")
    if lay["psize"] != [16, 16]:
        raise NotImplementedError(f"psize {lay['psize']}: psize must be [16,16]")
    if lay["feat_comb"] not in ("pre", "post"):
        raise ValueError(f"feat_comb {lay['feat_comb']!r}: 'pre' or 'post'")
    nc = len(lay["conv_dims"])
    if nc == 0 or len(lay["conv_kers"]) != nc or len(lay["conv_strs"]) != nc:
        raise ValueError("conv_dims, conv_kers and conv_strs must be non-empty lists of one length")
    if nc > 4 or len(lay["fc_dims"]) > 4:
        raise NotImplementedError("at most 4 convolutions and 4 hidden FC layers are implemented")
    for what in ("conv_dims", "fc_dims"):
        for d in lay[what]:
            if d <= 0:
                raise ValueError(f"{what} {lay[what]}: dims must be positive")
            if d % 16 or d > 1024:
                raise NotImplementedError(f"{what} {lay[what]}: dims must be multiples of 16 in [16, 1024]")
    side = 16
    for k, st in zip(lay["conv_kers"], lay["conv_strs"]):
        if k not in (1, 3, 5):
            raise NotImplementedError(f"conv_kers {lay['conv_kers']}: kernel sizes 1, 3 and 5 are implemented")
        if st not in (1, 2):
            raise NotImplementedError(f"conv_strs {lay['conv_strs']}: strides 1 and 2 are implemented")
        if side + 2 - k < 0:
            raise ValueError(f"conv_kers {lay['conv_kers']} / conv_strs {lay['conv_strs']}: the map shrinks below 1x1")
        side = (side + 2 - k) // st + 1
    return lay


def regressor_shapes(lay):
    feat_dim = sum(FEAT_DIMS[i] for i in lay["feat_idx"])
    cin = feat_dim if lay["feat_comb"] == "post" else 2 * feat_dim
    shapes, bns = {}, {}
    for i, (d, k) in enumerate(zip(lay["conv_dims"], lay["conv_kers"])):
        shapes[f"conv.{2 * i}.weight"] = (d, cin, k, k)
        bns[f"conv.{2 * i + 1}"] = d
        cin = d
    k = lay["conv_dims"][-1] * (2 if lay["feat_comb"] == "post" else 1)
    for i, d in enumerate(lay["fc_dims"]):
        shapes[f"fc.{3 * i}.weight"], shapes[f"fc.{3 * i}.bias"] = (d, k), (d,)
        bns[f"fc.{3 * i + 1}"] = d
        k = d
    n = 3 * len(lay["fc_dims"])
    shapes[f"fc.{n}.weight"], shapes[f"fc.{n}.bias"] = (5, k), (5,)
    return shapes, bns


class RegressorWeights:

    def __init__(self, sd, device, config=None, feat_idx=None, generic=False):
        lay = regressor_layout(config, feat_idx)
        self.layout = lay
        self.generic = bool(generic) or lay != RELEASED_LAYOUT
        self.device = torch.device(device)
        if self.generic:
            self._create_generic(sd, lay)
            return
        exp = {"conv.0.weight": (512, 518, 3, 3), "conv.2.weight": (512, 512, 3, 3), "fc.0.weight": (512, 512),
               "fc.3.weight": (256, 512), "fc.6.weight": (5, 256)}
        for k, shp in exp.items():
            if tuple(sd[k].shape) != shp:
                raise NotImplementedError(f"regressor {k} has shape {tuple(sd[k].shape)}; only the released "
                                          f"configuration {shp} is implemented")
        keep = {k: _host(v) for k, v in sd.items() if v.is_floating_point()}
        p = _lib.RegressorParams()

        def bn(prefix):
            return _lib.BnParams(keep[prefix + ".weight"].data_ptr(), keep[prefix + ".bias"].data_ptr(),
                                 keep[prefix + ".running_mean"].data_ptr(), keep[prefix + ".running_var"].data_ptr())

        p.conv1_w = keep["conv.0.weight"].data_ptr(); p.bn1 = bn("conv.1")
        p.conv2_w = keep["conv.2.weight"].data_ptr(); p.bn2 = bn("conv.3")
        p.fc1_w = keep["fc.0.weight"].data_ptr(); p.fc1_b = keep["fc.0.bias"].data_ptr(); p.bnf1 = bn("fc.1")
        p.fc2_w = keep["fc.3.weight"].data_ptr(); p.fc2_b = keep["fc.3.bias"].data_ptr(); p.bnf2 = bn("fc.4")
        p.fc3_w = keep["fc.6.weight"].data_ptr(); p.fc3_b = keep["fc.6.bias"].data_ptr()
        self.handle = ctypes.c_void_p()
        with torch.cuda.device(device):
            _lib.check(_lib.p2p_regressor_create(ctypes.byref(p), ctypes.byref(self.handle)), "p2p_regressor_create")
        env = os.environ.get("P2P_REGRESS_MODE")
        if env:
            self.set_mode(env)

    def _create_generic(self, sd, lay):
        shapes, bns = regressor_shapes(lay)
        for k, shp in shapes.items():
            if k not in sd or tuple(sd[k].shape) != shp:
                got = tuple(sd[k].shape) if k in sd else "no tensor"
                raise ValueError(f"regressor {k}: the configuration asks for shape {shp}, the state_dict has {got}")
        keep = {k: _host(v) for k, v in sd.items() if v.is_floating_point()}

        def bn(prefix):
            return _lib.BnParams(keep[prefix + ".weight"].data_ptr(), keep[prefix + ".bias"].data_ptr(),
                                 keep[prefix + ".running_mean"].data_ptr(), keep[prefix + ".running_var"].data_ptr())

        c, t = _lib.RegressorConfig(), _lib.RegressorTensors()
        c.n_feat = len(lay["feat_idx"])
        for i, j in enumerate(lay["feat_idx"]):
            c.feat_idx[i] = j
        c.feat_comb = _lib.FEAT_COMB[lay["feat_comb"]]
        c.n_conv, c.n_fc, c.psize = len(lay["conv_dims"]), len(lay["fc_dims"]), lay["psize"][0]
        for i in range(c.n_conv):
            c.conv_dim[i], c.conv_ker[i], c.conv_str[i] = lay["conv_dims"][i], lay["conv_kers"][i], lay["conv_strs"][i]
            t.conv_w[i] = keep[f"conv.{2 * i}.weight"].data_ptr()
            t.conv_bn[i] = bn(f"conv.{2 * i + 1}")
        for i in range(c.n_fc):
            c.fc_dim[i] = lay["fc_dims"][i]
            t.fc_w[i], t.fc_b[i] = keep[f"fc.{3 * i}.weight"].data_ptr(), keep[f"fc.{3 * i}.bias"].data_ptr()
            t.fc_bn[i] = bn(f"fc.{3 * i + 1}")
        t.out_w, t.out_b = keep[f"fc.{3 * c.n_fc}.weight"].data_ptr(), keep[f"fc.{3 * c.n_fc}.bias"].data_ptr()
        self.handle = ctypes.c_void_p()
        with torch.cuda.device(self.device):
            _lib.check(_lib.p2p_regressor_create_config(ctypes.byref(c), ctypes.byref(t), ctypes.byref(self.handle)),
                       "p2p_regressor_create_config")

    def set_mode(self, mode):
        if self.generic:
            if mode == "generic":
                return
            raise NotImplementedError(f"regressor mode {mode!r}: a generic regressor runs the exact-fp32 generic kernels only")
        if mode not in _lib.REGRESS_MODES:
            removed = {"bf16x2": "round 5", "bf16x3": "round 4"}
            why = f" ({mode!r} was removed in {removed[mode]})" if mode in removed else ""
            raise ValueError(f"unknown regressor mode {mode!r}{why}: one of {sorted(_lib.REGRESS_MODES)}")
        with torch.cuda.device(self.device):
            _lib.check(_lib.p2p_regressor_set_mode(self.handle, _lib.REGRESS_MODES[mode]), "p2p_regressor_set_mode")

    @property
    def mode(self):
        code = _lib.p2p_regressor_get_mode(self.handle)
        return "generic" if code == _lib.REGRESS_GENERIC else {v: k for k, v in _lib.REGRESS_MODES.items()}[code]

    def __del__(self):
        if getattr(self, "handle", None) and _lib is not None:
            _lib.p2p_regressor_destroy(self.handle)
            self.handle = None


_workspaces = {}

regress_events = None


def _workspace(device, nbytes):
    key = (device.index, torch.cuda.current_stream(device).cuda_stream)
    ws = _workspaces.get(key)
    if ws is None or ws.numel() < nbytes:
        ws = torch.empty(nbytes, dtype=torch.uint8, device=device)
        _workspaces[key] = ws
    return ws


COARSE_WORKSPACE_LIMIT = 16 << 30


def coarse_forward_batch(feat_a, feat_b, ksize, ncn, want_delta=True, out_corr=None, out_delta=None):
    feat_a, feat_b = _f32c(feat_a, "feat_a"), _f32c(feat_b, "feat_b")
    if feat_a.dim() != 4 or feat_b.dim() != 4 or feat_a.shape[0] != feat_b.shape[0]:
        raise ValueError("coarse_forward_batch expects [B,C,h,w] feature maps with equal B")
    nb, c, ha, wa = feat_a.shape
    _, c2, hb, wb = feat_b.shape
    if c != c2:
        raise ValueError("channel mismatch between the two feature maps")
    dev = feat_a.device
    k = max(ksize, 1)
    shape = (nb, ha // k, wa // k, hb // k, wb // k)
    corr = out_corr if out_corr is not None else torch.empty(shape, dtype=torch.float32, device=dev)
    delta = None
    if ksize > 1 and want_delta:
        delta = out_delta if out_delta is not None else torch.empty(shape, dtype=torch.uint8, device=dev)
    assert corr.is_contiguous() and corr.numel() == math.prod(shape) and corr.dtype == torch.float32
    assert delta is None or (delta.is_contiguous() and delta.numel() == math.prod(shape) and delta.dtype == torch.uint8)
    if nb == 0:
        return corr, delta
    with torch.cuda.device(dev):
        per_pair = _lib.p2p_coarse_workspace_bytes_for(ncn.handle, c, ha, wa, hb, wb, ksize)
        if per_pair == 0:
            raise ValueError("coarse_forward: bad sizes")
        pairs = max(1, min(nb, COARSE_WORKSPACE_LIMIT // per_pair))
        ws = _workspace(dev, pairs * per_pair)
        _lib.check(_lib.p2p_coarse_forward_batch(feat_a.data_ptr(), feat_b.data_ptr(), nb, c, ha, wa, hb, wb, ksize,
                                                 ncn.handle, corr.data_ptr(),
                                                 delta.data_ptr() if delta is not None else None,
                                                 ws.data_ptr(), ws.numel(), _stream()), "p2p_coarse_forward_batch")
    return corr, delta


def coarse_forward(feat_a, feat_b, ksize, ncn, want_delta=True, out_corr=None, out_delta=None):
    corr, delta = coarse_forward_batch(feat_a[None], feat_b[None], ksize, ncn, want_delta,
                                       out_corr[None] if out_corr is not None else None,
                                       out_delta[None] if out_delta is not None else None)
    return corr[0], (delta[0] if delta is not None else None)


def neigh_consensus_batch(x, ncn):
    x = _f32c(x, "x")
    if x.dim() != 5:
        raise ValueError("neigh_consensus_batch expects [B,hA,wA,hB,wB]")
    nb, ha, wa, hb, wb = x.shape
    y = torch.empty_like(x)
    if nb == 0 or x.numel() == 0:
        return y
    with torch.cuda.device(x.device):
        per = _lib.p2p_neigh_consensus_workspace_bytes(ncn.handle, ha, wa, hb, wb)
        nbytes = per * max(1, min(nb, COARSE_WORKSPACE_LIMIT // per))
        ws = torch.empty(nbytes, dtype=torch.uint8, device=x.device)
        _lib.check(_lib.p2p_neigh_consensus_batch(x.data_ptr(), nb, ha, wa, hb, wb, ncn.handle, y.data_ptr(), ws.data_ptr(), nbytes,
                                                  _stream()), "p2p_neigh_consensus_batch")
    return y


def delta_unpack(delta, ksize):
    out = torch.empty((4,) + tuple(delta.shape), dtype=torch.int64, device=delta.device)
    if delta.numel() == 0:
        return out[0], out[1], out[2], out[3]
    with torch.cuda.device(delta.device):
        _lib.check(_lib.p2p_delta_unpack(delta.data_ptr(), delta.numel(), ksize, out.data_ptr(), _stream()),
                   "p2p_delta_unpack")
    return out[0], out[1], out[2], out[3]


def coarse_matches_batch(corr, delta, ksize, upsample, center=True, out_matches=None, out_scores=None):
    corr = _f32c(corr, "corr4d")
    if corr.dim() != 5:
        raise ValueError("coarse_matches_batch expects corr4d of shape [B,hA,wA,hB,wB]")
    nb, ha, wa, hb, wb = corr.shape
    n = ha * wa + hb * wb
    dev = corr.device
    matches = out_matches if out_matches is not None else torch.empty((nb, n, 4), dtype=torch.int64, device=dev)
    scores = out_scores if out_scores is not None else torch.empty((nb, n), dtype=torch.float32, device=dev)
    assert matches.is_contiguous() and matches.numel() == nb * n * 4 and matches.dtype == torch.int64
    assert scores.is_contiguous() and scores.numel() == nb * n and scores.dtype == torch.float32
    if delta is not None:
        delta = delta.contiguous()
        if delta.dtype != torch.uint8 or delta.numel() != corr.numel():
            raise ValueError("delta must be the packed uint8 volume with the shape of corr4d")
    if nb == 0:
        return matches, scores
    with torch.cuda.device(dev):
        _lib.check(_lib.p2p_coarse_matches_batch(corr.data_ptr(), delta.data_ptr() if delta is not None else None, nb,
                                                 ha, wa, hb, wb, ksize, upsample, int(bool(center)),
                                                 matches.data_ptr(), scores.data_ptr(), _stream()),
                   "p2p_coarse_matches_batch")
    return matches, scores


def coarse_matches(corr, delta, ksize, upsample, center=True, out_matches=None, out_scores=None):
    m, sc = coarse_matches_batch(corr[None], delta[None] if delta is not None else None, ksize, upsample, center,
                                 out_matches[None] if out_matches is not None else None,
                                 out_scores[None] if out_scores is not None else None)
    return m[0], sc[0]


def coarse_matches_topk_batch(corr, delta, ksize, upsample, center, topk, do_softmax=True):
    corr = _f32c(corr, "corr4d")
    if corr.dim() != 5:
        raise ValueError("coarse_matches_topk_batch expects corr4d of shape [B,hA,wA,hB,wB]")
    nb, ha, wa, hb, wb = corr.shape
    topk = int(topk)
    n = max(topk, 0) * (ha * wa + hb * wb)
    dev = corr.device
    matches = torch.empty((nb, n, 4), dtype=torch.int64, device=dev)
    scores = torch.empty((nb, n), dtype=torch.float32, device=dev)
    if delta is not None:
        delta = delta.contiguous()
        if delta.dtype != torch.uint8 or delta.numel() != corr.numel():
            raise ValueError("delta must be the packed uint8 volume with the shape of corr4d")
    if nb == 0:
        return matches, scores
    with torch.cuda.device(dev):
        _lib.check(_lib.p2p_coarse_matches_topk_batch(corr.data_ptr(), delta.data_ptr() if delta is not None else None, nb,
                                                      ha, wa, hb, wb, ksize, upsample, int(bool(center)), topk,
                                                      int(bool(do_softmax)), matches.data_ptr(), scores.data_ptr(), _stream()),
                   "p2p_coarse_matches_topk_batch")
    return matches, scores


def score_norm(normalize):
    if normalize is not None and not isinstance(normalize, str) or normalize not in _lib.SCORE_NORMS:
        raise ValueError(f"normalize must be None, 'softmax' or 'l1', got {normalize!r}")
    return _lib.SCORE_NORMS[normalize]


def coarse_score_batch(corr, normalize="softmax", return_cells=False):
    norm = score_norm(normalize)
    corr = _f32c(corr, "corr4d")
    if corr.dim() != 5:
        raise ValueError("coarse_score_batch expects corr4d of shape [B,hA,wA,hB,wB]")
    nb, ha, wa, hb, wb = corr.shape
    dev = corr.device
    pair = torch.empty((nb,), dtype=torch.float32, device=dev)
    cells = torch.empty((nb, ha * wa + hb * wb), dtype=torch.float32, device=dev)
    if nb:
        with torch.cuda.device(dev):
            _lib.check(_lib.p2p_coarse_score_batch(corr.data_ptr(), nb, ha, wa, hb, wb, norm, cells.data_ptr(), pair.data_ptr(),
                                                   None, 0, _stream()), "p2p_coarse_score_batch")
    return (pair, cells) if return_cells else pair


def filter_coarse_batch(matches, scores, ncn_thres=0.0, mutual=True):
    if matches.dtype != torch.int64 or matches.dim() != 3 or matches.shape[-1] != 4 or not matches.is_cuda:
        raise TypeError("matches must be an int64 [B,n,4] tensor on the GPU")
    scores = _f32c(scores, "scores")
    matches = matches.contiguous()
    nb, n, _ = matches.shape
    dev = matches.device
    out_m, out_s = torch.empty_like(matches), torch.empty_like(scores)
    counts = torch.empty((nb,), dtype=torch.int32, device=dev)
    if nb and n:
        with torch.cuda.device(dev):
            need = _lib.p2p_filter_coarse_workspace_bytes(nb, n)
            ws = torch.empty(need, dtype=torch.uint8, device=dev) if need else None
            _lib.check(_lib.p2p_filter_coarse_batch(matches.data_ptr(), scores.data_ptr(), nb, n, float(ncn_thres),
                                                    int(bool(mutual)), out_m.data_ptr(), out_s.data_ptr(),
                                                    counts.data_ptr(), ws.data_ptr() if need else None, need, _stream()),
                       "p2p_filter_coarse_batch")
    else:
        counts.zero_()
    return out_m, out_s, counts


_small_ring = staging.PinnedRing(8)


def small_to_device(array, dtype, device):
    return staging.upload([torch.as_tensor(array, dtype=dtype)], device, _small_ring)[0]


def match_tail_batch(fine, scores, coarse, counts, scale, io_thres):
    if fine.dtype != torch.float32 or coarse.dtype != torch.int64 or counts.dtype != torch.int32 or not fine.is_cuda:
        raise TypeError("match_tail_batch: fine fp32, coarse int64, counts int32 on the GPU expected")
    fine, scores, coarse = fine.contiguous(), _f32c(scores, "scores"), coarse.contiguous()
    nb, n, _ = fine.shape
    dev = fine.device
    scale = scale.to(torch.float64).reshape(nb, 4) if torch.is_tensor(scale) and scale.is_cuda else \
        small_to_device(torch.as_tensor(scale, dtype=torch.float64).reshape(nb, 4), torch.float64, dev)
    out_m = torch.empty((nb, n, 4), dtype=torch.float64, device=dev)
    out_c = torch.empty((nb, n, 4), dtype=torch.float64, device=dev)
    out_s = torch.empty((nb, n), dtype=torch.float32, device=dev)
    out_n = torch.empty((nb,), dtype=torch.int32, device=dev)
    if nb and n:
        with torch.cuda.device(dev):
            _lib.check(_lib.p2p_match_tail_batch(fine.data_ptr(), scores.data_ptr(), coarse.data_ptr(), counts.data_ptr(),
                                                 scale.data_ptr(), nb, n, float(io_thres), out_m.data_ptr(), out_s.data_ptr(),
                                                 out_c.data_ptr(), out_n.data_ptr(), _stream()), "p2p_match_tail_batch")
    else:
        out_n.zero_()
    return out_m, out_s, out_c, out_n


EPI_BINS_MEASURE = [0, 1e-2, 1, 5, 10, 25, 50, 100, 400, 2500, 1e5]
EPI_BINS_EVAL = [0, 1e-2, 1, 5, 10, 25, 50, 100, 2500, 1e5]


def epi_kind(kind):
    if not isinstance(kind, str) or kind not in _lib.EPI_KINDS:
        raise ValueError(f"kind must be one of {sorted(_lib.EPI_KINDS)}, got {kind!r}")
    return _lib.EPI_KINDS[kind]


def epi_edges(bins):
    edges = np.asarray(bins, dtype=np.float64)
    if edges.ndim != 1 or edges.size < 2:
        raise ValueError(f"bins must be a one-dimensional sequence of at least two edges, got shape {edges.shape}")
    if np.isnan(edges).any() or bool((np.diff(edges) < 0).any()):
        raise ValueError("bins must increase monotonically and hold no NaN")
    if edges.size - 1 > _lib.EPI_MAX_BINS:
        raise NotImplementedError(f"{edges.size - 1} bins: at most {_lib.EPI_MAX_BINS} are implemented")
    return edges


def epipolar_batch(matches, counts, F, kind="sampson", eps=1e-8, bins=None, out_dtype=None):
    code = epi_kind(kind)
    eps = float(eps)
    if not eps >= 0.0:
        raise ValueError(f"eps must be >= 0, got {eps!r}")
    edges = epi_edges(bins) if bins is not None else None
    if not torch.is_tensor(matches) or matches.dim() != 3 or matches.shape[-1] != 4:
        raise ValueError("matches must be a [B,n,4] tensor")
    nb, n, _ = matches.shape
    F = torch.as_tensor(F)
    if tuple(F.shape) == (3, 3) and nb == 1:
        F = F[None]
    if tuple(F.shape) != (nb, 3, 3):
        raise ValueError(f"F must have shape [{nb},3,3] (or [3,3] for one item), got {tuple(F.shape)}")
    out_dtype = torch.float64 if out_dtype is None else out_dtype
    if out_dtype not in (torch.float64, torch.float32):
        raise ValueError(f"out_dtype must be torch.float64 or torch.float32, got {out_dtype}")
    if counts is not None and (not torch.is_tensor(counts) or counts.numel() != nb):
        raise ValueError(f"counts must be an int32 tensor of {nb} values or None")
    name = str(matches.dtype).replace("torch.", "")
    if name not in _lib.DTYPES or not matches.is_cuda:
        raise TypeError(f"matches must be a float64, float32 or int64 tensor on the GPU (got {matches.dtype}, {matches.device})")
    if counts is not None and (counts.dtype != torch.int32 or counts.device != matches.device):
        raise TypeError("counts must be an int32 tensor on the device of matches")
    dev = matches.device
    matches = matches.contiguous()
    dist = torch.zeros((nb, n), dtype=out_dtype, device=dev)
    hist = torch.zeros((nb, len(edges) - 1), dtype=torch.int32, device=dev) if edges is not None else None
    if nb == 0 or n == 0:
        return dist, hist
    if nb > 65535:
        raise ValueError(f"epipolar_batch: {nb} items (at most 65535 per call)")
    with torch.cuda.device(dev):
        if F.is_cuda:
            Fd = F.to(dev, torch.float64).contiguous()
            dedges = small_to_device(edges, torch.float64, dev) if edges is not None else None
        else:
            parts = [F.to(torch.float64).contiguous()] + ([torch.from_numpy(edges)] if edges is not None else [])
            up = staging.upload(parts, dev, _small_ring)
            Fd, dedges = up[0], (up[1] if edges is not None else None)
        if counts is None:
            counts = torch.full((nb,), n, dtype=torch.int32, device=dev)
        counts = counts.contiguous()
        _lib.check(_lib.p2p_epipolar_batch(matches.data_ptr(), _lib.DTYPES[name], counts.data_ptr(), Fd.data_ptr(), nb, n,
                                           code, eps, dedges.data_ptr() if edges is not None else None,
                                           len(edges) - 1 if edges is not None else 0, dist.data_ptr(),
                                           _lib.DTYPES[str(out_dtype).replace("torch.", "")],
                                           hist.data_ptr() if hist is not None else None, _stream()), "p2p_epipolar_batch")
    return dist, hist


def regress_batch_dev(reg1, reg2, pyrs1, pyrs2, proposals, counts, want_raw=False, out=None):
    nb, stride, _ = proposals.shape
    dev = proposals.device
    if proposals.dtype not in (torch.int64, torch.float32):
        raise TypeError("proposals must be int64 or float32")
    if counts.dtype != torch.int32 or counts.numel() != nb or not counts.is_cuda:
        raise TypeError("counts must be an int32 [B] tensor on the GPU")
    proposals = proposals.contiguous()
    pyr_a, pyr_b, keep = (_lib.Pyramid * nb)(), (_lib.Pyramid * nb)(), []
    for i in range(nb):
        pa, ka = _pyramid(pyrs1[i])
        pb, kb = _pyramid(pyrs2[i])
        pyr_a[i], pyr_b[i] = pa, pb
        keep.append((ka, kb))
    given = out or {}
    two = reg2 is not None
    out = {"matches1": torch.empty((nb, stride, 4), device=dev), "probs1": torch.empty((nb, stride), device=dev)}
    if two:
        out["matches2"], out["probs2"] = torch.empty((nb, stride, 4), device=dev), torch.empty((nb, stride), device=dev)
    if want_raw:
        out["raw1"] = torch.empty((nb, stride, 5), device=dev)
        if two:
            out["raw2"] = torch.empty((nb, stride, 5), device=dev)
    for k in out:
        if k in given:
            if given[k].shape != out[k].shape or given[k].dtype != torch.float32 or not given[k].is_contiguous() or given[k].device != dev:
                raise ValueError(f"out[{k!r}] must be a contiguous float32 tensor of shape {tuple(out[k].shape)} on {dev}")
            out[k] = given[k]
    g = lambda k: out[k].data_ptr() if k in out else None
    if nb and stride:
        with torch.cuda.device(dev):
            ws = _regress_scratch(dev, nb * stride, reg1)
            _lib.check(_lib.p2p_regress_batch_dev(reg1.handle, reg2.handle if two else None, nb, pyr_a, pyr_b,
                                                  counts.data_ptr(), stride, proposals.data_ptr(),
                                                  int(proposals.is_floating_point()), g("matches1"), g("probs1"), g("raw1"),
                                                  g("matches2"), g("probs2"), g("raw2"), ws.data_ptr(), ws.numel(), _stream()),
                       "p2p_regress_batch_dev")
    del keep
    return out


generic_scratch_limit = None


def _regress_scratch(dev, n, reg=None):
    if reg is None:
        nbytes = _lib.p2p_regress_workspace_bytes(int(n))
    else:
        nbytes = _lib.p2p_regress_workspace_bytes_for(reg.handle, int(n))
        if generic_scratch_limit is not None and getattr(reg, "generic", False):
            nbytes = min(nbytes, int(generic_scratch_limit))
    return torch.empty(max(int(nbytes), 128), dtype=torch.uint8, device=dev)


def _pyramid(levels):
    if len(levels) != 4:
        raise ValueError("a pyramid is the 4 maps of feat_idx [0,1,2,3]")
    lv = [_f32c(t, "pyramid level") for t in levels]
    h, w = lv[0].shape[-2:]
    if h < 8 or w < 8:
        raise ValueError(f"images must be at least 8x8 pixels (got {h}x{w})")
    up = lambda d, j: (d + (1 << j) - 1) >> j
    exp = [(3, h, w), (64, up(h, 1), up(w, 1)), (64, up(h, 2), up(w, 2)), (128, up(h, 3), up(w, 3))]
    for t, e in zip(lv, exp):
        if tuple(t.shape) != e:
            raise ValueError(f"pyramid level has shape {tuple(t.shape)}, expected {e}")
    p = _lib.Pyramid()
    for j in range(4):
        p.level[j] = lv[j].data_ptr()
    p.height, p.width = h, w
    return p, lv


def regress_batch(reg1, reg2, pyrs1, pyrs2, proposals, want_mid=True, want_raw=False):
    nitems = len(proposals)
    if nitems == 0:
        return []
    dev = proposals[0].device
    dtype = proposals[0].dtype
    if dtype == torch.int64:
        is_float = 0
    elif dtype == torch.float32:
        is_float = 1
    else:
        raise TypeError("proposals must be int64 or float32")
    if any(p.dtype != dtype for p in proposals):
        raise TypeError("all proposal arrays of a batch must share one dtype")
    counts = [int(p.shape[0]) for p in proposals]
    n = sum(counts)
    allp = proposals[0].contiguous() if nitems == 1 else torch.cat([p.reshape(-1, 4) for p in proposals])
    pyr_a = (_lib.Pyramid * nitems)()
    pyr_b = (_lib.Pyramid * nitems)()
    keep = []
    for i in range(nitems):
        pa, ka = _pyramid(pyrs1[i])
        pb, kb = _pyramid(pyrs2[i])
        pyr_a[i], pyr_b[i] = pa, pb
        keep.append((ka, kb))
    cnt = (ctypes.c_int * nitems)(*counts)
    bufs = {}

    def buf(key, cols, cond=True):
        if not cond:
            return None
        bufs[key] = torch.empty((n, cols) if cols > 1 else (n,), dtype=torch.float32, device=dev)
        return bufs[key].data_ptr()

    two = reg2 is not None
    m1 = buf("matches1", 4, want_mid or not two)
    q1 = buf("probs1", 1, want_mid or not two)
    r1 = buf("raw1", 5, want_raw)
    m2 = buf("matches2", 4, two)
    q2 = buf("probs2", 1, two)
    r2 = buf("raw2", 5, two and want_raw)
    if n:
        with torch.cuda.device(dev):
            ws = _regress_scratch(dev, n, reg1)
            ev = None
            if regress_events is not None:
                ev = (torch.cuda.Event(enable_timing=True), torch.cuda.Event(enable_timing=True))
                ev[0].record()
            _lib.check(_lib.p2p_regress_batch(reg1.handle, reg2.handle if two else None, nitems, pyr_a, pyr_b, cnt,
                                              allp.data_ptr(), is_float, m1, q1, r1, m2, q2, r2, ws.data_ptr(), ws.numel(),
                                              _stream()), "p2p_regress_batch")
            if ev is not None:
                ev[1].record()
                regress_events.append((ev[0], ev[1], n, 2 if two else 1))
    del keep
    outs, start = [], 0
    for c in counts:
        outs.append({k: v[start:start + c] for k, v in bufs.items()})
        start += c
    return outs


def regress(reg1, reg2, pyr1, pyr2, proposals, want_mid=True, want_raw=False):
    return regress_batch(reg1, reg2, [pyr1], [pyr2], [proposals], want_mid, want_raw)[0]


def _op_input(t, name, dim=None):
    if not isinstance(t, torch.Tensor):
        raise TypeError(f"{name} must be a tensor")
    if not t.is_cuda:
        raise RuntimeError(f"{name} must be on the GPU (got {t.device}): the operators have no CPU path")
    if t.dtype != torch.float32:
        raise TypeError(f"{name} must be float32 (got {t.dtype})")
    if t.requires_grad and torch.is_grad_enabled():
        raise NotImplementedError(f"{name} requires grad: the operators are inference only (wrap the call in torch.no_grad())")
    if dim is not None and t.dim() != dim:
        raise ValueError(f"{name} must have {dim} dimensions (got {tuple(t.shape)})")
    return t.detach().contiguous()


def correlation_batch(feat_a, feat_b):
    feat_a, feat_b = _op_input(feat_a, "feat1", 4), _op_input(feat_b, "feat2", 4)
    if feat_a.shape[:2] != feat_b.shape[:2] or feat_a.device != feat_b.device:
        raise ValueError(f"feature maps {tuple(feat_a.shape)} and {tuple(feat_b.shape)} must agree in batch, channels and device")
    nb, c, ha, wa = feat_a.shape
    hb, wb = feat_b.shape[2:]
    out = torch.empty((nb, ha * wa, hb * wb), dtype=torch.float32, device=feat_a.device)
    if out.numel() == 0:
        return out
    with torch.cuda.device(feat_a.device):
        _lib.check(_lib.p2p_correlation_batch(feat_a.data_ptr(), feat_b.data_ptr(), nb, c, ha, wa, hb, wb, out.data_ptr(), _stream()),
                   "p2p_correlation_batch")
    return out


def maxpool4d_batch(x, k, want_delta=True):
    x = _op_input(x, "corr4d_hres", 5)
    nb, h1, w1, h2, w2 = x.shape
    k = int(k)
    shape = (nb, h1 // k, w1 // k, h2 // k, w2 // k) if k > 0 else (nb, 0, 0, 0, 0)
    pooled = torch.empty(shape, dtype=torch.float32, device=x.device)
    delta = torch.empty(shape, dtype=torch.uint8, device=x.device) if want_delta else None
    if x.numel() == 0 and k > 0:
        return pooled, delta
    with torch.cuda.device(x.device):
        _lib.check(_lib.p2p_maxpool4d_batch(x.data_ptr(), nb, h1, w1, h2, w2, k, pooled.data_ptr(),
                                            delta.data_ptr() if want_delta else None, _stream()), "p2p_maxpool4d_batch")
    return pooled, delta


def mutual_matching_batch(x):
    x = _op_input(x, "corr4d", 5)
    nb, ha, wa, hb, wb = x.shape
    y = torch.empty_like(x)
    if x.numel() == 0:
        return y
    with torch.cuda.device(x.device):
        nbytes = _lib.p2p_mutual_matching_workspace_bytes(nb, ha, wa, hb, wb)
        ws = torch.empty(max(nbytes, 4), dtype=torch.uint8, device=x.device)
        _lib.check(_lib.p2p_mutual_matching_batch(x.data_ptr(), nb, ha, wa, hb, wb, y.data_ptr(), ws.data_ptr(), nbytes, _stream()),
                   "p2p_mutual_matching_batch")
    return y


def l2_normalize(x, dim):
    x = _op_input(x, "feat")
    dim = dim % x.dim()
    outer, c, inner = math.prod(x.shape[:dim]), x.shape[dim], math.prod(x.shape[dim + 1:])
    y = torch.empty_like(x)
    if x.numel() == 0:
        return y
    with torch.cuda.device(x.device):
        _lib.check(_lib.p2p_l2_normalize(x.data_ptr(), outer, c, inner, y.data_ptr(), _stream()), "p2p_l2_normalize")
    return y


class Conv4dWeights:

    def __init__(self, weight, bias, device):
        w = _host(weight)
        if w.dim() != 6 or len({w.shape[0], w.shape[3], w.shape[4], w.shape[5]}) != 1:
            raise ValueError(f"Conv4d weight has shape {tuple(w.shape)}: expected the stored layout [k, c_out, c_in, k, k, k]")
        b = _host(bias) if bias is not None else None
        if b is not None and tuple(b.shape) != (w.shape[1],):
            raise ValueError(f"Conv4d bias has shape {tuple(b.shape)}: expected ({w.shape[1]},)")
        self.c_in, self.c_out, self.k = int(w.shape[2]), int(w.shape[1]), int(w.shape[0])
        self.handle = ctypes.c_void_p()
        with torch.cuda.device(device):
            _lib.check(_lib.p2p_conv4d_create(w.data_ptr(), b.data_ptr() if b is not None else None, self.c_in, self.c_out, self.k,
                                              ctypes.byref(self.handle)), "p2p_conv4d_create")
        self.device = torch.device(device)

    def __del__(self):
        if getattr(self, "handle", None) and _lib is not None:
            _lib.p2p_conv4d_destroy(self.handle)
            self.handle = None


def conv4d_forward_batch(x, conv):
    x = _op_input(x, "data", 6)
    nb, c, h1, w1, h2, w2 = x.shape
    if c != conv.c_in:
        raise ValueError(f"data has {c} channels, the layer takes {conv.c_in}")
    y = torch.empty((nb, conv.c_out, h1, w1, h2, w2), dtype=torch.float32, device=x.device)
    if y.numel() == 0:
        return y
    with torch.cuda.device(x.device):
        _lib.check(_lib.p2p_conv4d_forward_batch(conv.handle, x.data_ptr(), nb, h1, w1, h2, w2, y.data_ptr(), _stream()),
                   "p2p_conv4d_forward_batch")
    return y


def tensor_signature(tensors):
    return tuple((id(t), t._version, t.data_ptr(), tuple(t.shape), str(t.device)) for t in tensors)
```

Baseline: 947.5.

## Fuse second mutual-matching pass into consensus epilogue and matcher

Adds a combined coarse-forward-plus-matches entry point. The fused neighbourhood-consensus kernel now writes the merged (symmetric) output directly and reduces row and column maxima into key buffers with atomics. The matcher applies the mutual-matching normalisation on the fly from those keys instead of materialising the normalised 4D correlation. This removes the separate second maxima pass, the mm_apply pass and the full corr4d round trip through HBM. It also drops the Y2 split-buffer path and the memset of the output, at the cost of extra atomics and per-element recompute in the match kernels.

```diff
diff --git a/include/p2p_hip.h b/include/p2p_hip.h
--- a/include/p2p_hip.h
+++ b/include/p2p_hip.h
@@ -101,6 +101,11 @@
                              int ksize, int upsample, int center, int64_t *matches_out, float *scores_out,
                              p2p_stream_t stream);
 
+int p2p_coarse_forward_matches_batch(const float *featA, const float *featB, int batch, int channels, int hA, int wA, int hB,
+                                     int wB, int ksize, const p2p_ncn *ncn, uint8_t *delta_out, int upsample, int center,
+                                     int64_t *matches_out, float *scores_out, void *workspace, size_t workspace_bytes,
+                                     p2p_stream_t stream);
+
 int p2p_coarse_matches_topk_batch(const float *corr4d, const uint8_t *delta, int batch, int hA, int wA, int hB, int wB,
                                   int ksize, int upsample, int center, int topk, int do_softmax,
                                   int64_t *matches_out, float *scores_out, p2p_stream_t stream);
diff --git a/patch2pix_amd/_lib.py b/patch2pix_amd/_lib.py
--- a/patch2pix_amd/_lib.py
+++ b/patch2pix_amd/_lib.py
@@ -101,6 +101,9 @@
 p2p_coarse_forward_batch = _sig("p2p_coarse_forward_batch", ctypes.c_int,
                                 [ctypes.c_void_p, ctypes.c_void_p] + [ctypes.c_int] * 7 +
                                 [ctypes.c_void_p, ctypes.c_void_p, ctypes.c_void_p, ctypes.c_void_p, ctypes.c_size_t, c_stream])
+p2p_coarse_forward_matches_batch = _sig("p2p_coarse_forward_matches_batch", ctypes.c_int,
+                                        [ctypes.c_void_p, ctypes.c_void_p] + [ctypes.c_int] * 7 + [ctypes.c_void_p, ctypes.c_void_p] +
+                                        [ctypes.c_int] * 2 + [ctypes.c_void_p, ctypes.c_void_p, ctypes.c_void_p, ctypes.c_size_t, c_stream])
 p2p_neigh_consensus_batch = _sig("p2p_neigh_consensus_batch", ctypes.c_int,
                                  [ctypes.c_void_p] + [ctypes.c_int] * 5 + [ctypes.c_void_p, ctypes.c_void_p, ctypes.c_void_p,
                                                                            ctypes.c_size_t, c_stream])
@@ -195,7 +198,8 @@
            "p2p_neigh_consensus_workspace_bytes", "p2p_resize_workspace_bytes", "p2p_resize_bicubic_batch",
            "p2p_coarse_score_workspace_bytes", "p2p_coarse_score_batch", "p2p_epipolar_batch",
            "p2p_correlation_batch", "p2p_maxpool4d_batch", "p2p_mutual_matching_workspace_bytes", "p2p_mutual_matching_batch",
-           "p2p_conv4d_create", "p2p_conv4d_destroy", "p2p_conv4d_forward_batch", "p2p_l2_normalize"]
+           "p2p_conv4d_create", "p2p_conv4d_destroy", "p2p_conv4d_forward_batch", "p2p_l2_normalize",
+           "p2p_coarse_forward_matches_batch"]
 
 
 def check(status, what):
diff --git a/patch2pix_amd/csrc/api.hip b/patch2pix_amd/csrc/api.hip
--- a/patch2pix_amd/csrc/api.hip
+++ b/patch2pix_amd/csrc/api.hip
@@ -11,9 +11,9 @@
 }
 
 #ifdef P2P_EXPERIMENT
-extern "C" int p2p_version(void) { return 110 | P2P_VERSION_EXPERIMENT; }
+extern "C" int p2p_version(void) { return 111 | P2P_VERSION_EXPERIMENT; }
 #else
-extern "C" int p2p_version(void) { return 110; }
+extern "C" int p2p_version(void) { return 111; }
 #endif
 extern "C" const char *p2p_last_error(void) { return p2p::g_err; }
 
diff --git a/patch2pix_amd/csrc/coarse.hip b/patch2pix_amd/csrc/coarse.hip
--- a/patch2pix_amd/csrc/coarse.hip
+++ b/patch2pix_amd/csrc/coarse.hip
@@ -3,13 +3,6 @@
 namespace p2p {
 
 constexpr float MM_EPS = 1e-5f;
-
-__device__ __forceinline__ int f2key(float f) {
-    int b = __float_as_int(f);
-    return b >= 0 ? b : b ^ 0x7fffffff;
-}
-__device__ __forceinline__ float key2f(int k) { return __int_as_float(k >= 0 ? k : k ^ 0x7fffffff); }
-constexpr int KEY_NEG_INF = (int)0xff800000 ^ 0x7fffffff;
 
 constexpr int PREP_P = 16;
 constexpr float CORR_FP16_SCALE = 4096.0f;
diff --git a/patch2pix_amd/csrc/coarse_api.hip b/patch2pix_amd/csrc/coarse_api.hip
--- a/patch2pix_amd/csrc/coarse_api.hip
+++ b/patch2pix_amd/csrc/coarse_api.hip
@@ -114,13 +114,71 @@
             st = launch_nc_generic(*ncn->gen, P, sWs, Y, sWs, (float *)(base + ws.act), sWs, (int)nz, d0, d1, d2, d3, stream);
             Y2 = nullptr;
         } else {
-            st = launch_nc_fused(P, Y, Y2, sWs, (int)nz, d0, d1, d2, d3, ncn->wfused.dev<unsigned char>(), ncn->b2, xmax, sWs, ncn->tile, stream);
+            st = launch_nc_fused(P, Y, Y2, sWs, (int)nz, d0, d1, d2, d3, ncn->wfused.dev<unsigned char>(), ncn->b2, xmax, sWs, ncn->tile,
+                                 nullptr, nullptr, 0, stream);
         }
         if (st != P2P_OK) return st;
         launch_maxima(Y, nAc, nBc, rkey2, ckey2, sWs, sWs, Y2, nz, stream);
         launch_mm_apply(Y, nAc, nBc, rkey2, ckey2, out, sWs, sWs, nel, nullptr, Y2, nz, stream);
     }
     return check_launch("coarse_forward kernels");
+}
+
+extern "C" int p2p_coarse_forward_matches_batch(const float *featA, const float *featB, int batch, int C, int hA, int wA, int hB,
+                                                int wB, int ksize, const p2p_ncn *ncn, uint8_t *delta_out, int upsample,
+                                                int center, int64_t *matches_out, float *scores_out, void *workspace,
+                                                size_t workspace_bytes, p2p_stream_t stream_) {
+    hipStream_t stream = (hipStream_t)stream_;
+    P2P_REQUIRE(featA && featB && ncn && matches_out && scores_out && workspace, P2P_EINVAL, "p2p_coarse_forward_matches: null argument");
+    P2P_REQUIRE(batch >= 1 && batch <= 65535, P2P_EINVAL, "p2p_coarse_forward_matches: batch %d out of range", batch);
+    P2P_REQUIRE(ksize == 1 || ksize == 2 || ksize == 4, P2P_EUNSUPPORTED, "p2p_coarse_forward_matches: ksize %d not supported (1, 2 or 4)", ksize);
+    P2P_REQUIRE(C > 0 && C % 32 == 0 && C <= 256, P2P_EUNSUPPORTED, "p2p_coarse_forward_matches: channels %d (multiple of 32, <= 256)", C);
+    P2P_REQUIRE(hA > 0 && wA > 0 && hB > 0 && wB > 0 && hA % ksize == 0 && wA % ksize == 0 && hB % ksize == 0 &&
+                    wB % ksize == 0, P2P_EINVAL, "p2p_coarse_forward_matches: feature map sizes must be positive multiples of ksize");
+    const size_t ws_any = coarse_ws(C, hA, wA, hB, wB, ksize).total;
+    P2P_REQUIRE(workspace_bytes >= ws_any, P2P_ENOMEM, "p2p_coarse_forward_matches: workspace %zu < %zu bytes (one pair)", workspace_bytes, ws_any);
+    const CoarseWs ws = coarse_ws(C, hA, wA, hB, wB, ksize, ncn->gen);
+    P2P_REQUIRE(workspace_bytes >= ws.total, P2P_ENOMEM, "p2p_coarse_forward_matches: workspace %zu < %zu bytes (one pair)", workspace_bytes,
+                ws.total);
+    P2P_REQUIRE(!ncn->gen || ((uintptr_t)workspace & 15) == 0, P2P_EINVAL,
+                "p2p_coarse_forward_matches: the workspace of a generic handle must be 16-byte aligned");
+    const int nA = hA * wA, nB = hB * wB, kk = ksize * ksize;
+    const int nAc = nA / kk, nBc = nB / kk;
+    const size_t nel = (size_t)nAc * nBc, nrows = (size_t)nAc + nBc;
+    const size_t sWs = ws.total / 4;
+    const int per_launch = (int)std::min<size_t>(batch, workspace_bytes / ws.total);
+    const int d0 = hA / ksize, d1 = wA / ksize, d2 = hB / ksize, d3 = wB / ksize;
+    for (int z0 = 0; z0 < batch; z0 += per_launch) {
+        const unsigned nz = (unsigned)std::min(per_launch, batch - z0);
+        const float *fA = featA + (size_t)z0 * C * nA, *fB = featB + (size_t)z0 * C * nB;
+        char *base = (char *)workspace;
+        unsigned short *fnA = (unsigned short *)(base + ws.fnA), *fnB = (unsigned short *)(base + ws.fnB);
+        float *P = (float *)(base + ws.P), *Y = (float *)(base + ws.Y);
+        uint8_t *dout = ksize == 1 ? nullptr : (delta_out ? delta_out + (size_t)z0 * nel : (uint8_t *)(base + ws.Y2));
+        const size_t sDelta = delta_out ? nel : ws.total;
+        int *rkey1 = (int *)(base + ws.keys), *ckey1 = rkey1 + nAc, *rkey2 = ckey1 + nBc, *ckey2 = rkey2 + nAc;
+        const int nkeys = 2 * (nAc + nBc);
+        int *xmax = rkey1 + nkeys;
+        launch_prep(PrepArgs{{fA, fB}, {fnA, fnB}, {hA, hB}, {wA, wB}, {(size_t)C * nA, (size_t)C * nB}, C, ksize, 2 * sWs, rkey1, nkeys, sWs},
+                    nz, stream);
+        int st = launch_corr_pool(fnA, fnB, nA, nB, C, ksize, P, dout, 2 * sWs, sWs, sDelta, nz, stream);
+        if (st != P2P_OK) return st;
+        launch_maxima(P, nAc, nBc, rkey1, ckey1, sWs, sWs, nullptr, nz, stream);
+        launch_mm_apply(P, nAc, nBc, rkey1, ckey1, P, sWs, sWs, sWs, xmax, nullptr, nz, stream);
+        if (ncn->gen) {
+            st = launch_nc_generic(*ncn->gen, P, sWs, Y, sWs, (float *)(base + ws.act), sWs, (int)nz, d0, d1, d2, d3, stream);
+            if (st != P2P_OK) return st;
+            launch_maxima(Y, nAc, nBc, rkey2, ckey2, sWs, sWs, nullptr, nz, stream);
+        } else {
+            st = launch_nc_fused(P, Y, nullptr, sWs, (int)nz, d0, d1, d2, d3, ncn->wfused.dev<unsigned char>(), ncn->b2, xmax, sWs, ncn->tile,
+                                 rkey2, ckey2, sWs, stream);
+            if (st != P2P_OK) return st;
+        }
+        MatchArgs m{Y, dout, d0, d1, d2, d3, ksize, upsample, center, (long long *)matches_out + (size_t)z0 * nrows * 4,
+                    scores_out + (size_t)z0 * nrows, sWs, nrows, rkey2, ckey2, sWs, sDelta};
+        launch_matches_mm(m, (int)nz, stream);
+    }
+    return check_launch("coarse_forward_matches kernels");
 }
 
 extern "C" int p2p_coarse_forward(const float *featA, const float *featB, int C, int hA, int wA, int hB, int wB,
@@ -151,11 +209,11 @@
                 (size_t)batch * sizeof(int));
     const size_t nel = (size_t)hA * wA * hB * wB;
     int *xmax = (int *)workspace;
-    P2P_HIP_CHECK(hipMemsetAsync(y_out, 0, (size_t)batch * nel * sizeof(float), stream));
     P2P_HIP_CHECK(hipMemsetAsync(xmax, 0, (size_t)batch * sizeof(int), stream));
     const int st = launch_absmax(x, nel, nel, batch, xmax, 1, stream);
     if (st != P2P_OK) return st;
-    return launch_nc_fused(x, y_out, nullptr, nel, batch, hA, wA, hB, wB, ncn->wfused.dev<unsigned char>(), ncn->b2, xmax, 1, ncn->tile, stream);
+    return launch_nc_fused(x, y_out, nullptr, nel, batch, hA, wA, hB, wB, ncn->wfused.dev<unsigned char>(), ncn->b2, xmax, 1, ncn->tile,
+                           nullptr, nullptr, 0, stream);
 }
 
 extern "C" int p2p_delta_unpack(const uint8_t *delta, size_t n, int ksize, int64_t *out, p2p_stream_t stream) {
diff --git a/patch2pix_amd/csrc/coarse_common.h b/patch2pix_amd/csrc/coarse_common.h
--- a/patch2pix_amd/csrc/coarse_common.h
+++ b/patch2pix_amd/csrc/coarse_common.h
@@ -5,6 +5,13 @@
 namespace p2p {
 
 struct NcGen;
+
+__device__ __forceinline__ int f2key(float f) {
+    int b = __float_as_int(f);
+    return b >= 0 ? b : b ^ 0x7fffffff;
+}
+__device__ __forceinline__ float key2f(int k) { return __int_as_float(k >= 0 ? k : k ^ 0x7fffffff); }
+constexpr int KEY_NEG_INF = (int)0xff800000 ^ 0x7fffffff;
 
 struct PrepArgs {
     const float *F[2];
@@ -31,8 +38,11 @@
     long long *matches;
     float *scores;
     size_t sX, sM;
+    const int *rkey, *ckey;
+    size_t sKeys, sDelta;
 };
 void launch_matches(const MatchArgs &m, int batch, hipStream_t stream);
+void launch_matches_mm(const MatchArgs &m, int batch, hipStream_t stream);
 void launch_matches_topk(const MatchArgs &m, int batch, int topk, int do_softmax, hipStream_t stream);
 void launch_delta_unpack(const uint8_t *delta, size_t n, int k, long long *out, hipStream_t stream);
 
@@ -48,7 +58,7 @@
 void pack_nc_fused(const float *w1, const float *b1, const float *w2, DeviceBlob &out);
 int launch_nc_fused(const float *X, float *Y, float *Y2, size_t stride, int pairs, int d0, int d1, int d2, int d3,
                     const unsigned char *w_dev, float b2, const int *xmax, size_t xmax_stride, const int *forced_tile,
-                    hipStream_t stream);
+                    int *rkey, int *ckey, size_t key_stride, hipStream_t stream);
 int launch_absmax(const float *x, size_t n, size_t stride, int pairs, int *out, size_t out_stride, hipStream_t stream);
 
 int nc_generic_create(const p2p_ncn_config *cfg, const p2p_ncn_tensors *t, NcGen **out);
diff --git a/patch2pix_amd/csrc/consensus.hip b/patch2pix_amd/csrc/consensus.hip
--- a/patch2pix_amd/csrc/consensus.hip
+++ b/patch2pix_amd/csrc/consensus.hip
@@ -22,6 +22,8 @@
     float *Y;
     float *Y2;
     size_t stride;
+    int *rkey, *ckey;
+    size_t key_stride;
     int d0, d1, d2, d3;
     int ta, tb, tc, td, P;
     int na, nb, nc, nd;
@@ -75,7 +77,10 @@
     const int br = wave >> 2, hw = wave & 3;
     const float *X = a.X + (size_t)blockIdx.z * a.stride;
     float *Y = ((br && a.Y2) ? a.Y2 : a.Y) + (size_t)blockIdx.z * a.stride;
-    const bool plain = a.Y2 != nullptr;
+    const bool merged = a.Y2 == nullptr;
+    int *rkey = (merged && a.rkey) ? a.rkey + (size_t)blockIdx.z * a.key_stride : nullptr;
+    int *ckey = (merged && a.ckey) ? a.ckey + (size_t)blockIdx.z * a.key_stride : nullptr;
+    float colmax = -INFINITY;
     int g = blockIdx.x;
     const int dt0 = (g % a.nd) * a.td; g /= a.nd;
     const int c0 = (g % a.nc) * a.tc; g /= a.nc;
@@ -135,16 +140,65 @@
         float *slot = Ya + (aout % 3) * YSLOT;
         const int ybase = (aout * a.d1 + b0) * (int)nB + c0 * a.d3 + dt0 + lane;
         const bool lane_in = lane < TD && dt0 + lane < a.d3;
+        if (merged) {
+            if (wave >= TC) return;
+            float *cd = (float *)(sm + 2 * XPLANE + 4 * HPLANE) + (aout % 3) * YSLOT + wave * P + lane + 1;
+            const bool row_in = c0 + wave < a.d2, col_in = lane_in && row_in;
+            const int ycol = ybase + wave * a.d3;
+            auto cells = [&](int bb) {
+                float v = -INFINITY;
+                if (lane < TD) {
+                    float *c1 = cd + bb * YROW, *c2 = c1 + 3 * YSLOT;
+                    const float s = fmaxf(*c1 + a.b2, 0.f) + fmaxf(*c2 + a.b2, 0.f);
+                    *c1 = 0.f; *c2 = 0.f;
+                    if (col_in && b0 + bb < a.d1) {
+                        Y[(unsigned)(ycol + bb * (int)nB)] = s;
+                        v = s;
+                    }
+                }
+                return v;
+            };
+            auto wave_max = [&](float v) {
+                v = fmaxf(v, __uint_as_float(P2P_SWAP_ADJACENT(__float_as_uint(v))));
+                v = fmaxf(v, __uint_as_float(P2P_SWAP_PAIRS(__float_as_uint(v))));
+                v = fmaxf(v, __uint_as_float(P2P_MIRROR_HALF_ROW(__float_as_uint(v))));
+                v = fmaxf(v, __uint_as_float(P2P_SWAP_HALF_ROWS(__float_as_uint(v))));
+                v = fmaxf(v, __shfl_xor(v, 16));
+                return fmaxf(v, __shfl_xor(v, 32));
+            };
+            if (FIXED) {
+                float rv[FIXED ? FTB : 1];
+#pragma unroll
+                for (int bb = 0; bb < FTB; ++bb) rv[bb] = cells(bb);
+                if (rkey) {
+#pragma unroll
+                    for (int bb = 0; bb < FTB; ++bb) colmax = fmaxf(colmax, rv[bb]);
+#pragma unroll
+                    for (int bb = 0; bb < FTB; ++bb) rv[bb] = wave_max(rv[bb]);
+                    float mine = rv[0];
+#pragma unroll
+                    for (int bb = 1; bb < FTB; ++bb) mine = lane == bb ? rv[bb] : mine;
+                    if (lane < FTB && row_in && b0 + lane < a.d1) atomicMax(rkey + aout * a.d1 + b0 + lane, f2key(mine));
+                }
+            } else {
+                for (int bb = 0; bb < TB; ++bb) {
+                    const float v = cells(bb);
+                    if (rkey) {
+                        colmax = fmaxf(colmax, v);
+                        const float rm = wave_max(v);
+                        if (lane == 0 && row_in && b0 + bb < a.d1) atomicMax(rkey + aout * a.d1 + b0 + bb, f2key(rm));
+                    }
+                }
+            }
+            return;
+        }
         auto row = [&](int r) {
             const int bb = r / TC, ro = r - bb * TC;
             if (lane < TD) {
                 float *cell = slot + bb * YROW + ro * P + lane + 1;
                 const float v = fmaxf(*cell + a.b2, 0.f);
                 *cell = 0.f;
-                if (lane_in && b0 + bb < a.d1 && c0 + ro < a.d2) {
-                    float *dst = Y + (unsigned)(ybase + bb * (int)nB + ro * a.d3);
-                    if (plain) *dst = v; else unsafeAtomicAdd(dst, v);
-                }
+                if (lane_in && b0 + bb < a.d1 && c0 + ro < a.d2) Y[(unsigned)(ybase + bb * (int)nB + ro * a.d3)] = v;
             }
         };
         if (FIXED) {
@@ -439,6 +493,9 @@
     }
     if (pending >= 0) flush(pending);
     if (nstrips > 0 && ap_last < a_hi && ap_last >= a0) flush(ap_last);
+    if (ckey && wave < TC && lane < TD && dt0 + lane < a.d3 && c0 + wave < a.d2) {
+        atomicMax(ckey + (c0 + wave) * a.d3 + dt0 + lane, f2key(colmax));
+    }
 #ifdef NCF_TIMING
     __syncthreads();
     if (blockIdx.x == 5 && br == 0 && lane == 0) {
@@ -579,12 +636,15 @@
 
 int launch_nc_fused(const float *X, float *Y, float *Y2, size_t stride, int pairs, int d0, int d1, int d2, int d3,
                     const unsigned char *w_dev, float b2, const int *xmax, size_t xmax_stride, const int *forced_tile,
-                    hipStream_t stream) {
+                    int *rkey, int *ckey, size_t key_stride, hipStream_t stream) {
+    P2P_REQUIRE((rkey != nullptr) == (ckey != nullptr) && !(Y2 && rkey), P2P_EINVAL,
+                "consensus kernel: the maxima keys come as a pair, and only with the one-array output");
     P2P_REQUIRE((unsigned long long)d0 * d1 * d2 * d3 < (1ull << 31), P2P_EUNSUPPORTED,
                 "consensus volume %d x %d x %d x %d has 2^31 cells or more", d0, d1, d2, d3);
     NcFusedArgs a{};
     a.X = X; a.Y = Y; a.Y2 = Y2; a.stride = stride; a.d0 = d0; a.d1 = d1; a.d2 = d2; a.d3 = d3; a.w = w_dev; a.b2 = b2;
     a.xmax = xmax; a.xmax_stride = xmax_stride;
+    a.rkey = rkey; a.ckey = ckey; a.key_stride = key_stride;
     nc_fused_tile(a, pairs, forced_tile);
     const size_t lds = nc_fused_lds_bytes(a.tb, a.tc, a.P);
     P2P_REQUIRE(a.P <= 64 && lds <= NCF_LDS_MAX && a.tc + 4 <= 12 && (a.tc + 2) * a.P <= 512, P2P_EUNSUPPORTED,
diff --git a/patch2pix_amd/csrc/matches.hip b/patch2pix_amd/csrc/matches.hip
--- a/patch2pix_amd/csrc/matches.hip
+++ b/patch2pix_amd/csrc/matches.hip
@@ -3,12 +3,24 @@
 
 namespace p2p {
 
+template <bool MM>
 __device__ __forceinline__ MatchArgs match_args_of_pair(MatchArgs m, size_t z) {
     m.X += z * m.sX;
-    if (m.delta) m.delta += z * m.sX;
+    if (m.delta) m.delta += z * (MM ? m.sDelta : m.sX);
     m.matches += z * m.sM * 4;
     m.scores += z * m.sM;
+    if constexpr (MM) { m.rkey += z * m.sKeys; m.ckey += z * m.sKeys; }
     return m;
+}
+
+template <bool MM>
+__device__ __forceinline__ float match_value(const float *X, size_t at, float rmax, float cmax) {
+    const float x = X[at];
+    if constexpr (MM) {
+        float v = mm_value(x, rmax, cmax);
+        P2P_OPAQUE(v);
+        return v;
+    } else return x;
 }
 
 template <bool RECIP>
@@ -38,9 +50,9 @@
 }
 
 constexpr int MC_COLS = 16, MC_SLICES = 16;
-template <bool ONE>
+template <bool ONE, bool MM = false>
 __device__ __forceinline__ void match_cols_scan(const MatchArgs &m_, int topk, int do_softmax) {
-    const MatchArgs m = match_args_of_pair(m_, blockIdx.z);
+    const MatchArgs m = match_args_of_pair<MM>(m_, blockIdx.z);
     __shared__ float smax[MC_SLICES][MC_COLS];
     __shared__ int sarg[MC_SLICES][MC_COLS];
     __shared__ float ssum[MC_SLICES][MC_COLS];
@@ -48,6 +60,9 @@
     const int cs = threadIdx.x & (MC_COLS - 1), rs = threadIdx.x / MC_COLS;
     const int col = blockIdx.x * MC_COLS + cs;
     const bool ok = col < nB;
+    float cmax = 0.f;
+    if constexpr (MM) cmax = ok ? key2f(m.ckey[col]) : 0.f;
+    auto rmax = [&](int r) { if constexpr (MM) return key2f(m.rkey[r]); else return 0.f; };
     float pv = INFINITY, top = 0.f, total = 1.f;
     int pi = -1;
     for (int t = 0; ONE || t < topk; ++t) {
@@ -55,7 +70,7 @@
         int arg = 0x7fffffff;
         if (ok)
             for (int r = rs; r < nA; r += MC_SLICES) {
-                const float v = m.X[(size_t)r * nB + col];
+                const float v = match_value<MM>(m.X, (size_t)r * nB + col, rmax(r), cmax);
                 if (match_candidate<ONE>(v, r, pv, pi) && v > best) { best = v; arg = r; }
             }
         smax[rs][cs] = best; sarg[rs][cs] = arg;
@@ -75,7 +90,7 @@
             if (softmax) {
                 float sum = 0.f;
                 if (ok)
-                    for (int r = rs; r < nA; r += MC_SLICES) sum += expf(m.X[(size_t)r * nB + col] - gb);
+                    for (int r = rs; r < nA; r += MC_SLICES) sum += expf(match_value<MM>(m.X, (size_t)r * nB + col, rmax(r), cmax) - gb);
                 ssum[rs][cs] = sum;
                 __syncthreads();
                 if (rs == 0 && ok) {
@@ -98,23 +113,27 @@
     }
 }
 __global__ __launch_bounds__(256) void match_cols_kernel(MatchArgs m) { match_cols_scan<true>(m, 1, 1); }
+__global__ __launch_bounds__(256) void match_cols_mm_kernel(MatchArgs m) { match_cols_scan<true, true>(m, 1, 1); }
 __global__ __launch_bounds__(256) void match_cols_topk_kernel(MatchArgs m, int topk, int do_softmax) { match_cols_scan<false>(m, topk, do_softmax); }
 
-template <bool ONE>
+template <bool ONE, bool MM = false>
 __device__ __forceinline__ void match_rows_scan(const MatchArgs &m_, int topk, int do_softmax) {
-    const MatchArgs m = match_args_of_pair(m_, blockIdx.z);
+    const MatchArgs m = match_args_of_pair<MM>(m_, blockIdx.z);
     const int nA = m.hA * m.wA, nB = m.hB * m.wB;
     const int row = blockIdx.x * 4 + (threadIdx.x >> 6);
     const int lane = threadIdx.x & 63;
     if (row >= nA) return;
     const float *x = m.X + (size_t)row * nB;
+    float rmax = 0.f;
+    if constexpr (MM) rmax = key2f(m.rkey[row]);
+    auto cmax = [&](int c) { if constexpr (MM) return key2f(m.ckey[c]); else return 0.f; };
     float pv = INFINITY, top = 0.f, total = 1.f;
     int pi = -1;
     for (int t = 0; ONE || t < topk; ++t) {
         float best = -INFINITY;
         int arg = 0x7fffffff;
         for (int c = lane; c < nB; c += 64) {
-            const float v = x[c];
+            const float v = match_value<MM>(x, c, rmax, cmax(c));
             if (match_candidate<ONE>(v, c, pv, pi) && v > best) { best = v; arg = c; }
         }
 #pragma unroll
@@ -129,7 +148,7 @@
             top = best;
             if (softmax) {
                 float sum = 0.f;
-                for (int c = lane; c < nB; c += 64) sum += expf(x[c] - best);
+                for (int c = lane; c < nB; c += 64) sum += expf(match_value<MM>(x, c, rmax, cmax(c)) - best);
 #pragma unroll
                 for (int s = 32; s >= 1; s >>= 1) sum += __shfl_xor(sum, s);
                 total = sum;
@@ -147,11 +166,17 @@
     }
 }
 __global__ __launch_bounds__(256) void match_rows_kernel(MatchArgs m) { match_rows_scan<true>(m, 1, 1); }
+__global__ __launch_bounds__(256) void match_rows_mm_kernel(MatchArgs m) { match_rows_scan<true, true>(m, 1, 1); }
 __global__ __launch_bounds__(256) void match_rows_topk_kernel(MatchArgs m, int topk, int do_softmax) { match_rows_scan<false>(m, topk, do_softmax); }
 
 void launch_matches(const MatchArgs &m, int batch, hipStream_t stream) {
     hipLaunchKernelGGL(match_cols_kernel, dim3(ceil_div(m.hB * m.wB, MC_COLS), 1, batch), dim3(256), 0, stream, m);
     hipLaunchKernelGGL(match_rows_kernel, dim3(ceil_div(m.hA * m.wA, 4), 1, batch), dim3(256), 0, stream, m);
+}
+
+void launch_matches_mm(const MatchArgs &m, int batch, hipStream_t stream) {
+    hipLaunchKernelGGL(match_cols_mm_kernel, dim3(ceil_div(m.hB * m.wB, MC_COLS), 1, batch), dim3(256), 0, stream, m);
+    hipLaunchKernelGGL(match_rows_mm_kernel, dim3(ceil_div(m.hA * m.wA, 4), 1, batch), dim3(256), 0, stream, m);
 }
 
 void launch_matches_topk(const MatchArgs &m, int batch, int topk, int do_softmax, hipStream_t stream) {
diff --git a/patch2pix_amd/networks/patch2pix.py b/patch2pix_amd/networks/patch2pix.py
--- a/patch2pix_amd/networks/patch2pix.py
+++ b/patch2pix_amd/networks/patch2pix.py
@@ -200,6 +200,9 @@
             matches_ = torch.gather(matches_, 1, order.unsqueeze(-1).expand(-1, -1, 4))
         return matches_, score_
 
+    def coarse_matches_from_feats(self, feat1, feat2, ksize=2, center=True):
+        return ops.coarse_forward_matches_batch(feat1, feat2, ksize, self._weights()[0], self.upsample, center)
+
     def cal_coarse_matches_topk(self, corr4d, delta4d, topk, ksize=1, do_softmax=True, upsample=16, center=True):
         return ops.coarse_matches_topk_batch(corr4d[:, 0], self._packed_delta(delta4d, ksize), ksize, upsample, center,
                                              topk, do_softmax)
@@ -274,8 +277,7 @@
         return fine, fine_scores, coarse_matches
 
     def coarse_async(self, feats1, feats2, ksize=2):
-        corr4d, delta4d = self.forward_coarse_match(feats1[-1], feats2[-1], ksize=ksize)
-        matches_, score_ = self.cal_coarse_matches(corr4d, delta4d, ksize=ksize, upsample=self.upsample, center=True)
+        matches_, score_ = self.coarse_matches_from_feats(feats1[-1], feats2[-1], ksize=ksize)
         return dict(feats1=feats1, feats2=feats2, matches=matches_, scores=score_,
                     staged=staging.readback([matches_, score_], self._ticket_ring))
 
@@ -295,8 +297,7 @@
         if max(feats1[0].shape[-2:] + feats2[0].shape[-2:]) >= (1 << 15):
             raise NotImplementedError("predict_fine_device: image sides must be below 32768 pixels")
         _, mid_w, fine_w = self._weights()
-        corr4d, delta4d = self.forward_coarse_match(feats1[4], feats2[4], ksize=ksize)
-        matches_, score_ = self.cal_coarse_matches(corr4d, delta4d, ksize=ksize, upsample=self.upsample, center=True)
+        matches_, score_ = self.coarse_matches_from_feats(feats1[4], feats2[4], ksize=ksize)
         coarse, _, counts = ops.filter_coarse_batch(matches_, score_, ncn_thres, mutual)
         nb = coarse.shape[0]
         out = ops.regress_batch_dev(mid_w, fine_w, [[f[b] for f in feats1[:4]] for b in range(nb)],
diff --git a/patch2pix_amd/ops.py b/patch2pix_amd/ops.py
--- a/patch2pix_amd/ops.py
+++ b/patch2pix_amd/ops.py
@@ -430,6 +430,36 @@
                                                  delta.data_ptr() if delta is not None else None,
                                                  ws.data_ptr(), ws.numel(), _stream()), "p2p_coarse_forward_batch")
     return corr, delta
+
+
+def coarse_forward_matches_batch(feat_a, feat_b, ksize, ncn, upsample, center=True, out_delta=None):
+    feat_a, feat_b = _f32c(feat_a, "feat_a"), _f32c(feat_b, "feat_b")
+    if feat_a.dim() != 4 or feat_b.dim() != 4 or feat_a.shape[0] != feat_b.shape[0]:
+        raise ValueError("coarse_forward_matches_batch expects [B,C,h,w] feature maps with equal B")
+    nb, c, ha, wa = feat_a.shape
+    _, c2, hb, wb = feat_b.shape
+    if c != c2:
+        raise ValueError("channel mismatch between the two feature maps")
+    dev = feat_a.device
+    k = max(ksize, 1)
+    cells = (ha // k) * (wa // k) * (hb // k) * (wb // k)
+    n = (ha // k) * (wa // k) + (hb // k) * (wb // k)
+    matches = torch.empty((nb, n, 4), dtype=torch.int64, device=dev)
+    scores = torch.empty((nb, n), dtype=torch.float32, device=dev)
+    assert out_delta is None or (out_delta.is_contiguous() and out_delta.numel() == nb * cells and out_delta.dtype == torch.uint8)
+    if nb == 0:
+        return matches, scores
+    with torch.cuda.device(dev):
+        per_pair = _lib.p2p_coarse_workspace_bytes_for(ncn.handle, c, ha, wa, hb, wb, ksize)
+        if per_pair == 0:
+            raise ValueError("coarse_forward_matches: bad sizes")
+        pairs = max(1, min(nb, COARSE_WORKSPACE_LIMIT // per_pair))
+        ws = _workspace(dev, pairs * per_pair)
+        _lib.check(_lib.p2p_coarse_forward_matches_batch(feat_a.data_ptr(), feat_b.data_ptr(), nb, c, ha, wa, hb, wb, ksize,
+                                                         ncn.handle, out_delta.data_ptr() if out_delta is not None else None,
+                                                         upsample, int(bool(center)), matches.data_ptr(), scores.data_ptr(),
+                                                         ws.data_ptr(), ws.numel(), _stream()), "p2p_coarse_forward_matches_batch")
+    return matches, scores
 
 
 def coarse_forward(feat_a, feat_b, ksize, ncn, want_delta=True, out_corr=None, out_delta=None):
```

Result: no change. 952.2 (median of 6 runs) (+0.5%).
